# serycjon/WOFT

Measured on AMD Instinct MI355X. Metric: tracked frames/sec at 1080p, 12 RAFT iters; flow EPE vs reference, higher is better.
Workload: dtype bf16x3 (split-bf16 MFMA operands emulating fp32, fp32 accumulate)

## Files before the change

include/woft_hip.h:

```cpp
#ifndef WOFT_HIP_H
#define WOFT_HIP_H

#include <stdint.h>

#ifdef __cplusplus
extern "C" {
#endif

#define WOFT_OK 0
#define WOFT_EINVAL (-1)
#define WOFT_ELAUNCH (-2)

int woft_abi_version(void);
int woft_sizeof(int which);
int woft_set_tuning(int key, int value);

enum woft_epilogue {
    WOFT_EPI_LINEAR = 0,
    WOFT_EPI_RELU = 1,
    WOFT_EPI_SIGMOID = 2,
    WOFT_EPI_TANH = 3,
    WOFT_EPI_RELU_RES_RELU = 4,
    WOFT_EPI_GRU_ZR = 5,
    WOFT_EPI_GRU_Q = 6,
    WOFT_EPI_CTX = 7,
    WOFT_EPI_WH_MEAN = 8,
    WOFT_EPI_FLOWHEAD = 9
};

typedef struct woft_conv_params {
    const float* in0;
    const float* in1;
    int32_t cs0, cs1;
    int32_t c_split;
    int32_t n_img, h, w;
    int32_t ho, wo;
    int32_t taps_y, taps_x;
    int32_t stride, pad_y, pad_x;
    int32_t cin_pad;
    int32_t flat;
    const float* wgt;
    const void* wgt_hi;
    const void* wgt_lo;
    int32_t precision;
    const float* bias;
    float alpha;
    int32_t cout;
    int32_t cout_pad;
    float* out;
    int64_t ldo;
    int32_t co_off;
    int32_t out_w, out_pitch;
    int32_t epi;
    int32_t split;
    const float* e0;
    const float* e1;
    int32_t lde0, lde1;
    float* out1;
    int32_t ldo1;
    float* stat_sum;
    float* stat_sq;
    int32_t tile_m, tile_n;
    int32_t halo;
    int32_t in_norm;
    const float* in_mean;
    const float* in_rstd;
    const float* bias_map;
    int32_t ld_bias_map;
    const int32_t* out_index;
    const float* wh0_lookup;
    int32_t wh0_ld;
    const float* wh0_mean;
    const void* wh0_w;
    const float* wh0_bias;
    const int32_t* wh0_index;
    const void* wgt_frag;
    const void* wgt_mx;
    int32_t roi_y0, roi_x0, roi_h, roi_w;
} woft_conv_params;

int woft_conv2d(const woft_conv_params* p, void* stream);
int woft_conv2d_pair(const woft_conv_params* a, const woft_conv_params* b, void* stream);
int woft_upload_u8(const void* src, void* pinned, void* dev, int64_t bytes, int32_t n_chunks, void* stream);
int woft_split_bf16(const float* x, int64_t n, void* hi, void* lo, void* stream);
int woft_conv3x3_narrow(const float* in, int32_t cs, int32_t n_img, int32_t h, int32_t w, int32_t cin_pad,
                        const float* wgt, const float* bias, int32_t cout, float* out, int64_t ldo, int32_t co_off,
                        void* stream);
int woft_flow_head_update(const float* in, int32_t cs, int32_t h, int32_t w, int32_t cin_pad, const float* wgt,
                          const float* bias, float* delta, int64_t ld_delta, float* coords1, float* flow4,
                          float* flow_cat, int32_t ld_cat, void* stream);
int woft_flow_head_gather(const float* part, int32_t n_planes, int32_t ld, int32_t h, int32_t w, const float* bias2,
                          float* delta, int64_t ld_delta, float* coords1, float* flow4, float* flow_cat, int32_t ld_cat,
                          void* stream);
int woft_split_bf16_lines(const float* x, int64_t n, void* out, void* stream);
int woft_corr_gemm_bf16(const void* a, const void* b, int64_t m, int64_t n, int64_t rows_a, int64_t rows_b, int32_t k,
                        float alpha, void* out, int64_t ldo, int32_t terms, int32_t out_bf16, void* stream);

int woft_inorm_finalize(const float* stat_sum, const float* stat_sq, int32_t n_part, int32_t ld,
                        int32_t channels, int32_t channels_pad, int64_t count, float eps,
                        float* mean, float* rstd, void* ws, void* stream);
int64_t woft_inorm_ws_bytes(void);
int woft_inorm_apply(const float* x, const float* mean, const float* rstd, const float* res,
                     const float* res_mean, const float* res_rstd, int32_t res_mode,
                     float* out, int64_t n_pix, int32_t channels, int32_t mode, void* stream);

int woft_preprocess_bgr_u8(const uint8_t* img, int32_t h, int32_t w, float* out,
                           int32_t hp, int32_t wp, int32_t pad_top, int32_t pad_left, void* stream);

int woft_avgpool2_nhwc(const float* in, int32_t h, int32_t w, int32_t c, float* out, void* stream);

int woft_feature_pyramid(const float* in, int32_t h, int32_t w, int32_t c, int32_t levels, float* const* pooled,
                         void* const* split, int32_t terms, void* stream);

typedef struct woft_lookup_params {
    const void* vol[4];
    int32_t ht[4], wt[4];
    int64_t plane[4];
    int32_t levels, radius;
    const float* coords;
    int64_t n_pix;
    float* out;
    int32_t ldo;
    int32_t vol_bf16;
    int32_t ablate;
} woft_lookup_params;
int woft_corr_lookup(const woft_lookup_params* p, void* stream);
typedef struct woft_lookup_otf_params {
    const void* f1;
    const void* f2[4];
    int32_t h[4], w[4];
    int32_t levels, radius, terms;
    int32_t hf, wf, k;
    float alpha;
    const float* coords;
    float* out;
    const int32_t* need;
    int32_t ldo;
    int32_t ablate;
    const float* fh_part;
    const float* fh_bias;
    float* fh_delta;
    float* fh_flow4;
    float* fh_flow_cat;
    int32_t fh_planes, fh_ld, fh_ld_delta, fh_ld_cat;
    int32_t roi_y0, roi_x0, roi_h, roi_w;
    int32_t smp_y0, smp_x0, smp_h, smp_w;
} woft_lookup_otf_params;
int woft_corr_lookup_otf(const woft_lookup_otf_params* p, void* stream);
int woft_tile_rows(const float* in, int32_t h, int32_t w, int32_t c, float* out, void* stream);

int woft_coords_update(float* coords1, const float* delta, int32_t ld_delta, int32_t wf, int64_t n_pix,
                       float* flow4, float* flow_cat, int32_t ld_cat, void* stream);
int woft_coords_init(float* coords1, int32_t hf, int32_t wf, float* flow4, float* flow_cat,
                     int32_t ld_cat, void* stream);
int woft_coords_init_flow(float* coords1, const float* flow_init, int32_t hf, int32_t wf, float* flow4, float* flow_cat,
                          int32_t ld_cat, void* stream);
int woft_forward_interpolate(const float* flow, int32_t hf, int32_t wf, float* out, void* stream);

int woft_sample_bilinear(const float* data, int32_t c, int32_t h, int32_t w, const float* x, const float* y, int64_t n,
                         float* out, void* stream);
int woft_flow_chain(const float* fab, const float* fbc, int32_t h, int32_t w, float* fac, void* stream);
int woft_flow_fb(const float* fab, const float* fba, int32_t h, int32_t w, float alpha, float beta, float* err, float* ok,
                 void* stream);

int woft_flow_chain_fold(const float* prev_flow, const float* prev_cost, const float* prev_vis, const float* step_flow,
                         const float* step_wlogit, const float* step_mlogit, int32_t h, int32_t w, float unit_cost,
                         float vis_thr, int32_t k, int32_t first, float* best_flow, float* best_cost, float* best_vis,
                         int32_t* best_sel, void* stream);

#define WOFT_CHAIN_HIST 130
int woft_chain_tc(const float* flow, const float* cost, const float* vis, const int32_t* sel, const uint8_t* tmask, int32_t gh,
                  int32_t gw, int32_t mh, int32_t mw, float vis_thr, float* dst, float* w, float* ok, int32_t* hist, void* stream);

int woft_features_pack(const float* f1, int64_t ld_f1, const float* net, int64_t ld_net, const float* inp, int64_t ld_inp,
                       int64_t P, int32_t fdim, int32_t hdim, int32_t cdim, float* record, void* stream);
int woft_features_unpack(const float* record, int64_t P, int32_t fdim, int32_t hdim, int32_t cdim, float* fmap, int64_t ld_fmap,
                         void* fmap_split, float* net, int64_t ld_net, float* xbuf, int64_t ld_xbuf, float* inp_c,
                         int64_t ld_inp_c, void* stream);

int woft_colsum(const float* f, int64_t n_pix, int32_t c, double* ws, int32_t n_part, double* total, void* stream);
int woft_wh_conv0(const float* lookup, int32_t ld_lookup, const float* mean, int64_t n_pix, int32_t nwin,
                  const float* wt, const float* bias, float* out, const int32_t* index, void* stream);
int woft_wh_pack(const float* lookup, int32_t ld_lookup, const float* f1, int32_t c, const double* f2_total,
                 float alpha, int64_t n_pix, int32_t nwin, float* mean, float* x8, void* stream);
int woft_wh_reduce(const float* act, int32_t c, int32_t nwin2, const float* w, float bias,
                   int64_t n_pix, float* out, void* stream);
int woft_warp_features(const float* f, int32_t h, int32_t w, int32_t c, int32_t cs, const float* coords, int64_t n_pix,
                       float* out, int32_t ld_out, void* stream);
int woft_wh_needed(const float* pts, const int32_t* count, int32_t n_max, int32_t top, int32_t left, int32_t hf, int32_t wf,
                   const int32_t* index, int32_t n_win, int32_t* bitmap, int32_t* dyn_index, int32_t* n_needed, void* stream);

int woft_convex_upsample(const float* coords1, const float* wlow, const float* mask, int32_t ld_mask,
                         int32_t hf, int32_t wf, int32_t crop_top, int32_t crop_left, int32_t h, int32_t w,
                         float* flow_up, float* dst, float* wout, int32_t do_sigmoid, void* stream);
int woft_convex_weights_at(const float* pts, const int32_t* count, int32_t n_max, const float* wlow, const float* mask,
                           int32_t ld_mask, int32_t hf, int32_t wf, int32_t crop_top, int32_t crop_left,
                           int32_t do_sigmoid, float* wsel, void* stream);
#define WOFT_WH_TRAIN_CHUNK 16
#define WOFT_WH_TRAIN_MAX_WIN (9 * 2048)
int woft_convex_weights_at_bwd(const float* pts, const int32_t* count, int32_t n_max, const float* g_wsel, const float* wlow,
                               const float* mask, int32_t ld_mask, int32_t hf, int32_t wf, int32_t crop_top,
                               int32_t crop_left, int32_t do_sigmoid, const int32_t* index, int32_t n_win, float* g_wlow,
                               void* stream);
int woft_wh_reduce_bwd(const float* act, const float* w6, const float* g_wlow, const int32_t* index, int32_t n_win,
                       float* g_act, double* ws, float* g_w6, float* g_b6, void* stream);
int woft_wh_train_conv(const float* x, int32_t cin, const float* wt, const float* bias, const float* gate, int32_t n_win,
                       float* y, void* stream);
int64_t woft_wh_wgrad_ws_bytes(int32_t n_win, int32_t cin);
int woft_wh_wgrad(const float* gy, const float* x, int32_t cin, int32_t cin_out, int32_t n_win, float* ws, float* gw,
                  float* gb, void* stream);
int woft_flow_to_tc(const float* flow, const float* weights, int32_t h, int32_t w, float* dst, float* wout,
                    int32_t do_sigmoid, void* stream);
int woft_upflow8(const float* coords1, const float* wlow, int32_t hf, int32_t wf,
                 int32_t crop_top, int32_t crop_left, int32_t h, int32_t w,
                 float* flow_up, float* dst, float* wout, int32_t do_sigmoid, void* stream);

int woft_warp_perspective_u8(const uint8_t* img, int32_t h, int32_t w, int32_t c, const double* hinv,
                             uint8_t* out, uint8_t* valid, int32_t nearest, void* stream);

int woft_warp_perspective_window_u8(const uint8_t* img, int32_t h, int32_t w, int32_t c, const double* hinv, int32_t y0,
                                    int32_t x0, int32_t hw, int32_t ww, uint8_t* out, uint8_t* valid, int32_t nearest,
                                    void* stream);
int woft_crop_u8(const uint8_t* img, int32_t h, int32_t w, int32_t c, int32_t y0, int32_t x0, int32_t hw, int32_t ww,
                 uint8_t* out, void* stream);
int64_t woft_mask_bbox_ws_bytes(void);
int woft_mask_bbox(const uint8_t* mask, int32_t h, int32_t w, const double* hinv, uint8_t* warped, void* ws, int32_t* bbox,
                   void* stream);

int woft_resize_linear_u8(const uint8_t* img, int32_t h, int32_t w, int32_t c, uint8_t* out, int32_t ho, int32_t wo,
                          float scale_y, float scale_x, void* stream);

int64_t woft_tc_select_ws_bytes(int64_t n);
int woft_tc_select(const float* dst, const float* w, const uint8_t* tmask, const uint8_t* pwmask, int32_t gh,
                   int32_t gw, int32_t mh, int32_t mw, int32_t check_dst, const float* sobol_u, int32_t n_draw,
                   void* ws, float* pa, float* pb, float* wout, int32_t cap, int32_t* count, void* stream);
int woft_tc_flags(const float* dst, const uint8_t* tmask, const uint8_t* pwmask, int32_t gh, int32_t gw, int32_t mh,
                  int32_t mw, int32_t check_dst, uint8_t* flags, void* stream);
int woft_tc_select_vis(const float* dst, const float* w, const uint8_t* tmask, const uint8_t* pwmask, int32_t gh,
                       int32_t gw, int32_t mh, int32_t mw, int32_t check_dst, const float* sobol_u, int32_t n_draw,
                       const float* vis, int32_t vis_mode, float vis_thr, void* ws, float* pa, float* pb, float* wout,
                       int32_t cap, int32_t* count, void* stream);
int woft_tc_flags_vis(const float* dst, const uint8_t* tmask, const uint8_t* pwmask, int32_t gh, int32_t gw, int32_t mh,
                      int32_t mw, int32_t check_dst, const float* vis, int32_t vis_mode, float vis_thr, uint8_t* flags,
                      void* stream);

#define WOFT_HFIT_SINGLE_MAX 2048
int64_t woft_hfit_ws_bytes(void);
int woft_hfit(const float* pa, const float* pb, const float* w, int32_t n_max, const int32_t* count,
              int32_t reweight, float huber_k, int32_t n_irls, void* ws, float* Hout, int32_t* status, void* stream);
#define WOFT_HFIT_BATCH_MAX 65535
int woft_hfit_batched(const float* pa, const float* pb, const float* w, int32_t batch, int32_t n_max,
                      const int32_t* counts, int32_t reweight, float huber_k, int32_t n_irls, float* Hout,
                      int32_t* status, void* stream);
int woft_hfit_batched_bwd(const float* pa, const float* pb, const float* w, int32_t batch, int32_t n_max,
                          const int32_t* counts, const float* gH, float* gpa, float* gpb, float* gw, int32_t* status,
                          void* stream);
int woft_hfit_step(const float* pa, const float* pb, const float* w, int32_t n, const float* rew, int32_t first,
                   void* ws, float* res, float* Hout, int32_t* status, void* stream);
int woft_inlier_frac(const float* pa, const float* pb, int32_t n_max, const int32_t* count, const float* H,
                     float thr, float* frac, void* stream);

int64_t woft_ransac_ws_bytes(int32_t n_max, int32_t max_iters);
int woft_ransac(const float* pa, const float* pb, int32_t n_max, const int32_t* count, int32_t max_iters, double thr,
                double conf, uint64_t seed, int32_t refine, void* ws, float* Hout, int32_t* status, int32_t* info,
                uint8_t* inlier_mask, void* stream);

int64_t woft_trs_ws_bytes(int32_t n_max, int32_t max_iters);
int woft_trs(const float* pa, const float* pb, int32_t n_max, const int32_t* count, int32_t max_iters, double thr,
             double conf, uint64_t seed, int32_t refine, void* ws, float* Hout, int32_t* status, int32_t* info,
             uint8_t* inlier_mask, void* stream);

#ifdef __cplusplus
}
#endif
#endif
```

woft_amd/_lib.py:

```python
import ctypes as C
import os
from pathlib import Path

import torch

LIB_PATH = Path(os.environ.get("WOFT_HIP_LIB") or Path(__file__).resolve().parent / "lib" / "libwoft_hip.so")

EPI_LINEAR, EPI_RELU, EPI_SIGMOID, EPI_TANH, EPI_RELU_RES_RELU, EPI_GRU_ZR, EPI_GRU_Q, EPI_CTX, EPI_WH_MEAN, EPI_FLOWHEAD = range(10)

vp, i32, i64, f32 = C.c_void_p, C.c_int32, C.c_int64, C.c_float


class ConvParams(C.Structure):
    _fields_ = [
        ("in0", vp), ("in1", vp), ("cs0", i32), ("cs1", i32), ("c_split", i32),
        ("n_img", i32), ("h", i32), ("w", i32), ("ho", i32), ("wo", i32),
        ("taps_y", i32), ("taps_x", i32), ("stride", i32), ("pad_y", i32), ("pad_x", i32),
        ("cin_pad", i32), ("flat", i32), ("wgt", vp), ("wgt_hi", vp), ("wgt_lo", vp), ("precision", i32),
        ("bias", vp), ("alpha", f32),
        ("cout", i32), ("cout_pad", i32), ("out", vp), ("ldo", i64), ("co_off", i32),
        ("out_w", i32), ("out_pitch", i32), ("epi", i32), ("split", i32),
        ("e0", vp), ("e1", vp), ("lde0", i32), ("lde1", i32), ("out1", vp), ("ldo1", i32),
        ("stat_sum", vp), ("stat_sq", vp), ("tile_m", i32), ("tile_n", i32), ("halo", i32),
        ("in_norm", i32), ("in_mean", vp), ("in_rstd", vp), ("bias_map", vp), ("ld_bias_map", i32),
        ("out_index", vp),
        ("wh0_lookup", vp), ("wh0_ld", i32), ("wh0_mean", vp), ("wh0_w", vp), ("wh0_bias", vp), ("wh0_index", vp),
        ("wgt_frag", vp), ("wgt_mx", vp),
        ("roi_y0", i32), ("roi_x0", i32), ("roi_h", i32), ("roi_w", i32),
    ]


class LookupParams(C.Structure):
    _fields_ = [
        ("vol", vp * 4), ("ht", i32 * 4), ("wt", i32 * 4), ("plane", i64 * 4),
        ("levels", i32), ("radius", i32), ("coords", vp), ("n_pix", i64), ("out", vp), ("ldo", i32),
        ("vol_bf16", i32), ("ablate", i32),
    ]


class LookupOtfParams(C.Structure):
    _fields_ = [
        ("f1", vp), ("f2", vp * 4), ("h", i32 * 4), ("w", i32 * 4),
        ("levels", i32), ("radius", i32), ("terms", i32), ("hf", i32), ("wf", i32), ("k", i32),
        ("alpha", f32), ("coords", vp), ("out", vp), ("need", vp), ("ldo", i32), ("ablate", i32),
        ("fh_part", vp), ("fh_bias", vp), ("fh_delta", vp), ("fh_flow4", vp), ("fh_flow_cat", vp),
        ("fh_planes", i32), ("fh_ld", i32), ("fh_ld_delta", i32), ("fh_ld_cat", i32),
        ("roi_y0", i32), ("roi_x0", i32), ("roi_h", i32), ("roi_w", i32),
        ("smp_y0", i32), ("smp_x0", i32), ("smp_h", i32), ("smp_w", i32),
    ]


_SIGS = {
    "woft_abi_version": (i32, []),
    "woft_sizeof": (i32, [i32]),
    "woft_set_tuning": (i32, [i32, i32]),
    "woft_conv2d": (i32, [C.POINTER(ConvParams), vp]),
    "woft_conv2d_pair": (i32, [C.POINTER(ConvParams), C.POINTER(ConvParams), vp]),
    "woft_upload_u8": (i32, [vp, vp, vp, i64, i32, vp]),
    "woft_split_bf16": (i32, [vp, i64, vp, vp, vp]),
    "woft_split_bf16_lines": (i32, [vp, i64, vp, vp]),
    "woft_flow_to_tc": (i32, [vp, vp, i32, i32, vp, vp, i32, vp]),
    "woft_corr_lookup_otf": (i32, [C.POINTER(LookupOtfParams), vp]),
    "woft_conv3x3_narrow": (i32, [vp, i32, i32, i32, i32, i32, vp, vp, i32, vp, i64, i32, vp]),
    "woft_flow_head_update": (i32, [vp, i32, i32, i32, i32, vp, vp, vp, i64, vp, vp, vp, i32, vp]),
    "woft_flow_head_gather": (i32, [vp, i32, i32, i32, i32, vp, vp, i64, vp, vp, vp, i32, vp]),
    "woft_corr_gemm_bf16": (i32, [vp, vp, i64, i64, i64, i64, i32, f32, vp, i64, i32, i32, vp]),
    "woft_inorm_finalize": (i32, [vp, vp, i32, i32, i32, i32, i64, f32, vp, vp, vp, vp]),
    "woft_inorm_ws_bytes": (i64, []),
    "woft_inorm_apply": (i32, [vp, vp, vp, vp, vp, vp, i32, vp, i64, i32, i32, vp]),
    "woft_preprocess_bgr_u8": (i32, [vp, i32, i32, vp, i32, i32, i32, i32, vp]),
    "woft_avgpool2_nhwc": (i32, [vp, i32, i32, i32, vp, vp]),
    "woft_feature_pyramid": (i32, [vp, i32, i32, i32, i32, vp, vp, i32, vp]),
    "woft_corr_lookup": (i32, [C.POINTER(LookupParams), vp]),
    "woft_tile_rows": (i32, [vp, i32, i32, i32, vp, vp]),
    "woft_coords_update": (i32, [vp, vp, i32, i32, i64, vp, vp, i32, vp]),
    "woft_coords_init": (i32, [vp, i32, i32, vp, vp, i32, vp]),
    "woft_coords_init_flow": (i32, [vp, vp, i32, i32, vp, vp, i32, vp]),
    "woft_forward_interpolate": (i32, [vp, i32, i32, vp, vp]),
    "woft_sample_bilinear": (i32, [vp, i32, i32, i32, vp, vp, i64, vp, vp]),
    "woft_flow_chain": (i32, [vp, vp, i32, i32, vp, vp]),
    "woft_flow_fb": (i32, [vp, vp, i32, i32, f32, f32, vp, vp, vp]),
    "woft_flow_chain_fold": (i32, [vp, vp, vp, vp, vp, vp, i32, i32, f32, f32, i32, i32, vp, vp, vp, vp, vp]),
    "woft_chain_tc": (i32, [vp, vp, vp, vp, vp, i32, i32, i32, i32, f32, vp, vp, vp, vp, vp]),
    "woft_features_pack": (i32, [vp, i64, vp, i64, vp, i64, i64, i32, i32, i32, vp, vp]),
    "woft_features_unpack": (i32, [vp, i64, i32, i32, i32, vp, i64, vp, vp, i64, vp, i64, vp, i64, vp]),
    "woft_colsum":(i32, [vp, i64, i32, vp, i32, vp, vp]),
    "woft_wh_pack": (i32, [vp, i32, vp, i32, vp, f32, i64, i32, vp, vp, vp]),
    "woft_wh_conv0": (i32, [vp, i32, vp, i64, i32, vp, vp, vp, vp, vp]),
    "woft_wh_reduce": (i32, [vp, i32, i32, vp, f32, i64, vp, vp]),
    "woft_warp_features": (i32, [vp, i32, i32, i32, i32, vp, i64, vp, i32, vp]),
    "woft_wh_needed": (i32, [vp, vp, i32, i32, i32, i32, i32, vp, i32, vp, vp, vp, vp]),
    "woft_convex_upsample": (i32, [vp, vp, vp, i32, i32, i32, i32, i32, i32, i32, vp, vp, vp, i32, vp]),
    "woft_convex_weights_at": (i32, [vp, vp, i32, vp, vp, i32, i32, i32, i32, i32, i32, vp, vp]),
    "woft_convex_weights_at_bwd": (i32, [vp, vp, i32, vp, vp, vp, i32, i32, i32, i32, i32, i32, vp, i32, vp, vp]),
    "woft_wh_reduce_bwd": (i32, [vp, vp, vp, vp, i32, vp, vp, vp, vp, vp]),
    "woft_wh_train_conv": (i32, [vp, i32, vp, vp, vp, i32, vp, vp]),
    "woft_wh_wgrad_ws_bytes": (i64, [i32, i32]),
    "woft_wh_wgrad": (i32, [vp, vp, i32, i32, i32, vp, vp, vp, vp]),
    "woft_upflow8": (i32, [vp, vp, i32, i32, i32, i32, i32, i32, vp, vp, vp, i32, vp]),
    "woft_warp_perspective_u8": (i32, [vp, i32, i32, i32, C.POINTER(C.c_double), vp, vp, i32, vp]),
    "woft_resize_linear_u8": (i32, [vp, i32, i32, i32, vp, i32, i32, f32, f32, vp]),
    "woft_warp_perspective_window_u8": (i32, [vp, i32, i32, i32, C.POINTER(C.c_double), i32, i32, i32, i32, vp, vp, i32, vp]),
    "woft_crop_u8": (i32, [vp, i32, i32, i32, i32, i32, i32, i32, vp, vp]),
    "woft_mask_bbox_ws_bytes": (i64, []),
    "woft_mask_bbox": (i32, [vp, i32, i32, C.POINTER(C.c_double), vp, vp, vp, vp]),
    "woft_tc_select_ws_bytes": (i64, [i64]),
    "woft_tc_select": (i32, [vp, vp, vp, vp, i32, i32, i32, i32, i32, vp, i32, vp, vp, vp, vp, i32, vp, vp]),
    "woft_tc_flags": (i32, [vp, vp, vp, i32, i32, i32, i32, i32, vp, vp]),
    "woft_tc_select_vis": (i32, [vp, vp, vp, vp, i32, i32, i32, i32, i32, vp, i32, vp, i32, f32, vp, vp, vp, vp, i32, vp, vp]),
    "woft_tc_flags_vis": (i32, [vp, vp, vp, i32, i32, i32, i32, i32, vp, i32, f32, vp, vp]),
    "woft_hfit_ws_bytes": (i64, []),
    "woft_hfit": (i32, [vp, vp, vp, i32, vp, i32, f32, i32, vp, vp, vp, vp]),
    "woft_hfit_batched": (i32, [vp, vp, vp, i32, i32, vp, i32, f32, i32, vp, vp, vp]),
    "woft_hfit_batched_bwd": (i32, [vp, vp, vp, i32, i32, vp, vp, vp, vp, vp, vp, vp]),
    "woft_hfit_step": (i32, [vp, vp, vp, i32, vp, i32, vp, vp, vp, vp, vp]),
    "woft_inlier_frac": (i32, [vp, vp, i32, vp, vp, f32, vp, vp]),
    "woft_ransac_ws_bytes": (i64, [i32, i32]),
    "woft_ransac": (i32, [vp, vp, i32, vp, i32, C.c_double, C.c_double, C.c_uint64, i32, vp, vp, vp, vp, vp, vp]),
    "woft_trs_ws_bytes": (i64, [i32, i32]),
    "woft_trs": (i32, [vp, vp, i32, vp, i32, C.c_double, C.c_double, C.c_uint64, i32, vp, vp, vp, vp, vp, vp]),
}

EXPORTS = tuple(_SIGS)
_lib = None


class WoftHipError(RuntimeError):
    pass


def load():
    global _lib
    if _lib is not None:
        return _lib
    if not LIB_PATH.exists():
        raise WoftHipError(f"{LIB_PATH} is missing: build it with `python -m woft_amd.build` "
                           "(hipcc --offload-arch=gfx950); woft_amd has no CPU fallback")
    lib = C.CDLL(str(LIB_PATH))
    for name, (res, args) in _SIGS.items():
        fn = getattr(lib, name)
        fn.restype, fn.argtypes = res, args
    if lib.woft_sizeof(0) != C.sizeof(ConvParams) or lib.woft_sizeof(1) != C.sizeof(LookupParams) \
            or lib.woft_sizeof(2) != C.sizeof(LookupOtfParams):
        raise WoftHipError("ctypes mirror of woft_conv_params / woft_lookup_params is out of sync with the library")
    _lib = lib
    return lib


def check(rc, what):
    if rc != 0:
        raise WoftHipError(f"{what} failed with code {rc}")


def ptr(t):
    return None if t is None else t.data_ptr()


_RAW_STREAM = getattr(torch._C, "_cuda_getCurrentRawStream", None) if os.environ.get("WOFT_RAW_STREAM", "1") != "0" else None
_CUR_DEV = torch.cuda.current_device


def stream_ptr():
    if _RAW_STREAM is None:
        return torch.cuda.current_stream().cuda_stream
    return _RAW_STREAM(_CUR_DEV())
```

woft_amd/csrc/elementwise.hip:

```cpp
#include <string.h>

#include "common.h"
#include "halo_map.h"

namespace {

__global__ void preprocess_kernel(const uint8_t* __restrict__ img, int h, int w, float* __restrict__ out,
                                  int hp, int wp, int pad_top, int pad_left) {
    const int64_t i = (int64_t)blockIdx.x * blockDim.x + threadIdx.x;
    if (i >= (int64_t)hp * wp) return;
    const int y = (int)(i / wp), x = (int)(i - (int64_t)y * wp);
    const int sy = min(max(y - pad_top, 0), h - 1), sx = min(max(x - pad_left, 0), w - 1);
    const uint8_t* px = img + ((int64_t)sy * w + sx) * 3;
    f32x4 v;
    v[0] = 2.f * ((float)px[2] / 255.0f) - 1.0f;
    v[1] = 2.f * ((float)px[1] / 255.0f) - 1.0f;
    v[2] = 2.f * ((float)px[0] / 255.0f) - 1.0f;
    v[3] = 0.f;
    *(f32x4*)(out + i * 4) = v;
}

constexpr int FIN_T = 256, FIN_MAXG = 64, FIN_MAXC = 256;
__global__ __launch_bounds__(FIN_T) void inorm_finalize_kernel(const float* __restrict__ s1, const float* __restrict__ s2,
                                                               int n_part, int ld, int channels, int channels_pad,
                                                               int64_t count, float eps, float* __restrict__ mean,
                                                               float* __restrict__ rstd, double* ws) {
    __shared__ double red[2][FIN_T * 4];
    __shared__ int s_last;
    const int c4n = (channels + 3) / 4;
    const int rpp = FIN_T / c4n;
    const int tr = threadIdx.x / c4n, tc = threadIdx.x - tr * c4n;
    const int G = gridDim.x, g = blockIdx.x;
    double a[4] = {0.0, 0.0, 0.0, 0.0}, b[4] = {0.0, 0.0, 0.0, 0.0};
    if (tr < rpp)
        for (int i = g * rpp + tr; i < n_part; i += G * rpp) {
            const f32x4 u = *(const f32x4*)(s1 + (int64_t)i * ld + tc * 4), v = *(const f32x4*)(s2 + (int64_t)i * ld + tc * 4);
#pragma unroll
            for (int k = 0; k < 4; ++k) {
                a[k] += (double)u[k];
                b[k] += (double)v[k];
            }
        }
#pragma unroll
    for (int k = 0; k < 4; ++k) {
        red[0][threadIdx.x * 4 + k] = a[k];
        red[1][threadIdx.x * 4 + k] = b[k];
    }
    __syncthreads();
    const int c = threadIdx.x;
    double ta = 0.0, tb = 0.0;
    if (c < channels) {
        const int q = c >> 2, k = c & 3;
        for (int r = 0; r < rpp; ++r) {
            ta += red[0][(r * c4n + q) * 4 + k];
            tb += red[1][(r * c4n + q) * 4 + k];
        }
    }
    if (G > 1) {
        if (c < channels) {
            ws[(int64_t)g * 2 * FIN_MAXC + c] = ta;
            ws[(int64_t)g * 2 * FIN_MAXC + FIN_MAXC + c] = tb;
        }
        int* ticket = (int*)(ws + (int64_t)FIN_MAXG * 2 * FIN_MAXC);
        asm volatile("s_waitcnt vmcnt(0)" ::: "memory");
        __syncthreads();
        if (threadIdx.x == 0) {
            __builtin_amdgcn_fence(__ATOMIC_RELEASE, "agent");
            asm volatile("s_waitcnt vmcnt(0)" ::: "memory");
            s_last = (__hip_atomic_fetch_add(ticket, 1, __ATOMIC_RELAXED, __HIP_MEMORY_SCOPE_AGENT) == G - 1);
            if (s_last) __builtin_amdgcn_fence(__ATOMIC_ACQUIRE, "agent");
        }
        __syncthreads();
        if (!s_last) return;
        if (threadIdx.x == 0) *ticket = 0;
        int cp = 1;
        while (cp < channels) cp <<= 1;
        const int nsl = FIN_T / cp, sl = threadIdx.x / cp, cc = threadIdx.x & (cp - 1);
        double pa = 0.0, pb = 0.0;
        if (cc < channels) {
#pragma unroll 8
            for (int j = sl; j < G; j += nsl) {
                pa += ws[(int64_t)j * 2 * FIN_MAXC + cc];
                pb += ws[(int64_t)j * 2 * FIN_MAXC + FIN_MAXC + cc];
            }
        }
        __syncthreads();
        red[0][threadIdx.x] = pa;
        red[1][threadIdx.x] = pb;
        __syncthreads();
        ta = tb = 0.0;
        if (c < channels)
            for (int r = 0; r < nsl; ++r) {
                ta += red[0][r * cp + c];
                tb += red[1][r * cp + c];
            }
    }
    if (c < channels) {
        const double mu = ta / (double)count;
        double var = tb / (double)count - mu * mu;
        if (var < 0.0) var = 0.0;
        mean[c] = (float)mu;
        rstd[c] = (float)(1.0 / sqrt(var + (double)eps));
    } else if (c < channels_pad) {
        mean[c] = 0.f;
        rstd[c] = 0.f;
    }
}

__global__ void inorm_apply_kernel(const float* __restrict__ x, const float* __restrict__ mean,
                                   const float* __restrict__ rstd, const float* __restrict__ res,
                                   const float* __restrict__ res_mean, const float* __restrict__ res_rstd, int res_mode,
                                   float* __restrict__ out, int64_t n4, int channels, int mode) {
    const int64_t stride = (int64_t)gridDim.x * blockDim.x;
    for (int64_t i = (int64_t)blockIdx.x * blockDim.x + threadIdx.x; i < n4; i += stride) {
        const int c = (int)((i * 4) % channels);
        f32x4 v = *(const f32x4*)(x + i * 4);
        const f32x4 mu = *(const f32x4*)(mean + c), rs = *(const f32x4*)(rstd + c);
        f32x4 r = {0.f, 0.f, 0.f, 0.f};
        if (mode == 2) {
            r = *(const f32x4*)(res + i * 4);
            if (res_mode != 0) {
                const f32x4 rmu = *(const f32x4*)(res_mean + c), rrs = *(const f32x4*)(res_rstd + c);
#pragma unroll
                for (int k = 0; k < 4; ++k) {
                    r[k] = (r[k] - rmu[k]) * rrs[k];
                    if (res_mode == 2) r[k] = fmaxf(r[k], 0.f);
                }
            }
        }
#pragma unroll
        for (int k = 0; k < 4; ++k) {
            float y = (v[k] - mu[k]) * rs[k];
            if (mode >= 1) y = fmaxf(y, 0.f);
            if (mode == 2) y = fmaxf(r[k] + y, 0.f);
            v[k] = y;
        }
        *(f32x4*)(out + i * 4) = v;
    }
}

__global__ void avgpool2_kernel(const float* __restrict__ in, int h, int w, int c, float* __restrict__ out) {
    const int ho = h / 2, wo = w / 2, c4 = c / 4;
    const int64_t n = (int64_t)ho * wo * c4;
    const int64_t i = (int64_t)blockIdx.x * blockDim.x + threadIdx.x;
    if (i >= n) return;
    const int cc = (int)(i % c4);
    const int64_t pix = i / c4;
    const int oy = (int)(pix / wo), ox = (int)(pix - (int64_t)oy * wo);
    const float* b = in + ((int64_t)(2 * oy) * w + 2 * ox) * c + cc * 4;
    const f32x4 p00 = *(const f32x4*)b, p01 = *(const f32x4*)(b + c);
    const f32x4 p10 = *(const f32x4*)(b + (int64_t)w * c), p11 = *(const f32x4*)(b + (int64_t)w * c + c);
    f32x4 o;
#pragma unroll
    for (int k = 0; k < 4; ++k) o[k] = (p00[k] + p01[k] + p10[k] + p11[k]) * 0.25f;
    *(f32x4*)(out + pix * c + cc * 4) = o;
}

typedef __bf16 pbf16x4 __attribute__((ext_vector_type(4)));
struct PyrArgs {
    const float* in;
    float* pooled[3];
    __bf16* split[4];
    int h, w, c, levels;
};
template <int TERMS>
__device__ __forceinline__ void pyr_split(__bf16* out, int64_t pix, int c, int q, const f32x4 v) {
    const pbf16x4 hi = __builtin_convertvector(v, pbf16x4);
    if (TERMS == 3) {
        __bf16* line = out + pix * (2 * (int64_t)c) + (q >> 3) * 64 + (q & 7) * 4;
        *(pbf16x4*)line = hi;
        *(pbf16x4*)(line + 32) = __builtin_convertvector(v - __builtin_convertvector(hi, f32x4), pbf16x4);
    } else {
        *(pbf16x4*)(out + pix * (int64_t)c + q * 4) = hi;
    }
}
template <int TERMS>
__global__ __launch_bounds__(256) void feature_pyramid_kernel(const PyrArgs a) {
    __shared__ f32x4 l2s[4][64];
    const int bxn = (a.w + 7) / 8;
    const int by = (int)blockIdx.x / bxn, bx = (int)blockIdx.x - by * bxn;
    const int sub = threadIdx.x >> 6, q0 = threadIdx.x & 63;
    const int c4 = a.c / 4;
    const int y0 = by * 8 + (sub >> 1) * 4, x0 = bx * 8 + (sub & 1) * 4;
    const int h1 = a.h / 2, w1 = a.w / 2, h2 = h1 / 2, w2 = w1 / 2, h3 = h2 / 2, w3 = w2 / 2;
    for (int qb = 0; qb < c4; qb += 64) {
        const int q = qb + q0;
        const bool qok = q < c4;
        f32x4 p[4][4];
#pragma unroll
        for (int i = 0; i < 4; ++i)
#pragma unroll
            for (int j = 0; j < 4; ++j) {
                const int y = y0 + i, x = x0 + j;
                const bool ok = qok && y < a.h && x < a.w;
                p[i][j] = ok ? *(const f32x4*)(a.in + ((int64_t)y * a.w + x) * a.c + q * 4) : f32x4{0.f, 0.f, 0.f, 0.f};
                if (ok) pyr_split<TERMS>(a.split[0], (int64_t)y * a.w + x, a.c, q, p[i][j]);
            }
        f32x4 o1[2][2];
#pragma unroll
        for (int i = 0; i < 2; ++i)
#pragma unroll
            for (int j = 0; j < 2; ++j) {
#pragma unroll
                for (int k = 0; k < 4; ++k)
                    o1[i][j][k] = (p[2 * i][2 * j][k] + p[2 * i][2 * j + 1][k] + p[2 * i + 1][2 * j][k] + p[2 * i + 1][2 * j + 1][k]) * 0.25f;
                const int y = y0 / 2 + i, x = x0 / 2 + j;
                if (a.levels > 1 && qok && y < h1 && x < w1) {
                    const int64_t pix = (int64_t)y * w1 + x;
                    *(f32x4*)(a.pooled[0] + pix * a.c + q * 4) = o1[i][j];
                    pyr_split<TERMS>(a.split[1], pix, a.c, q, o1[i][j]);
                }
            }
        f32x4 o2;
#pragma unroll
        for (int k = 0; k < 4; ++k) o2[k] = (o1[0][0][k] + o1[0][1][k] + o1[1][0][k] + o1[1][1][k]) * 0.25f;
        {
            const int y = y0 / 4, x = x0 / 4;
            if (a.levels > 2 && qok && y < h2 && x < w2) {
                const int64_t pix = (int64_t)y * w2 + x;
                *(f32x4*)(a.pooled[1] + pix * a.c + q * 4) = o2;
                pyr_split<TERMS>(a.split[2], pix, a.c, q, o2);
            }
        }
        __syncthreads();
        l2s[sub][q0] = o2;
        __syncthreads();
        if (sub == 0 && a.levels > 3 && qok && by < h3 && bx < w3) {
            f32x4 o3;
#pragma unroll
            for (int k = 0; k < 4; ++k) o3[k] = (l2s[0][q0][k] + l2s[1][q0][k] + l2s[2][q0][k] + l2s[3][q0][k]) * 0.25f;
            const int64_t pix = (int64_t)by * w3 + bx;
            *(f32x4*)(a.pooled[2] + pix * a.c + q * 4) = o3;
            pyr_split<TERMS>(a.split[3], pix, a.c, q, o3);
        }
    }
}

}

extern "C" int woft_abi_version(void) { return 10000 * 0 + 100 * 4 + 0; }

extern "C" int woft_preprocess_bgr_u8(const uint8_t* img, int32_t h, int32_t w, float* out, int32_t hp, int32_t wp,
                                      int32_t pad_top, int32_t pad_left, void* stream) {
    if (!img || !out || h <= 0 || w <= 0 || hp < h || wp < w || pad_top < 0 || pad_left < 0) return WOFT_EINVAL;
    const int64_t n = (int64_t)hp * wp;
    hipLaunchKernelGGL(preprocess_kernel, dim3((unsigned)ceil_div64(n, 256)), dim3(256), 0, (hipStream_t)stream, img, h,
                       w, out, hp, wp, pad_top, pad_left);
    return woft_launch_status();
}

extern "C" int64_t woft_inorm_ws_bytes(void) { return (int64_t)FIN_MAXG * 2 * FIN_MAXC * 8 + 64; }

extern "C" int woft_inorm_finalize(const float* stat_sum, const float* stat_sq, int32_t n_part, int32_t ld,
                                   int32_t channels, int32_t channels_pad, int64_t count, float eps, float* mean,
                                   float* rstd, void* ws, void* stream) {
    if (!stat_sum || !stat_sq || !mean || !rstd || n_part <= 0 || channels <= 0 || count <= 0) return WOFT_EINVAL;
    if (channels_pad < channels || channels_pad > FIN_MAXC || ld % 4 != 0 || ld < channels) return WOFT_EINVAL;
    const int rpp = FIN_T / ((channels + 3) / 4);
    int G = (n_part + 4 * rpp - 1) / (4 * rpp);
    G = (ws == nullptr || G < 2) ? 1 : (G > FIN_MAXG ? FIN_MAXG : G);
    hipLaunchKernelGGL(inorm_finalize_kernel, dim3(G), dim3(FIN_T), 0, (hipStream_t)stream, stat_sum, stat_sq, n_part, ld,
                       channels, channels_pad, count, eps, mean, rstd, (double*)ws);
    return woft_launch_status();
}

extern "C" int woft_inorm_apply(const float* x, const float* mean, const float* rstd, const float* res,
                                const float* res_mean, const float* res_rstd, int32_t res_mode, float* out,
                                int64_t n_pix, int32_t channels, int32_t mode, void* stream) {
    if (!x || !mean || !rstd || !out || n_pix <= 0 || channels <= 0 || channels % 4 != 0) return WOFT_EINVAL;
    if (mode < 0 || mode > 2 || (mode == 2 && !res)) return WOFT_EINVAL;
    if (res_mode < 0 || res_mode > 2 || (res_mode != 0 && (mode != 2 || !res_mean || !res_rstd))) return WOFT_EINVAL;
    const int64_t n4 = n_pix * channels / 4;
    const int64_t blocks = ceil_div64(n4, 256);
    hipLaunchKernelGGL(inorm_apply_kernel, dim3((unsigned)(blocks < 8192 ? blocks : 8192)), dim3(256), 0,
                       (hipStream_t)stream, x, mean, rstd, res, res_mean, res_rstd, res_mode, out, n4, channels, mode);
    return woft_launch_status();
}

extern "C" int woft_avgpool2_nhwc(const float* in, int32_t h, int32_t w, int32_t c, float* out, void* stream) {
    if (!in || !out || h < 2 || w < 2 || c <= 0 || c % 4 != 0) return WOFT_EINVAL;
    const int64_t n = (int64_t)(h / 2) * (w / 2) * (c / 4);
    hipLaunchKernelGGL(avgpool2_kernel, dim3((unsigned)ceil_div64(n, 256)), dim3(256), 0, (hipStream_t)stream, in, h,
                       w, c, out);
    return woft_launch_status();
}

extern "C" int woft_upload_u8(const void* src, void* pinned, void* dev, int64_t bytes, int32_t n_chunks, void* stream) {
    if (!src || !pinned || !dev || bytes <= 0 || n_chunks < 1 || n_chunks > 64) return WOFT_EINVAL;
    const int64_t per = ((bytes + n_chunks - 1) / n_chunks + 4095) / 4096 * 4096;
    for (int64_t off = 0; off < bytes; off += per) {
        const int64_t n = bytes - off < per ? bytes - off : per;
        memcpy((char*)pinned + off, (const char*)src + off, (size_t)n);
        if (hipMemcpyAsync((char*)dev + off, (const char*)pinned + off, (size_t)n, hipMemcpyHostToDevice, (hipStream_t)stream) != hipSuccess)
            return WOFT_ELAUNCH;
    }
    return WOFT_OK;
}

extern "C" int woft_sizeof(int which) {
    if (which == 0) return (int)sizeof(woft_conv_params);
    if (which == 1) return (int)sizeof(woft_lookup_params);
    if (which == 2) return (int)sizeof(woft_lookup_otf_params);
    return -1;
}

extern "C" int woft_feature_pyramid(const float* in, int32_t h, int32_t w, int32_t c, int32_t levels, float* const* pooled,
                                    void* const* split, int32_t terms, void* stream) {
    if (!in || !pooled || !split || h <= 0 || w <= 0 || c <= 0 || c % 32 != 0 || levels < 1 || levels > 4 ||
        (terms != 1 && terms != 3))
        return WOFT_EINVAL;
    PyrArgs a;
    a.in = in; a.h = h; a.w = w; a.c = c; a.levels = levels;
    for (int l = 0; l < 4; ++l) {
        a.split[l] = l < levels ? (__bf16*)split[l] : nullptr;
        if (l < levels && a.split[l] == nullptr) return WOFT_EINVAL;
        if (l >= 1) {
            a.pooled[l - 1] = l < levels ? pooled[l - 1] : nullptr;
            if (l < levels && a.pooled[l - 1] == nullptr) return WOFT_EINVAL;
        }
    }
    const dim3 grid((unsigned)(((h + 7) / 8) * ((w + 7) / 8)));
    if (terms == 3) hipLaunchKernelGGL(feature_pyramid_kernel<3>, grid, dim3(256), 0, (hipStream_t)stream, a);
    else hipLaunchKernelGGL(feature_pyramid_kernel<1>, grid, dim3(256), 0, (hipStream_t)stream, a);
    return woft_launch_status();
}
```

woft_amd/csrc/lookup_otf.hip:

```cpp
#include <type_traits>
#include <utility>

#include "common.h"
#include "dma.h"

namespace {

typedef __bf16 bf16x8 __attribute__((ext_vector_type(8)));

template <bool MAX>
__device__ __forceinline__ int wave_reduce_minmax(int v) {
#define WOFT_DPP_STEP(ctrl, rmask)                                                        \
    {                                                                                     \
        const int o = __builtin_amdgcn_update_dpp(v, v, ctrl, rmask, 0xf, false);         \
        v = MAX ? (o > v ? o : v) : (o < v ? o : v);                                      \
    }
    WOFT_DPP_STEP(0xB1, 0xf)
    WOFT_DPP_STEP(0x4E, 0xf)
    WOFT_DPP_STEP(0x141, 0xf)
    WOFT_DPP_STEP(0x140, 0xf)
    WOFT_DPP_STEP(0x142, 0xa)
    WOFT_DPP_STEP(0x143, 0xc)
#undef WOFT_DPP_STEP
    return __builtin_amdgcn_readlane(v, 63);
}

__device__ __forceinline__ void lds_dma16x2(const void* gbase, uint32_t o0_plus_4096, uint32_t o1, uint32_t lds_addr_second) {
    const uint64_t gb = (uint64_t)(uintptr_t)gbase;
    const uint32_t g_hi = (uint32_t)__builtin_amdgcn_readfirstlane((int)(uint32_t)(gb >> 32));
    const uint32_t g_lo = (uint32_t)__builtin_amdgcn_readfirstlane((int)(uint32_t)gb);
    const uint64_t gu = ((uint64_t)g_hi << 32) | (uint64_t)g_lo;
    uint32_t saved_m0;
    asm volatile("s_mov_b32 %0, m0\n\ts_mov_b32 m0, %1\n\ts_nop 0\n\t"
                 "global_load_lds_dwordx4 %2, %4 offset:-4096\n\tglobal_load_lds_dwordx4 %3, %4\n\ts_mov_b32 m0, %0"
                 : "=&s"(saved_m0)
                 : "s"(lds_addr_second), "v"(o0_plus_4096), "v"(o1), "s"(gu)
                 : "memory", "vcc");
}

struct BlockRect {
    int by0, bx0, ny, nx;
};
__host__ __device__ __forceinline__ BlockRect block_rect(const woft_lookup_otf_params& p) {
    if ((p.roi_y0 | p.roi_x0 | p.roi_h | p.roi_w) == 0) return BlockRect{0, 0, (p.hf + 7) / 8, (p.wf + 7) / 8};
    const int by0 = p.roi_y0 / 8, bx0 = p.roi_x0 / 8;
    return BlockRect{by0, bx0, (p.roi_y0 + p.roi_h - 1) / 8 - by0 + 1, (p.roi_x0 + p.roi_w - 1) / 8 - bx0 + 1};
}

template <int TERMS, int R, int K, int ABL>
__global__ __launch_bounds__(256, 2) void corr_lookup_otf_kernel(const woft_lookup_otf_params p) {
    constexpr int NPX = 64, NT = 256;
    constexpr int NW = 2 * R + 1, N2 = NW * NW;
    constexpr int NPL = (TERMS == 1) ? 1 : 2;
    constexpr int LD = (TERMS == 1) ? K : 2 * K;
    constexpr int NK = LD / 64;
    constexpr int NSUB = (TERMS == 1) ? 4 : 2;
    constexpr int GS = 2, NGRP = 3, NST = GS * NGRP, DEPTH = NGRP - 1;
    static_assert(NK % GS == 0, "K steps per chunk must be a multiple of the steps per barrier");
    __shared__ __attribute__((aligned(16))) __bf16 stage[NST * 64 * 64];
    constexpr int WS = NW + 1, WLD = WS * WS + 2;
    __shared__ __attribute__((aligned(16))) float Wn[NPX * WLD];
    constexpr int MAXL = 4;
    __shared__ __attribute__((aligned(16))) int s_org[MAXL][NPX];
    __shared__ __attribute__((aligned(16))) int s_pm[MAXL][NPX];
    __shared__ float s_fx[MAXL][NPX], s_fy[MAXL][NPX];
    __shared__ int s_box[MAXL][4];
    __shared__ float s_trash[64];
    __shared__ uint32_t s_probe[24];
    int n_probe = 0;

    const int tid = threadIdx.x;
    const int lane = tid & 63;
    const int wave = __builtin_amdgcn_readfirstlane(tid >> 6);
    const int wm = wave >> 1, wn = wave & 1;
    const int r32 = lane & 31, hh = lane >> 5;
    constexpr int ld = LD, nk = NK;
    const BlockRect br = block_rect(p);
    const int tiles_x = br.nx, ntiles = br.nx * br.ny;
    int tile;
    {
        const int q = ntiles / 8, rr = ntiles % 8, xcd = blockIdx.x % 8, idx = blockIdx.x / 8;
        tile = (xcd < rr ? xcd * (q + 1) : rr * (q + 1) + (xcd - rr) * q) + idx;
    }
    const int px0 = (br.bx0 + tile % tiles_x) * 8, py0 = (br.by0 + tile / tiles_x) * 8;
    const bool sampled = (p.smp_y0 | p.smp_x0 | p.smp_h | p.smp_w) == 0 ||
                         (py0 < p.smp_y0 + p.smp_h && py0 + 8 > p.smp_y0 && px0 < p.smp_x0 + p.smp_w && px0 + 8 > p.smp_x0);
    if (p.need != nullptr) {
        int any = 0;
        if (tid < NPX) {
            const int y = py0 + (tid >> 3), x = px0 + (tid & 7);
            if (y < p.hf && x < p.wf) any = p.need[y * p.wf + x];
        }
        if (!__syncthreads_or(any)) return;
    }
    float cx = 0.f, cy = 0.f;
    if (tid < NPX) {
        const int y = py0 + (tid >> 3), x = px0 + (tid & 7);
        if (y < p.hf && x < p.wf) {
            const int64_t i = (int64_t)y * p.wf + x;
            cx = p.coords[i * 2];
            cy = p.coords[i * 2 + 1];
            if (p.fh_part != nullptr) {
                typedef float f32x2 __attribute__((ext_vector_type(2)));
                float dx = p.fh_bias ? p.fh_bias[0] : 0.f, dy = p.fh_bias ? p.fh_bias[1] : 0.f;
                const int64_t plane = (int64_t)p.hf * p.wf * p.fh_ld;
#pragma unroll
                for (int ky = 0; ky < 3; ++ky)
#pragma unroll
                    for (int kx = 0; kx < 3; ++kx) {
                        const int yy = y + ky - 1, xx = x + kx - 1;
                        f32x2 v = {0.f, 0.f};
                        if (yy >= 0 && yy < p.hf && xx >= 0 && xx < p.wf) {
                            const float* src = p.fh_part + ((int64_t)yy * p.wf + xx) * p.fh_ld + (ky * 3 + kx) * 2;
                            v = *(const f32x2*)src;
                            for (int t = 1; t < p.fh_planes; ++t) v += *(const f32x2*)(src + t * plane);
                        }
                        dx += v[0];
                        dy += v[1];
                    }
                p.fh_delta[i * p.fh_ld_delta] = dx;
                p.fh_delta[i * p.fh_ld_delta + 1] = dy;
                cx += dx;
                cy += dy;
                ((float*)p.coords)[i * 2] = cx;
                ((float*)p.coords)[i * 2 + 1] = cy;
                const float fx = cx - (float)x, fy = cy - (float)y;
                if (p.fh_flow4 != nullptr) *(f32x4*)(p.fh_flow4 + i * 4) = f32x4{fx, fy, 0.f, 0.f};
                if (p.fh_flow_cat != nullptr) {
                    p.fh_flow_cat[i * p.fh_ld_cat] = fx;
                    p.fh_flow_cat[i * p.fh_ld_cat + 1] = fy;
                }
            }
        }
    }
    if (!sampled) return;
    if (tid < NPX) {
        const int y = py0 + (tid >> 3), x = px0 + (tid & 7);
        const bool cvalid = y < p.hf && x < p.wf;
#pragma unroll
        for (int l = 0; l < MAXL; ++l) {
            if (l < p.levels) {
                int wx0 = 0, wy0 = 0;
                float fx = 0.f, fy = 0.f;
                if (cvalid) {
                    const float sc = 1.0f / (float)(1 << l);
                    const float xs = cx * sc, ys = cy * sc;
                    float flx = floorf(xs), fly = floorf(ys);
                    fx = xs - flx;
                    fy = ys - fly;
                    flx = fminf(fmaxf(flx, -1.0e6f), 1.0e6f);
                    fly = fminf(fmaxf(fly, -1.0e6f), 1.0e6f);
                    wx0 = (int)flx - R;
                    wy0 = (int)fly - R;
                }
                s_fx[l][tid] = fx; s_fy[l][tid] = fy;
                const int ox = wx0 < -16384 ? -16384 : (wx0 > 16384 ? 16384 : wx0);
                const int oy = wy0 < -16384 ? -16384 : (wy0 > 16384 ? 16384 : wy0);
                s_org[l][tid] = cvalid ? ((ox & 0xffff) | (oy << 16)) : 0x40004000;
                s_pm[l][tid] = 4 * (tid * WLD - (ox * WS + oy));
                const int b0 = wave_reduce_minmax<false>(cvalid ? wx0 : 0x3fffffff), b1 = wave_reduce_minmax<true>(cvalid ? wx0 : -0x3fffffff);
                const int b2 = wave_reduce_minmax<false>(cvalid ? wy0 : 0x3fffffff), b3 = wave_reduce_minmax<true>(cvalid ? wy0 : -0x3fffffff);
                if (tid == 0) { s_box[l][0] = b0; s_box[l][1] = b1; s_box[l][2] = b2; s_box[l][3] = b3; }
            }
        }
    }
    bf16x8 afr[NK][NSUB][NPL];
    {
        const int m = wm * 32 + r32;
        int y = py0 + (m >> 3), x = px0 + (m & 7);
        y = y < p.hf ? y : p.hf - 1;
        x = x < p.wf ? x : p.wf - 1;
        const char* row = (const char*)p.f1 + (int64_t)(y * p.wf + x) * (ld * 2);
#pragma unroll
        for (int ks = 0; ks < NK; ++ks)
#pragma unroll
            for (int s2 = 0; s2 < NSUB; ++s2) {
                if (TERMS == 0) {
                    afr[ks][s2][0] = *(const bf16x8*)(row + ks * 128 + hh * 64 + s2 * 32);
                    afr[ks][s2][NPL - 1] = *(const bf16x8*)(row + ks * 128 + hh * 64 + s2 * 32 + 16);
                } else {
                    afr[ks][s2][0] = *(const bf16x8*)(row + ks * 128 + (s2 * 2 + hh) * 16);
                    if (TERMS == 3) afr[ks][s2][NPL - 1] = *(const bf16x8*)(row + ks * 128 + 64 + (s2 * 2 + hh) * 16);
                }
            }
    }
    const int swz = (4 * (wave & 1) + (lane >> 4)) & 7;
    const uint32_t chunk_off = (uint32_t)(((lane & 7) ^ swz) * 16);
    const uint32_t st_addr = lds_addr_of(stage);
    const int sw = (r32 >> 1) & 7;
    const __bf16* b_rows = stage + (wn * 32 + r32) * 64;

    uint32_t* stamps = ((ABL & 16) && tid == 0 && p.ldo >= 4 * N2 + 24)
                           ? (uint32_t*)(p.out + ((int64_t)py0 * p.wf + px0) * p.ldo + 4 * N2) : nullptr;
    int n_stamp = 0;
    auto stamp = [&]() __attribute__((always_inline)) { if ((ABL & 16) && stamps && n_stamp < 24) stamps[n_stamp++] = (uint32_t)__builtin_amdgcn_s_memtime(); };
    stamp();

    __syncthreads();
    stamp();
    auto sel4 = [](int l, int a0, int a1, int a2, int a3) __attribute__((always_inline)) { return l == 0 ? a0 : (l == 1 ? a1 : (l == 2 ? a2 : a3)); };
    int W = 0, bx0 = 0, by0 = 0, bw = 1, N = 0, S = 0, G = 0;
    bool clipped = false;
    const char* f2 = nullptr;
    uint32_t b_off[2] = {0u, 0u};
    int is_c = 0, is_k = 0;
    auto issue = [&](int s_idx) __attribute__((always_inline)) {
        if (is_k == 0) {
#pragma unroll
            for (int tt = 0; tt < 2; ++tt) {
                int pos = is_c * 64 + (wave + 4 * tt) * 8 + (lane >> 3);
                pos = pos < N ? pos : N - 1;
                const int by = pos / bw, bx = pos - by * bw;
                b_off[tt] = (uint32_t)((by0 + by) * W + bx0 + bx) * (uint32_t)(ld * 2) + chunk_off + (tt == 0 ? 4096u : 0u);
            }
        }
        const uint32_t st = st_addr + (uint32_t)(s_idx % NST) * 8192u;
        if (!(ABL & 1) || s_idx < NST) lds_dma16x2(f2 + is_k * 128, b_off[0], b_off[1], st + (uint32_t)(wave + 4) * 1024u);
        if (++is_k == nk) { is_k = 0; ++is_c; }
    };
    auto start_level = [&](int l) __attribute__((always_inline)) {
        W = sel4(l, p.w[0], p.w[1], p.w[2], p.w[3]);
        const int H = sel4(l, p.h[0], p.h[1], p.h[2], p.h[3]);
        bx0 = __builtin_amdgcn_readfirstlane(s_box[l][0]);
        by0 = __builtin_amdgcn_readfirstlane(s_box[l][2]);
        int bx1 = __builtin_amdgcn_readfirstlane(s_box[l][1]), by1 = __builtin_amdgcn_readfirstlane(s_box[l][3]);
        clipped = bx0 < 0 || by0 < 0 || bx1 + NW > W - 1 || by1 + NW > H - 1;
        bx0 = bx0 > 0 ? bx0 : 0;
        by0 = by0 > 0 ? by0 : 0;
        bx1 = (bx1 + NW < W - 1) ? bx1 + NW : W - 1;
        by1 = (by1 + NW < H - 1) ? by1 + NW : H - 1;
        bw = bx1 - bx0 + 1;
        const int bh = by1 - by0 + 1;
        N = (bw > 0 && bh > 0) ? bw * bh : 0;
        bw = bw > 0 ? bw : 1;
        f2 = (const char*)(l == 0 ? p.f2[0] : (l == 1 ? p.f2[1] : (l == 2 ? p.f2[2] : p.f2[3])));
        S = ((N + 63) / 64) * nk;
        G = S / GS;
        is_c = 0; is_k = 0;
        for (int g = 0; g < DEPTH && g < G; ++g)
#pragma unroll
            for (int e = 0; e < GS; ++e) issue(g * GS + e);
    };
    start_level(0);
    for (int l = 0; l < p.levels; ++l) {
        if (clipped) {
            const f32x4 z4 = {0.f, 0.f, 0.f, 0.f};
            for (int i = tid; i < NPX * WLD / 4; i += NT) ((f32x4*)Wn)[i] = z4;
            static_assert((NPX * WLD) % 4 == 0, "window array is zeroed 16 bytes at a time");
        }
        f32x16 acc;
#pragma unroll
        for (int r = 0; r < 16; ++r) acc[r] = 0.f;
        int c0 = 0;
        stamp();
        for (int s0 = 0; s0 < S; s0 += NK) {
            [&]<int... KGS>(std::integer_sequence<int, KGS...>) {
            ([&] {
                constexpr int kg = KGS;
                const int g = s0 / GS + kg;
                const int rem = G - 1 - g;
                const bool pr = (ABL & 64) && l == 0 && s0 == NK && tid == 0;
                auto mark = [&]() __attribute__((always_inline)) { if ((ABL & 64) && pr && n_probe < 24) s_probe[n_probe++] = (uint32_t)__builtin_amdgcn_s_memtime(); };
                mark();
                if (rem >= DEPTH - 1) dma_wait<(DEPTH - 1) * GS * 2>();
                else dma_wait<0>();
                mark();
                __syncthreads();
                mark();
                const bool feed = g + DEPTH < G;
                mark();
                constexpr int NU = GS * NSUB;
                bf16x8 bq[2][NPL];
                auto load_b = [&](auto u_tag) __attribute__((always_inline)) {
                    constexpr int u = decltype(u_tag)::value;
                    constexpr int e = u / NSUB, s2 = u % NSUB;
                    const __bf16* br = b_rows + ((s0 + kg * GS + e) % NST) * 4096;
                    if (TERMS == 0) {
                        bq[u & 1][0] = *(const bf16x8*)(br + ((hh * 4 + s2 * 2) ^ sw) * 8);
                        bq[u & 1][NPL - 1] = *(const bf16x8*)(br + ((hh * 4 + s2 * 2 + 1) ^ sw) * 8);
                    } else {
                        bq[u & 1][0] = *(const bf16x8*)(br + ((s2 * 2 + hh) ^ sw) * 8);
                        if (TERMS == 3) bq[u & 1][NPL - 1] = *(const bf16x8*)(br + ((4 + s2 * 2 + hh) ^ sw) * 8);
                    }
                };
                if (!(ABL & 2)) {
                    load_b(std::integral_constant<int, 0>{});
                    [&]<int... U>(std::integer_sequence<int, U...>) {
                        ([&] {
                            constexpr int u = U, e = u / NSUB, s2 = u % NSUB;
                            constexpr int ks = kg * GS + e;
                            if constexpr (u + 1 < NU) load_b(std::integral_constant<int, u + 1>{});
                            __builtin_amdgcn_sched_barrier(0);
                            const bf16x8 bh = bq[u & 1][0];
                            if (TERMS == 0) {
                                const f32x4 a0 = __builtin_bit_cast(f32x4, afr[ks][s2][0]), a1 = __builtin_bit_cast(f32x4, afr[ks][s2][NPL - 1]);
                                const f32x4 b0 = __builtin_bit_cast(f32x4, bh), b1 = __builtin_bit_cast(f32x4, bq[u & 1][NPL - 1]);
#pragma unroll
                                for (int s = 0; s < 4; ++s) acc = __builtin_amdgcn_mfma_f32_32x32x2f32(a0[s], b0[s], acc, 0, 0, 0);
#pragma unroll
                                for (int s = 0; s < 4; ++s) acc = __builtin_amdgcn_mfma_f32_32x32x2f32(a1[s], b1[s], acc, 0, 0, 0);
                            } else if (TERMS == 3) {
                                const bf16x8 bl = bq[u & 1][NPL - 1];
                                const bf16x8 ah = afr[ks][s2][0], al = afr[ks][s2][NPL - 1];
                                acc = __builtin_amdgcn_mfma_f32_32x32x16_bf16(al, bh, acc, 0, 0, 0);
                                acc = __builtin_amdgcn_mfma_f32_32x32x16_bf16(ah, bl, acc, 0, 0, 0);
                                acc = __builtin_amdgcn_mfma_f32_32x32x16_bf16(ah, bh, acc, 0, 0, 0);
                            } else {
                                acc = __builtin_amdgcn_mfma_f32_32x32x16_bf16(afr[ks][s2][0], bh, acc, 0, 0, 0);
                            }
                            __builtin_amdgcn_sched_barrier(0);
                            if constexpr (s2 == 0) { if (feed) issue((g + DEPTH) * GS + e); }
                        }(), ...);
                    }(std::make_integer_sequence<int, NU>{});
                }
                mark();
            }(), ...);
            }(std::make_integer_sequence<int, NK / GS>{});
            if (!(ABL & 4)) {
                typedef int i32x4 __attribute__((ext_vector_type(4)));
                typedef unsigned short u16x2 __attribute__((ext_vector_type(2)));
                const int pos = c0 + wn * 32 + r32;
                const int by = pos / bw, bx = pos - by * bw;
                const int tx = bx0 + bx, ty = by0 + by;
                const int d_pos = pos < N ? ((tx & 0xffff) | (ty << 16)) : 0x7fff7fff;
                const uint32_t d_q4 = lds_addr_of(Wn) + 4u * (uint32_t)(tx * WS + ty);
                const uint32_t trash = lds_addr_of(s_trash) + 4u * (uint32_t)lane;
                i32x4 org[4], pm[4];
#pragma unroll
                for (int g4 = 0; g4 < 4; ++g4) {
                    org[g4] = *(const i32x4*)&s_org[l][wm * 32 + 4 * hh + 8 * g4];
                    pm[g4] = *(const i32x4*)&s_pm[l][wm * 32 + 4 * hh + 8 * g4];
                }
                const u16x2 lim = {(unsigned short)(WS - 1), (unsigned short)(WS - 1)};
#pragma unroll
                for (int r = 0; r < 16; ++r) {
                    const u16x2 dd = __builtin_bit_cast(u16x2, d_pos) - __builtin_bit_cast(u16x2, (int)org[r >> 2][r & 3]);
                    const u16x2 mn = __builtin_elementwise_min(dd, lim);
                    const bool inside = __builtin_bit_cast(uint32_t, mn) == __builtin_bit_cast(uint32_t, dd);
                    const uint32_t cell = inside ? (uint32_t)pm[r >> 2][r & 3] + d_q4 : trash;
                    *(__attribute__((address_space(3))) float*)(uintptr_t)cell = acc[r] * p.alpha;
                }
            }
#pragma unroll
            for (int r = 0; r < 16; ++r) acc[r] = 0.f;
            if ((ABL & 64) && l == 0 && s0 == NK && tid == 0 && n_probe < 24) s_probe[n_probe++] = (uint32_t)__builtin_amdgcn_s_memtime();
            c0 += 64;
        }
        stamp();
        __syncthreads();
        if (l + 1 < p.levels) start_level(l + 1);
        if (!(ABL & 8)) {
            for (int it = tid; it < NPX * NW; it += NT) {
                const int pix = it / NW, i = it - pix * NW;
                const int gy = py0 + (pix >> 3), gx = px0 + (pix & 7);
                if (gy >= p.hf || gx >= p.wf) continue;
                const float fx = s_fx[l][pix], fy = s_fy[l][pix];
                const float* cq = Wn + pix * WLD + i * WS;
                float h[WS];
#pragma unroll
                for (int j = 0; j < WS; ++j) h[j] = cq[j] * (1.f - fx) + cq[WS + j] * fx;
                float* o = p.out + ((int64_t)gy * p.wf + gx) * p.ldo + l * N2 + i * NW;
#pragma unroll
                for (int j = 0; j < NW; ++j) o[j] = h[j] * (1.f - fy) + h[j + 1] * fy;
            }
        }
        stamp();
        __syncthreads();
    }
    if ((ABL & 64) && tid == 0 && p.ldo >= 4 * N2 + 24) {
        uint32_t* o = (uint32_t*)(p.out + ((int64_t)py0 * p.wf + px0) * p.ldo + 4 * N2);
        for (int i = 0; i < 24; ++i) o[i] = i < n_probe ? s_probe[i] : 0u;
    }
}

}

extern "C" int woft_corr_lookup_otf(const woft_lookup_otf_params* pp, void* stream) {
    if (!pp) return WOFT_EINVAL;
    const woft_lookup_otf_params& p = *pp;
    if (p.levels < 1 || p.levels > 4 || !p.f1 || !p.coords || !p.out || p.hf <= 0 || p.wf <= 0) return WOFT_EINVAL;
    if (p.terms != 0 && p.terms != 1 && p.terms != 3) return WOFT_EINVAL;
    if (p.k <= 0 || p.k % (p.terms == 1 ? 64 : 32) != 0) return WOFT_EINVAL;
    const int64_t row_bytes = (int64_t)p.k * (p.terms == 1 ? 2 : 4);
    if ((int64_t)p.hf * p.wf * row_bytes >= (1ll << 32)) return WOFT_EINVAL;
    for (int l = 0; l < p.levels; ++l)
        if (!p.f2[l] || p.h[l] <= 0 || p.w[l] <= 0 || (int64_t)p.h[l] * p.w[l] * row_bytes >= (1ll << 32)) return WOFT_EINVAL;
    const int nout = p.levels * (2 * p.radius + 1) * (2 * p.radius + 1);
    if (p.ldo < nout) return WOFT_EINVAL;
    if (p.fh_part != nullptr && (p.fh_delta == nullptr || p.fh_planes < 1 || p.fh_ld < 20 || p.fh_ld % 4 != 0 || p.fh_ld_delta < 2 ||
                                 (p.fh_flow_cat != nullptr && p.fh_ld_cat < 2) || p.need != nullptr))
        return WOFT_EINVAL;
    for (int l = 0; l < p.levels; ++l) {
        if (p.h[l] > 16384 || p.w[l] > 16384) return WOFT_EINVAL;
        if ((int64_t)p.h[l] * p.w[l] * row_bytes >= (1ll << 32) - 4096) return WOFT_EINVAL;
    }
    auto rect_bad = [&](int y0, int x0, int h, int w) {
        return (y0 | x0 | h | w) != 0 && (h <= 0 || w <= 0 || y0 < 0 || x0 < 0 || y0 > p.hf - h || x0 > p.wf - w);
    };
    if (rect_bad(p.roi_y0, p.roi_x0, p.roi_h, p.roi_w) || rect_bad(p.smp_y0, p.smp_x0, p.smp_h, p.smp_w)) return WOFT_EINVAL;
    if (p.ablate != 0 && ((p.roi_y0 | p.roi_x0 | p.roi_h | p.roi_w) != 0 || (p.smp_y0 | p.smp_x0 | p.smp_h | p.smp_w) != 0)) return WOFT_EINVAL;
    hipStream_t s = (hipStream_t)stream;
    const BlockRect br = block_rect(p);
    dim3 grid((unsigned)(br.nx * br.ny));
#define OTF(T, RR, KK, AB) woft_launch(0, corr_lookup_otf_kernel<T, RR, KK, AB>, grid, dim3(256), 0, s, p)
    if (p.ablate != 0) {
        if (!(p.k == 256 && p.radius == 4 && p.terms == 3)) return WOFT_EINVAL;
        switch (p.ablate) {
            case 1: OTF(3, 4, 256, 1); break;
            case 2: OTF(3, 4, 256, 2); break;
            case 3: OTF(3, 4, 256, 3); break;
            case 8: OTF(3, 4, 256, 8); break;
            case 15: OTF(3, 4, 256, 15); break;
            case 16: OTF(3, 4, 256, 16); break;
            case 64: OTF(3, 4, 256, 64); break;
            default: return WOFT_EINVAL;
        }
    } else if (p.k == 256 && p.radius == 4) {
        if (p.terms == 3) OTF(3, 4, 256, 0); else if (p.terms == 0) OTF(0, 4, 256, 0); else OTF(1, 4, 256, 0);
    } else if (p.k == 128 && p.radius == 3) {
        if (p.terms == 3) OTF(3, 3, 128, 0); else if (p.terms == 0) OTF(0, 3, 128, 0); else OTF(1, 3, 128, 0);
    }
    else return WOFT_EINVAL;
#undef OTF
    return woft_launch_status();
}
```

woft_amd/engine.py:

```python
import math
import os
from typing import NamedTuple

import torch

from . import _lib, conv_select, flow_region, ops, wh_train
from .conv_select import KERNELS, Kernel
from .ops import Act, new_act

EPI = _lib
DEFER_NORM = os.environ.get("WOFT_DEFER_NORM", "1") != "0"
FUSE_FLOWHEAD = os.environ.get("WOFT_FUSE_FLOWHEAD", "1") != "0"
PAIR_BRANCHES = os.environ.get("WOFT_PAIR", "1") != "0"
PYRAMID_ONE_LAUNCH = os.environ.get("WOFT_PYRAMID", "1") != "0"
FOLD_GATHER = os.environ.get("WOFT_FOLD_GATHER", "1") != "0"


def _ru(x, m):
    return (x + m - 1) // m * m


class Step(NamedTuple):
    kind: str
    arg: object
    tag: str = None


class _Folded(NamedTuple):
    prog_iter_first: list
    prog_iter: list
    prog_iter_last: list
    gather: list
    lookup: object


def _timed(sink, launch, *args, extra=None):
    if sink is None:
        return launch(*args)
    s, e = torch.cuda.Event(enable_timing=True), torch.cuda.Event(enable_timing=True)
    s.record()
    launch(*args)
    e.record()
    sink.append((s, e) if extra is None else (s, e, extra()))


def _head_layers(sd, prefix, cin):
    idx = sorted(int(k.split(".")[2]) for k in sd if k.startswith(prefix) and k.endswith(".weight"))
    shapes = [tuple(sd[f"{prefix}{i}.weight"].shape) for i in idx]
    ok = not (len(idx) < 2 or shapes[-1][0] != 1 or shapes[-1][2:] != (1, 1) or shapes[0][1] != cin
              or any(a[0] != b[1] for a, b in zip(shapes, shapes[1:])) or any(sh[2] != sh[3] or sh[2] % 2 == 0 for sh in shapes))
    return idx, shapes, ok


class _Spec:

    def __init__(self, small):
        self.small = small
        if small:
            self.fdim, self.hdim, self.cdim, self.radius = 128, 96, 64, 3
            self.fnorm, self.cnorm = "instance", "none"
        else:
            self.fdim, self.hdim, self.cdim, self.radius = 256, 128, 128, 4
            self.fnorm, self.cnorm = "instance", "batch"
        self.levels = 4
        self.nwin = 2 * self.radius + 1
        self.corr_c = self.levels * self.nwin ** 2
        self.corr_cs = _ru(self.corr_c, 32)
        self.xdim = _ru(self.cdim + (82 if small else 128), 32)
        self.flow_off = self.cdim + (80 if small else 126)


class _Enc:

    def __init__(self, sd, p, norm, spec, out_split=None):
        self.norm = norm

        def get(name, stride=1, flat_cs=0, bn=None):
            w, b = sd[name + ".weight"], sd[name + ".bias"]
            if norm == "batch" and bn is not None:
                w, b = ops.fold_bn(w, b, sd[bn + ".weight"], sd[bn + ".bias"], sd[bn + ".running_mean"],
                                   sd[bn + ".running_var"])
            return ops.pack_conv(w, b, stride=stride, flat_cs=flat_cs)

        self.conv1 = get(p + ".conv1", 2, 4, p + ".norm1")
        self.blocks = []
        for li, stride in ((1, 1), (2, 2), (3, 2)):
            for bi in range(2):
                q = f"{p}.layer{li}.{bi}"
                s = stride if bi == 0 else 1
                if spec.small:
                    convs = [get(q + ".conv1", 1, bn=q + ".norm1"), get(q + ".conv2", s, bn=q + ".norm2"),
                             get(q + ".conv3", 1, bn=q + ".norm3")]
                else:
                    convs = [get(q + ".conv1", s, bn=q + ".norm1"), get(q + ".conv2", 1, bn=q + ".norm2")]
                blk = dict(stride=s, convs=convs)
                if s != 1:
                    blk["down"] = get(q + ".downsample.0", s, bn=q + ".downsample.1")
                self.blocks.append(blk)
        w2, b2 = sd[p + ".conv2.weight"], sd[p + ".conv2.bias"]
        if out_split:
            self.conv2_net = ops.pack_conv(w2[:out_split], b2[:out_split])
            self.conv2_inp = ops.pack_conv(w2[out_split:], b2[out_split:])
        else:
            self.conv2 = ops.pack_conv(w2, b2)


class RaftEngine:
    def __init__(self, state_dict, small=False, weighted=True, precision="fp32", corr="volume", volume_storage=None,
                 mask_head=False):
        if precision not in ops.PRECISION:
            raise ValueError(f"precision must be one of {sorted(ops.PRECISION)}")
        if corr not in ("volume", "otf"):
            raise ValueError("corr must be 'volume' or 'otf'")
        self.precision = precision
        self.prec_corr = self.prec_wh = "bf16x3" if precision in ("fp16", "f16mx8") else precision
        self.corr = corr
        self.volume_storage = volume_storage or ("bf16" if precision == "bf16" else "fp32")
        if self.volume_storage not in ("fp32", "bf16") or (self.volume_storage == "bf16" and precision == "fp32"):
            raise ValueError("volume_storage: 'fp32', or 'bf16' with the split-bf16 precisions (their GEMM packs it)")
        _lib.load()
        if not torch.cuda.is_available():
            raise _lib.WoftHipError("woft_amd needs a HIP device: there is no CPU fallback")
        sd = {k: v.detach().float().cpu() for k, v in state_dict.items()}
        self.weighted, self.small, self.mask_head = weighted, small, bool(mask_head)
        self.spec = sp = _Spec(small)
        self.radius, self.levels = sp.radius, sp.levels
        if self.mask_head and not weighted:
            raise ValueError("mask_head: the MaskHead belongs to WeightedRAFT (weighted_raft.py:75-76), not to plain RAFT")
        self.convc2 = self.mk1 = self.mk2 = None
        self.wh_std = self.wh_flat0 = False
        self.wh0 = self.wh2 = self.wh4 = self.wh0_frag = self.wh_layers = self.wh6_c = self.wh6_w = self.wh6_b = None
        self.mh_shapes = self.mh_layers = self.mh_c = self.mh_wlast = self.mh_b = None
        self._pack_encoders(sd)
        self._pack_update_block(sd)
        if weighted:
            self._pack_weight_head(sd)
        if self.mask_head:
            self._pack_mask_head(sd)
        self._plans = {}

    def _pack_encoders(self, sd):
        self.fnet = _Enc(sd, "fnet", self.spec.fnorm, self.spec)
        self.cnet = _Enc(sd, "cnet", self.spec.cnorm, self.spec, out_split=self.spec.hdim)

    def _pack_update_block(self, sd):
        sp, small, precision = self.spec, self.small, self.precision
        u = "update_block."
        g = lambda n, **kw: ops.pack_conv(sd[u + n + ".weight"], sd[u + n + ".bias"], **kw)
        self.convc1 = g("encoder.convc1")
        self.convf1 = g("encoder.convf1", flat_cs=4)
        self.convf2 = g("encoder.convf2")
        self.convm = g("encoder.conv")
        self.fh1 = g("flow_head.conv1")
        self.fh2 = g("flow_head.conv2")
        self.fh2_frag = (ops.pack_flowhead_frags(sd[u + "flow_head.conv2.weight"], 2 if precision in ("bf16x3", "f16mx8") else 1,
                                                 f16=precision == "fp16")
                         if precision != "fp32" and FUSE_FLOWHEAD else None)
        if not small:
            self.convc2 = g("encoder.convc2")
            self.mk1 = g("mask.0")
            self.mk2 = g("mask.2", scale=0.25)
        hd_, cd_, mot = sp.hdim, sp.cdim, (82 if small else 128)
        dyn = [(0, hd_, 0), (hd_ + cd_, hd_ + cd_ + mot, hd_)]
        ctx = [(hd_, hd_ + cd_, 0)]
        self.zr_dyn, self.zr_inp, self.q_dyn, self.q_inp = [], [], [], []
        for sfx, pd in (("", None),) if small else (("1", (0, 2)), ("2", (2, 0))):
            zr_w, zr_b = (torch.cat([sd[f"{u}gru.convz{sfx}{s}"], sd[f"{u}gru.convr{sfx}{s}"]], 0) for s in (".weight", ".bias"))
            q_w, q_b = sd[f"{u}gru.convq{sfx}.weight"], sd[f"{u}gru.convq{sfx}.bias"]
            self.zr_dyn.append(ops.pack_conv(zr_w, None, padding=pd, cin_layout=dyn))
            self.zr_inp.append(ops.pack_conv(zr_w, zr_b, padding=pd, cin_layout=ctx))
            self.q_dyn.append(ops.pack_conv(q_w, None, padding=pd, cin_layout=dyn))
            self.q_inp.append(ops.pack_conv(q_w, q_b, padding=pd, cin_layout=ctx))

    def _pack_weight_head(self, sd):
        sp, precision = self.spec, self.precision
        w = "weight_head.net."
        idx, shapes, ok = _head_layers(sd, w, sp.levels + 1)
        if not ok:
            raise ValueError(f"weight head layers {shapes}: not a WeightHead (weighted_raft.py:318-345)")
        self.wh_std = shapes == [(128, 5, 3, 3), (128, 128, 3, 3), (128, 128, 3, 3), (1, 128, 1, 1)]
        last = idx[-1]
        if self.wh_std:
            self.wh0, self.wh2, self.wh4, self.wh0_frag = self._wh_std_packed(sd)
        else:
            k0 = shapes[0][2]
            self.wh_flat0 = k0 * 8 <= 32
            self.wh_layers = [ops.pack_conv(sd[f"{w}{idx[0]}.weight"], sd[f"{w}{idx[0]}.bias"], flat_cs=8 if self.wh_flat0 else 0)]
            self.wh_layers += [ops.pack_conv(sd[f"{w}{i}.weight"], sd[f"{w}{i}.bias"]) for i in idx[1:-1]]
        self.wh6_c = shapes[-1][1]
        self.wh6_w = torch.zeros(_ru(self.wh6_c, 4))
        self.wh6_w[:self.wh6_c] = sd[f"{w}{last}.weight"].reshape(-1)
        self.wh6_w = self.wh6_w.contiguous().cuda()
        self.wh6_b = float(sd[f"{w}{last}.bias"].item())

    def _wh_std_packed(self, sd):
        w = "weight_head.net."
        wh0 = ops.pack_conv(sd[w + "0.weight"], sd[w + "0.bias"], flat_cs=8)
        wh2 = ops.pack_conv(sd[w + "2.weight"], sd[w + "2.bias"])
        wh4 = ops.pack_conv(sd[w + "4.weight"], sd[w + "4.bias"])
        wh0_frag = (ops.pack_wh0_frags(sd[w + "0.weight"], 2 if self.prec_wh == "bf16x3" else 1)
                    if self.precision != "fp32" and self.spec.nwin == 9 else None)
        return wh0, wh2, wh4, wh0_frag

    def repack_weight_head(self, sd):
        assert self.weighted and self.wh_std
        sd = {k: v.detach().float().cpu() for k, v in sd.items() if k.startswith("weight_head.net.")}
        wh0, wh2, wh4, frag = self._wh_std_packed(sd)
        for old, new in ((self.wh0, wh0), (self.wh2, wh2), (self.wh4, wh4)):
            ops.repack_conv_(old, new)
        if self.wh0_frag is not None:
            self.wh0_frag.copy_(frag)
        self.wh6_w[:self.wh6_c].copy_(sd["weight_head.net.6.weight"].reshape(-1))
        self.wh6_b = float(sd["weight_head.net.6.bias"].item())
        for plan in self._plans.values():
            plan.wh0_t.copy_(self.wh0.wgt[:128].t())
            plan.wh6_b.fill_(self.wh6_b)
            if plan._wh6_pad is not None:
                plan._wh6_pad[:self.wh6_c].copy_(self.wh6_w[:self.wh6_c])
            plan._graphs.clear()

    def _pack_mask_head(self, sd):
        sp = self.spec
        m = "mask_head.net."
        idx, shapes, ok = _head_layers(sd, m, 2 * sp.fdim)
        if not ok:
            raise ValueError(f"mask head layers {shapes}: not a MaskHead on {2 * sp.fdim} channels (weighted_raft.py:387-409)")
        self.mh_shapes = shapes
        self.mh_layers = [ops.pack_conv(sd[f"{m}{i}.weight"], sd[f"{m}{i}.bias"]) for i in idx[:-1]]
        self.mh_c = shapes[-1][1]
        self.mh_wlast = sd[f"{m}{idx[-1]}.weight"].reshape(-1).clone()
        self.mh_b = float(sd[f"{m}{idx[-1]}.bias"].item())

    def plan(self, hp, wp, slot=0):
        key = (hp, wp) if slot == 0 else (hp, wp, slot)
        if key not in self._plans:
            self._plans[key] = _Plan(self, hp, wp)
        return self._plans[key]

    def drop_plan(self, key):
        return self._plans.pop(key, None)


class _Plan:

    def __init__(self, eng, hp, wp):
        assert hp % 8 == 0 and wp % 8 == 0
        self.eng, self.hp, self.wp = eng, hp, wp
        self.prec, self.prec_corr, self.prec_wh = eng.precision, eng.prec_corr, eng.prec_wh
        self.otf = eng.corr == "otf"
        self.hf, self.wf, self.P = hp // 8, wp // 8, (hp // 8) * (wp // 8)
        self.source_tag = None
        self.target_valid = False
        self.lookup_events = None
        self.wh_events = None
        self.conv_events = None
        self._graphs = {}
        self.mk = self.mask = self.prog_iter_last = self.folded = self.fh_part = None
        self.x8 = self.x32 = self.wmean = self.wlow = self.cs_ws = self.cs_tot = self.wh6_b = self._wh6_pad = None
        self.a1 = self.a2 = self.wh0_t = self.wh_last = None
        self.wh0_direct = self.wh0_fused = self.wh_fused = False
        self.prog_mask, self.prog_wh, self.prog_mh = [], [], []
        self.mh_warped = self.mh_last = self.mh_w = self.mh_low = None
        self.flow_region, self._flow_regions = None, {}
        self.wh_region, self._wh_regions = None, {}
        self._wh_dyn = {}
        self._wh_train = None
        self._plan_features()
        self._plan_update_block()
        if eng.weighted:
            self._plan_weight_head()
        if eng.mask_head:
            self._plan_mask_head()

    @staticmethod
    def _z(*s, dtype=torch.float32):
        return torch.zeros(*s, dtype=dtype, device="cuda")

    def _plan_features(self):
        eng, sp, hp, wp, hf, wf, P, z = self.eng, self.eng.spec, self.hp, self.wp, self.hf, self.wf, self.P, self._z
        self.img = [new_act(1, hp, wp, 3, cs=4), new_act(1, hp, wp, 3, cs=4)]
        self.f1rows = z(_ru(P, 128), sp.fdim)
        self.f1 = Act(self.f1rows[:P], 1, hf, wf, sp.fdim)
        x3 = self.prec_corr == "bf16x3"
        bf = lambda rows: (z(rows.shape[0], rows.shape[1] * (2 if x3 else 1), dtype=torch.bfloat16)
                           if self.prec != "fp32" else None)
        self.f1s = bf(self.f1rows)
        if self.otf and self.prec == "fp32":
            self.f1s = self.f1rows
        self.dims, self.f2rows, self.f2act, self.vol, self.f2s = [], [], [], [], []
        h, w = hf, wf
        for _ in range(sp.levels):
            self.dims.append((h, w))
            self.f2act.append(new_act(1, h, w, sp.fdim, zero=True))
            if self.otf:
                self.f2s.append(bf(self.f2act[-1].t) if self.prec != "fp32" else self.f2act[-1].t)
            else:
                n = ops.tiled_dims(h, w)[2]
                rows = z(_ru(n, 128), sp.fdim)
                self.f2rows.append(rows)
                self.f2s.append(bf(rows))
                self.vol.append(z(P, n, dtype=torch.bfloat16 if eng.volume_storage == "bf16" else torch.float32))
            h, w = h // 2, w // 2
        self.net0 = new_act(1, hf, wf, sp.hdim, zero=True)
        self.xbuf = new_act(1, hf, wf, sp.xdim, zero=True)
        self.flow_cat = self.xbuf.t[:, sp.flow_off:]
        self._enc_scratch = {}
        n_stat = 2 * math.ceil((hp // 2) * (wp // 2) / 64) * 128
        self.stats = (z(n_stat), z(n_stat))
        self.fin_ws = ops.inorm_ws("cuda")
        self._norm_slots = {}
        self.prog_f_src = self._encoder_program(eng.fnet, self.img[0], [(eng.fnet.conv2, self.f1, 0, EPI.EPI_LINEAR)])
        self.prog_f_dst = self._encoder_program(eng.fnet, self.img[1],
                                                [(eng.fnet.conv2, self.f2act[0], 0, EPI.EPI_LINEAR)])
        self.prog_c_src = self._encoder_program(eng.cnet, self.img[0],
                                                [(eng.cnet.conv2_net, self.net0, 0, EPI.EPI_TANH),
                                                 (eng.cnet.conv2_inp, self.xbuf, 0, EPI.EPI_RELU)])
        self.prog_volume = self._volume_program()

    def _plan_update_block(self):
        eng, sp, hf, wf, P, z, cp = self.eng, self.eng.spec, self.hf, self.wf, self.P, self._z, self._cp
        self.coords = z(P, 2)
        self.corr = new_act(1, hf, wf, sp.corr_c, cs=sp.corr_cs, zero=True)
        self.c1 = new_act(1, hf, wf, 96 if sp.small else 256, zero=True)
        self.cf = new_act(1, hf, wf, 128 if sp.small else 256, zero=True)
        self.fl1 = new_act(1, hf, wf, 64 if sp.small else 128, zero=True)
        self.flow4 = new_act(1, hf, wf, 2, cs=4, zero=True)
        self.inp_c = new_act(1, hf, wf, sp.cdim, zero=True)
        self.gate_bias = [(new_act(1, hf, wf, 2 * sp.hdim, zero=True), new_act(1, hf, wf, sp.hdim, zero=True))
                          for _ in eng.zr_inp]
        self.prog_gate_bias = []
        for k in range(len(eng.zr_inp)):
            self.prog_gate_bias += [Step("conv", cp(self.inp_c, eng.zr_inp[k], self.gate_bias[k][0])),
                                    Step("conv", cp(self.inp_c, eng.q_inp[k], self.gate_bias[k][1]))]
        self.zbuf = new_act(1, hf, wf, sp.hdim, zero=True)
        self.rh = new_act(1, hf, wf, sp.hdim, zero=True)
        self.hA = new_act(1, hf, wf, sp.hdim, zero=True)
        self.hB = new_act(1, hf, wf, sp.hdim, zero=True)
        self.fh = new_act(1, hf, wf, 128 if sp.small else 256, zero=True)
        self.delta = new_act(1, hf, wf, 2, cs=4, zero=True)
        self.flow_init = z(2, hf, wf)
        if self.otf:
            terms = 3 if self.prec_corr == "bf16x3" else (0 if self.prec == "fp32" else 1)
            self.lookup = ops.make_lookup_otf_params(self.f1s, self.f2s, self.dims, hf, wf, sp.fdim, self.coords,
                                                     self.corr.t, sp.radius, terms)
        else:
            self.lookup = ops.make_lookup_params(self.vol, self.dims, self.coords, self.corr.t, sp.radius)
        self.prog_iter_first = self._iter_program(first=True)
        self.prog_iter = self._iter_program(first=False)
        if not sp.small:
            self.mk = new_act(1, hf, wf, 256, zero=True)
            self.mask = new_act(1, hf, wf, 576, zero=True)
            self.prog_mask = [cp(self.hB, eng.mk1, self.mk, epi=EPI.EPI_RELU),
                              cp(self.mk, eng.mk2, self.mask)]
            k = next((i for i, st in enumerate(self.prog_iter) if st.tag == "fh1"), None)
            if PAIR_BRANCHES and k is not None and ops.pair_ok(self.prog_iter[k].arg, self.prog_mask[0]):
                self.prog_iter_last = (self.prog_iter[:k] + [Step("conv2", (self.prog_iter[k].arg, self.prog_mask[0]), "fh1+mk1")]
                                       + self.prog_iter[k + 1:])
        self.folded = self._fold_gather_programs()

    def _plan_weight_head(self):
        eng, sp, P, z, n = self.eng, self.eng.spec, self.P, self._z, self.eng.spec.nwin
        self.x8 = new_act(P, n, n, 5, cs=8, zero=True)
        self.wmean = z(P)
        self.wlow = z(P)
        self.cs_ws = z(256, sp.fdim, dtype=torch.float64)
        self.cs_tot = z(sp.fdim, dtype=torch.float64)
        self.wh6_b = torch.tensor([eng.wh6_b], dtype=torch.float32, device="cuda")
        cpw = lambda *a, **kw: self._cp(*a, precision=self.prec_wh, **kw)
        if eng.wh_std:
            self.a2 = new_act(P, n, n, 128)
            self.wh0_direct = n in (7, 9)
            self.wh0_fused = (eng.wh0_frag is not None and os.environ.get("WOFT_WH0_FUSED", "1") != "0"
                              and ops.select_conv(self.a2, eng.wh2, precision=self.prec_wh).kernel is Kernel.WINDOW_9X9)
            self.a1 = self.a2 if self.wh0_fused else new_act(P, n, n, 128)
            self.wh0_t = eng.wh0.wgt[:128].t().contiguous()
            self.prog_wh, self.wh_fused = self._wh_program(P, None)
            return
        x = self.x8
        if not eng.wh_flat0:
            self.x32 = x = new_act(P, n, n, 5, cs=32, zero=True)
        for pc in eng.wh_layers:
            out = new_act(P, n, n, pc.cout, cs=_ru(_ru(pc.cout, 4), 32), zero=True)
            self.prog_wh.append(cpw(x, pc, out, epi=EPI.EPI_RELU))
            x = out
        self.wh_last = x

    def _plan_mask_head(self):
        eng, sp, hf, wf = self.eng, self.eng.spec, self.hf, self.wf
        self.mh_warped = new_act(1, hf, wf, sp.fdim, zero=True)
        x = None
        for k, pc in enumerate(eng.mh_layers):
            out = new_act(1, hf, wf, pc.cout, cs=_ru(_ru(pc.cout, 4), 32), zero=True)
            src = dict(x2=self.mh_warped, c_split=sp.fdim) if k == 0 else {}
            self.prog_mh.append(self._cp(self.f1 if k == 0 else x, pc, out, epi=EPI.EPI_RELU, precision=self.prec_wh, **src))
            x = out
        self.mh_last = x
        self.mh_w = torch.zeros(x.cs, dtype=torch.float32)
        self.mh_w[:eng.mh_c] = eng.mh_wlast
        self.mh_w = self.mh_w.to("cuda")
        self.mh_low = self._z(self.P)

    def _fold_gather_programs(self):
        progs = [p for p in (self.prog_iter_first, self.prog_iter, self.prog_iter_last) if p is not None]
        if not (FOLD_GATHER and self.otf and all(p and p[-1].kind == "fh_gather" and p[0].kind == "lookup" for p in progs)):
            return None
        n_planes, bias2 = self.prog_iter[-1].arg
        lk = ops.copy_params(self.lookup)
        lk.fh_part, lk.fh_bias, lk.fh_delta = _lib.ptr(self.fh_part), _lib.ptr(bias2), _lib.ptr(self.delta.t)
        lk.fh_flow4, lk.fh_flow_cat = _lib.ptr(self.flow4.t), self.flow_cat.data_ptr()
        lk.fh_planes, lk.fh_ld, lk.fh_ld_delta, lk.fh_ld_cat = n_planes, self.fh_part.shape[1], self.delta.cs, self.xbuf.cs
        lk._keep = (self.lookup._keep, bias2, self.fh_part)
        first, mid, last = ([head] + p[1:-1] if p is not None else None
                            for p, head in ((self.prog_iter_first, self.prog_iter_first[0]), (self.prog_iter, Step("lookup", lk)),
                                            (self.prog_iter_last, Step("lookup", lk))))
        return _Folded(first, mid, last, [self.prog_iter[-1]], lk)

    def _wh_program(self, n_win, index):
        eng, n = self.eng, self.eng.spec.nwin
        cp = lambda *a, **kw: self._cp(*a, precision=self.prec_wh, **kw)
        a1 = Act(self.a1.t[:n_win * n * n], n_win, n, n, 128)
        a2 = Act(self.a2.t[:n_win * n * n], n_win, n, n, 128)
        prog = ([] if self.wh0_direct else [cp(self.x8, eng.wh0, a1, epi=EPI.EPI_RELU)]) + [
            cp(a1, eng.wh2, a2, epi=EPI.EPI_RELU), cp(a2, eng.wh4, a1, epi=EPI.EPI_RELU)]
        if self.wh0_fused:
            assert Kernel(prog[0].halo) is Kernel.WINDOW_9X9
            prog[0] = cp(a1, eng.wh2, a2, epi=EPI.EPI_RELU,
                         wh0=(self.corr, self.wmean, eng.wh0_frag, eng.wh0.bias, index))
        last = prog[-1]
        fused = Kernel(last.halo) is Kernel.WINDOW_9X9
        if fused:
            last.epi = EPI.EPI_WH_MEAN
            last.e0, last.e1 = _lib.ptr(eng.wh6_w), _lib.ptr(self.wh6_b)
            last.out, last.ldo, last.co_off = _lib.ptr(self.wlow), 1, 0
            last.out_index = _lib.ptr(index) if index is not None else None
        return prog, fused

    def set_weight_region(self, index):
        if index is None or not (self.eng.weighted and self.wh0_direct and self.wh_fused):
            self.wh_region = None
            return
        key = index.data_ptr()
        if key not in self._wh_regions:
            prog, fused = self._wh_program(int(index.numel()), index)
            assert fused
            self._wh_regions[key] = (index, prog)
        self.wh_region = self._wh_regions[key]

    def _layer_taps(self):
        e = self.eng
        r = lambda pc: (flow_region.reach(pc.kh or pc.taps_y, pc.pad_y), flow_region.reach(pc.kw or pc.taps_x, pc.pad_x))
        return {"convc1": r(e.convc1), "convc2": r(e.convc2), "convf1": r(e.convf1), "convf2": r(e.convf2), "convm": r(e.convm),
                "gru0": r(e.zr_dyn[0]), "gru1": r(e.zr_dyn[1]), "fh1": r(e.fh1), "fh2": r(e.fh2), "mk1": r(e.mk1), "mk2": r(e.mk2)}

    def set_flow_region(self, rect, iters=None):
        self.flow_region = None
        sp = self.eng.spec
        if rect is None or iters is None or iters < 2 or sp.small or not self.otf or self.folded is None \
                or self.prog_iter_last is None or len(self.eng.zr_dyn) != 2:
            return False
        key = (tuple(int(v) for v in rect), int(iters))
        if key not in self._flow_regions:
            self._flow_regions[key] = self._flow_region_programs(*key, [self._iteration(it, key[1], True) for it in range(key[1])])
        self.flow_region = self._flow_regions[key]
        return self.flow_region is not None

    def _iteration(self, it, iters, folded):
        progs = self.folded if folded else self
        if it == 0:
            return progs.prog_iter_first
        if it == iters - 1 and progs.prog_iter_last is not None:
            return progs.prog_iter_last
        return progs.prog_iter

    def _flow_region_programs(self, rect, iters, base):
        hf, wf = self.hf, self.wf
        taps = self._layer_taps()
        parts = {}
        for first in (True, False):
            for _, pp in flow_region.iteration_launches(taps, first=first, last=True, folded=True):
                for part in pp:
                    parts[(first, part[0])] = part
        launches, where = [], []
        for it in range(iters):
            for k, st in enumerate(base[it]):
                if st.kind == "lookup":
                    names = (["gather"] if st.arg.fh_part else []) + ["lookup"]
                elif st.kind in ("conv", "conv2") and st.tag is not None:
                    names = st.tag.split("+")
                else:
                    return None
                if any((it == 0, n) not in parts for n in names):
                    return None
                launches.append((it, st.tag or "lookup", [parts[(it == 0, n)] for n in names]))
                where.append((it, k))
        launches += [(-1, tag, pp) for tag, pp in flow_region.closing_launches(taps)]
        rects, _ = flow_region.schedule(launches, flow_region.final_need(rect, hf, wf), hf, wf)

        def tiles(kernel, r):
            if kernel is not None:
                return conv_select.roi_tiles(kernel, r, hf, wf)
            y0, x0, h, w = r or (0, 0, hf, wf)
            return (-(-(y0 + h) // 8) - y0 // 8) * (-(-(x0 + w) // 8) - x0 // 8)

        small = lambda r, kernel=None: (r is not None and not flow_region.is_full(r, hf, wf)
                                        and 10 * tiles(kernel, r) <= 9 * tiles(kernel, None))
        roi = lambda p: KERNELS[Kernel(p.halo)].roi

        def restricted(p, r):
            q = ops.copy_params(p)
            q.roi_y0, q.roi_x0, q.roi_h, q.roi_w = r
            return q

        progs = {}
        for (it, k), (_, tag, _), rr in zip(where, launches, rects):
            st = base[it][k]
            new = None
            if st.kind == "lookup" and small(rr[-1]):
                lk = restricted(st.arg, rr[0])
                lk.smp_y0, lk.smp_x0, lk.smp_h, lk.smp_w = rr[-1]
                new = Step("lookup", lk)
            elif st.kind == "conv" and roi(st.arg) and small(rr[0], Kernel(st.arg.halo)):
                new = Step("conv", restricted(st.arg, rr[0]), tag + "@roi")
            elif st.kind == "conv2" and roi(st.arg[0]) and any(small(r, Kernel(st.arg[0].halo)) for r in rr):
                new = Step("conv2", tuple(restricted(p, r) if small(r, Kernel(p.halo)) else p for p, r in zip(st.arg, rr)), tag + "@roi")
            if new is not None:
                progs.setdefault(it, list(base[it]))[k] = new
        if not progs:
            return None
        return {"key": (rect, iters), "iters": progs,
                "rects": [(it, tag, rr) for (it, tag, _), rr in zip(launches, rects)]}

    def _cp(self, *a, **kw):
        kw.setdefault("precision", self.prec)
        return ops.conv_params(*a, **kw)

    def _scratch(self, name, n, h, w, c):
        cs = _ru(c, 32)
        key = (name, h, w, cs)
        if key not in self._enc_scratch:
            self._enc_scratch[key] = new_act(n, h, w, c, cs=cs, zero=True)
        return self._enc_scratch[key]

    def _encoder_program(self, e, img, outputs):
        prog = []
        inorm = e.norm == "instance"
        tag = "i" if inorm else "c"

        def slot(name):
            key = f"{tag}_{name}"
            if key not in self._norm_slots:
                self._norm_slots[key] = (torch.zeros(256, device="cuda"), torch.zeros(256, device="cuda"))
            return self._norm_slots[key]

        def materialise(x):
            if not isinstance(x, list):
                return x
            if x[4] is None:
                _, raw_x, mode, ms, _ = x
                x[4] = self._scratch(f"{tag}_mat_{len(prog)}", 1, raw_x.h, raw_x.w, raw_x.c)
                prog.append(Step("apply", (raw_x, x[4], mode - 1, None, ms, None, 0)))
            return x[4]

        def layer(x, pc, name, relu, res=None, defer=False):
            xin, in_norm, in_stats = x, 0, None
            if isinstance(x, list):
                _, raw_x, mode, ms, mat = x
                if mat is None and ops.select_conv(raw_x, pc, in_norm=mode, precision=self.prec).in_norm:
                    xin, in_norm, in_stats = raw_x, mode, ms
                else:
                    xin = materialise(x)
            ho, wo = pc.out_hw(xin.h, xin.w)
            out = self._scratch(f"{tag}_{name}", 1, ho, wo, pc.cout)
            kw = dict(in_norm=in_norm, in_stats=in_stats) if in_norm else {}
            if not inorm:
                epi = EPI.EPI_RELU_RES_RELU if res is not None else (EPI.EPI_RELU if relu else EPI.EPI_LINEAR)
                prog.append(Step("conv", self._cp(xin, pc, out, epi=epi, e0=materialise(res) if res is not None else None, **kw)))
                return out
            raw = self._scratch(f"{tag}_raw_{name}", 1, ho, wo, pc.cout)
            p = self._cp(xin, pc, raw, stats=self.stats, **kw)
            rows = 2 * p._m_tiles
            ms = slot(name)
            prog.append(Step("conv", p))
            prog.append(Step("fin", (rows, pc.cout_pad, pc.cout, raw.cs, p._m, ms)))
            if defer and res is None:
                return ["raw", raw, 2 if relu else 1, ms, None]
            if res is None:
                prog.append(Step("apply", (raw, out, 1 if relu else 0, None, ms, None, 0)))
            elif isinstance(res, list) and res[4] is None:
                prog.append(Step("apply", (raw, out, 2, res[1], ms, res[3], res[2])))
            else:
                prog.append(Step("apply", (raw, out, 2, materialise(res), ms, None, 0)))
            return out

        x = layer(img, e.conv1, "c1", True, defer=inorm and DEFER_NORM)
        for i, blk in enumerate(e.blocks):
            res = x if blk["stride"] == 1 else layer(x, blk["down"], f"b{i}_d", False, defer=inorm and DEFER_NORM)
            y = x
            for k, pc in enumerate(blk["convs"][:-1]):
                y = layer(y, pc, f"b{i}_{k}", True, defer=inorm)
            x = layer(y, blk["convs"][-1], f"b{i}_o", True, res=res)
        x = materialise(x)
        for pc, out, co_off, epi in outputs:
            prog.append(Step("conv", self._cp(x, pc, out, co_off=co_off, epi=epi)))
        return prog

    def _volume_program(self):
        sp = self.eng.spec
        prog = []
        alpha = 1.0 / math.sqrt(float(sp.fdim))
        x3 = self.prec_corr == "bf16x3"
        if self.otf and self.prec != "fp32" and PYRAMID_ONE_LAUNCH and sp.fdim % 32 == 0 and self.f2act[0].cs == sp.fdim and sp.levels <= 4:
            return [Step("pyramid", ops.PyramidArgs(self.f2act[:sp.levels], self.f2s[:sp.levels], 3 if x3 else 1))]
        for l in range(sp.levels):
            if l > 0:
                prog.append(Step("pool", (self.f2act[l - 1], self.f2act[l])))
            if self.otf:
                if self.prec != "fp32":
                    prog.append(Step("split", (self.f2act[l].t, self.f2s[l])))
                continue
            prog.append(Step("tile", (self.f2act[l], self.f2rows[l])))
            if self.prec == "fp32":
                prog.append(Step("conv", ops.corr_volume(self.f1, self.f2rows[l], self.vol[l].shape[1], self.vol[l], alpha)))
            else:
                prog.append(Step("split", (self.f2rows[l], self.f2s[l])))
                prog.append(Step("cgemm", (self.f1s, self.f2s[l], self.P, self.vol[l].shape[1], alpha, self.vol[l],
                                       3 if x3 else 1)))
        return prog

    def _iter_program(self, first):
        e, cp, sp = self.eng, self._cp, self.eng.spec
        hd = sp.hdim
        h_in = self.net0 if first else self.hB
        prog = [Step("lookup", self.lookup)]
        if sp.small:
            prog += [Step("conv", cp(self.corr, e.convc1, self.cf, co_off=0, epi=EPI.EPI_RELU)),
                     Step("conv", cp(self.flow4, e.convf1, self.fl1, epi=EPI.EPI_RELU)),
                     Step("conv", cp(self.fl1, e.convf2, self.cf, co_off=96, epi=EPI.EPI_RELU)),
                     Step("conv", cp(self.cf, e.convm, self.xbuf, co_off=sp.cdim, epi=EPI.EPI_RELU))]
        else:
            flo = [Step("conv", cp(self.flow4, e.convf1, self.fl1, epi=EPI.EPI_RELU), "convf1"),
                   Step("conv", cp(self.fl1, e.convf2, self.cf, co_off=192, epi=EPI.EPI_RELU), "convf2")]
            cor = [Step("conv", cp(self.corr, e.convc1, self.c1, epi=EPI.EPI_RELU), "convc1"),
                   Step("conv", cp(self.c1, e.convc2, self.cf, co_off=0, epi=EPI.EPI_RELU), "convc2")]
            if PAIR_BRANCHES:
                for c_, f_ in zip(cor, flo):
                    if ops.pair_ok(c_.arg, f_.arg):
                        prog.append(Step("conv2", (c_.arg, f_.arg), c_.tag + "+" + f_.tag))
                    else:
                        prog += [c_, f_]
            else:
                prog += cor + flo
            prog.append(Step("conv", cp(self.cf, e.convm, self.xbuf, co_off=sp.cdim, epi=EPI.EPI_RELU), "convm"))
        steps = len(e.zr_dyn)
        states = [h_in, self.hA, self.hB] if steps == 2 else [h_in, self.hB]
        if steps == 1 and not first:
            states = [self.hB, self.hA]
        for k in range(steps):
            hi, ho = states[k], states[k + 1]
            gz, gq = self.gate_bias[k]
            pzr = cp(hi, e.zr_dyn[k], self.zbuf, x2=self.xbuf, x2_off=sp.cdim, c_split=hd,
                     epi=EPI.EPI_GRU_ZR, split=hd, e0=hi, out1=self.rh, bias_map=gz)
            pq = cp(self.rh, e.q_dyn[k], ho, x2=self.xbuf, x2_off=sp.cdim, c_split=hd,
                    epi=EPI.EPI_GRU_Q, e0=hi, e1=self.zbuf, bias_map=gq)
            prog += [Step("conv", pzr, f"gru_zr{k}"), Step("conv", pq, f"gru_q{k}")]
        if steps == 1 and not first:
            prog.append(Step("copy", (self.hA.t, self.hB.t)))
        fused = None
        if e.fh2_frag is not None and e.fh2.cout == 2:
            if self.fh_part is None:
                self.fh_part = torch.zeros(4 * self.P, 20, dtype=torch.float32, device="cuda")
            fused = ops.flowhead_params(self.hB, e.fh1, self.fh_part, e.fh2_frag, precision=self.prec)
        if fused is not None:
            prog += [Step("conv", fused, "fh1"), Step("fh_gather", (fused._n_planes, e.fh2.bias[:2].contiguous()))]
            return prog
        prog.append(Step("conv", cp(self.hB, e.fh1, self.fh, epi=EPI.EPI_RELU), "fh1"))
        if ops.narrow_ok(self.fh, e.fh2):
            prog.append(Step("fh_update", (self.fh, e.fh2, self.delta)))
        else:
            prog += [Step("conv", cp(self.fh, e.fh2, self.delta)), Step("coords", None)]
        return prog

    def run(self, prog):
        ev = self.conv_events
        for kind, a, tag in prog:
            if kind == "conv":
                ops.run_conv(a) if ev is None else _timed(ev.get(tag), ops.run_conv, a)
            elif kind == "conv2":
                ops.run_conv_pair(*a) if ev is None else _timed(ev.get(tag), ops.run_conv_pair, *a)
            elif kind == "fin":
                rows, ld, c, c_pad, count, ms = a
                ops.inorm_finalize(self.stats, rows, ld, c, count, ms[0], ms[1], channels_pad=c_pad, ws=self.fin_ws)
            elif kind == "apply":
                raw, out, mode, res, ms, res_ms, res_mode = a
                ops.inorm_apply(raw, ms[0], ms[1], out, mode, res=res, res_stats=res_ms, res_mode=res_mode)
            elif kind == "pyramid":
                ops.feature_pyramid(a)
            elif kind == "pool":
                ops.avgpool2(a[0], a[1])
            elif kind == "split":
                self._split(a[0], a[1])
            elif kind == "tile":
                ops.tile_rows(a[0], a[1])
            elif kind == "cgemm":
                ops.corr_gemm_bf16(*a)
            elif kind == "lookup":
                self._lookup(a)
            elif kind == "copy":
                a[1].copy_(a[0])
            elif kind == "fh_gather":
                ops.flow_head_gather(self.fh_part, a[0], self.hf, self.wf, a[1], self.delta, self.coords, self.flow4.t,
                                     self.flow_cat, self.xbuf.cs)
            elif kind == "fh_update":
                ops.flow_head_update(a[0], a[1], a[2], self.coords, self.flow4.t, self.flow_cat, self.xbuf.cs)
            elif kind == "coords":
                ops.coords_update(self.coords, self.delta.t, self.delta.cs, self.wf, self.flow4.t, self.flow_cat, self.xbuf.cs)
            else:
                raise ValueError(kind)

    def _lookup(self, params):
        _timed(self.lookup_events, ops.run_lookup_otf if self.otf else ops.run_lookup, params)

    def _split(self, rows, out):
        if self.prec_corr == "bf16x3":
            ops.split_bf16_lines(rows, out)
        else:
            ops.split_bf16(rows, out, None)

    def load_image(self, slot, img_u8, pad_top, pad_left):
        ops.preprocess(img_u8, self.img[slot], self.hp, self.wp, pad_top, pad_left)

    def encode_source(self, reuse_target=False):
        reused = bool(reuse_target) and self.otf and self.target_valid
        if reused:
            self.f1rows[:self.P].copy_(self.f2act[0].t.view(self.P, -1))
            if self.prec != "fp32":
                self.f1s[:self.P].copy_(self.f2s[0])
        else:
            self.run(self.prog_f_src)
        self.run(self.prog_c_src)
        if self.prec != "fp32" and not reused:
            self._split(self.f1rows, self.f1s)
        self.inp_c.t.copy_(self.xbuf.t[:, :self.eng.spec.cdim])
        self.run(self.prog_gate_bias)
        return reused

    @property
    def record_dims(self):
        sp = self.eng.spec
        return sp.fdim, sp.hdim, sp.cdim

    def new_record(self):
        return torch.empty(ops.features_record_floats(self.P, *self.record_dims), dtype=torch.float32, device="cuda")

    def encode_record(self, record):
        self.source_tag, self.target_valid = None, False
        self.run(self.prog_f_src)
        self.run(self.prog_c_src)
        ops.features_pack(self.f1rows, self.net0.t, self.xbuf.t, self.P, self.record_dims, record)

    def restore_source(self, record):
        x3 = self.prec != "fp32" and self.prec_corr == "bf16x3"
        self.source_tag = None
        ops.features_unpack(record, self.P, self.record_dims, self.f1rows, self.f1s if x3 else None, self.net0.t, self.xbuf.t,
                            self.inp_c.t)
        if self.prec != "fp32" and not x3:
            self._split(self.f1rows, self.f1s)
        self.run(self.prog_gate_bias)

    def restore_target(self, record):
        self.target_valid = False
        ops.features_unpack(record, self.P, self.record_dims, self.f2act[0].t)

    def set_flow_init(self, flow_init):
        if tuple(flow_init.shape) != (2, self.hf, self.wf):
            raise ValueError(f"flow_init must have shape (2, {self.hf}, {self.wf}) for a {self.hp} x {self.wp} padded input, "
                             f"got {tuple(flow_init.shape)}")
        self.flow_init.copy_(flow_init, non_blocking=True)

    def flow_low(self):
        return self.flow4.t[:, :2].t().reshape(2, self.hf, self.wf).contiguous()

    def flow(self, iters, crop, h, w, flow_up=None, dst=None, wout=None, do_sigmoid=False, trace=None, defer_wh=False,
             mout=None, mask_sigmoid=False, flow_init=None, skip_wh=False, target_restored=False):
        e, sp = self.eng, self.eng.spec
        if iters < 1:
            raise ValueError("iters must be >= 1")
        if not target_restored:
            self.run(self.prog_f_dst)
        self.run(self.prog_volume)
        self.target_valid = True
        if flow_init is None:
            ops.coords_init(self.coords, self.hf, self.wf, self.flow4.t, self.flow_cat, self.xbuf.cs)
        else:
            if flow_init is not True:
                self.set_flow_init(flow_init)
            ops.coords_init_flow(self.coords, self.flow_init, self.hf, self.wf, self.flow4.t, self.flow_cat, self.xbuf.cs)
            if trace is not None:
                trace(self, -1)
        folded = self.folded is not None and trace is None
        region = self.flow_region if (trace is None and flow_init is None) else None
        if region is not None and region["key"][1] != iters:
            region = None
        for it in range(iters):
            prog = self._iteration(it, iters, folded)
            self.run(prog if region is None else region["iters"].get(it, prog))
            if trace is not None:
                trace(self, it)
        if folded:
            self.run(self.folded.gather)
        for p in self.prog_mask[1 if iters > 1 and self.prog_iter_last is not None else 0:]:
            ops.run_conv(p)
        if defer_wh:
            assert e.weighted and not sp.small and self.wh_region is not None and not e.mask_head
            self._upsample(None, crop, h, w, flow_up=flow_up, dst=dst, wout=None, do_sigmoid=do_sigmoid)
            return
        if skip_wh:
            self._upsample(None, crop, h, w, flow_up=flow_up, dst=dst, wout=None, do_sigmoid=do_sigmoid)
            return
        if e.weighted:
            self._weight_head(self.wh_region[1] if self.wh_region is not None else self.prog_wh,
                              self.wh_region[0] if self.wh_region is not None else None)
        wout = wout if e.weighted else None
        self._upsample(self.wlow, crop, h, w, flow_up=flow_up, dst=dst, wout=wout, do_sigmoid=do_sigmoid)
        if e.mask_head:
            self._mask_head()
            if mout is not None:
                self._upsample(self.mh_low, crop, h, w, wout=mout, do_sigmoid=mask_sigmoid)

    def _upsample(self, wlow, crop, h, w, **outputs):
        if self.eng.spec.small:
            ops.upflow8(self.coords, wlow, self.hf, self.wf, crop, h, w, **outputs)
        else:
            ops.convex_upsample(self.coords, wlow, self.mask.t, self.hf, self.wf, crop, h, w, **outputs)

    def _mask_head(self):
        e = self.eng
        ops.warp_features(self.f2act[0], self.coords, self.mh_warped)
        for p in self.prog_mh:
            ops.run_conv(p)
        ops.wh_reduce(self.mh_last, 1, self.mh_w, e.mh_b, self.P, self.mh_low)

    def finish_weights(self, pts, count, n_max, pad, crop, h, w, flow_up=None, dst=None, wout=None, do_sigmoid=False,
                       w_points=None):
        index, _ = self.wh_region[:2]
        key = index.data_ptr()
        if key not in self._wh_dyn:
            dyn = torch.full_like(index, -1)
            prog, fused = self._wh_program(int(index.numel()), dyn)
            assert fused
            self._wh_dyn[key] = (dyn, prog, torch.zeros(self.P, dtype=torch.int32, device=index.device),
                                 torch.zeros(1, dtype=torch.int32, device=index.device))
        dyn, prog, bitmap, n_needed = self._wh_dyn[key]
        ops.wh_needed(pts, count, n_max, pad[0], pad[1], self.hf, self.wf, index, bitmap, dyn, n_needed)
        self._weight_head(prog, dyn, n_needed, need=bitmap)
        if w_points is not None:
            ops.convex_weights_at(pts, count, n_max, self.wlow, self.mask.t, self.hf, self.wf, crop, w_points,
                                  do_sigmoid=do_sigmoid)
            return
        self._upsample(self.wlow, crop, h, w, flow_up=flow_up, dst=dst, wout=wout, do_sigmoid=do_sigmoid)

    def _wh6_padded(self, cs):
        if self._wh6_pad is None or self._wh6_pad.numel() != cs:
            self._wh6_pad = torch.zeros(cs, dtype=torch.float32, device="cuda")
            self._wh6_pad[:self.eng.wh6_c] = self.eng.wh6_w[:self.eng.wh6_c]
        return self._wh6_pad

    def _weight_head(self, prog_wh, index, n_needed=None, need=None):
        e, sp = self.eng, self.eng.spec
        if self.otf:
            self.lookup.need = _lib.ptr(need)
        self._lookup(self.lookup)
        if self.otf:
            self.lookup.need = None
        n = sp.nwin
        ops.colsum(self.f2act[0].t, self.P, sp.fdim, self.cs_ws, self.cs_tot)
        ops.wh_pack(self.corr, self.f1, self.cs_tot, 1.0 / (math.sqrt(float(sp.fdim)) * self.P), n, self.wmean,
                    None if self.wh0_direct else self.x8)
        if self.x32 is not None:
            self.x32.t[:, :8].copy_(self.x8.t)
        n_win = int(index.numel()) if index is not None else self.P
        if index is not None:
            self.wlow.zero_()
        if self.wh0_direct and not self.wh0_fused:
            ops.wh_conv0(self.corr, self.wmean, n_win, n, self.wh0_t, e.wh0.bias, self.a1, index)
        _timed(self.wh_events, ops.run_conv, prog_wh[0], extra=lambda: n_win if n_needed is None else n_needed.clone())
        for p in prog_wh[1:]:
            ops.run_conv(p)
        if not self.wh_fused:
            last = self.a1 if e.wh_std else self.wh_last
            ops.wh_reduce(last, n * n, self._wh6_padded(last.cs), e.wh6_b, self.P, self.wlow)

    def _wh_train_buffers(self, n_max):
        cap = 9 * n_max
        t = self._wh_train
        if t is None or t["cap"] < cap:
            z, P = self._z, self.P
            i32 = lambda *s: torch.zeros(*s, dtype=torch.int32, device="cuda")
            t = dict(cap=cap, x8=z(cap, 81, 8), act=[z(cap, 81, 128) for _ in range(3)], g=[z(cap, 81, 128) for _ in range(2)],
                     out=z(cap), wlow=z(P), g_wlow=z(P), bitmap=i32(P), dyn=i32(P),
                     all=torch.arange(P, dtype=torch.int32, device="cuda"),
                     ws=z(ops.wh_wgrad_ws_floats(cap, 128)), ws64=z(-(-cap // ops.WH_TRAIN_CHUNK) * 129, dtype=torch.float64),
                     gen=0 if t is None else t["gen"])
            self._wh_train = t
        return t

    def wh_train_forward(self, params, pts, count, n_max, pad, crop, do_sigmoid=False):
        sp, n = self.eng.spec, self.eng.spec.nwin
        assert self.eng.weighted and self.eng.wh_std and not sp.small and n == 9 and 0 < n_max <= ops.HFIT_SINGLE_MAX
        t = self._wh_train_buffers(n_max)
        t["gen"] += 1
        w0, b0, w2, b2, w4, b4, w6, b6 = (p.detach() for p in params)
        wsel = torch.zeros(n_max, dtype=torch.float32, device="cuda")
        ops.wh_needed(pts, count, n_max, pad[0], pad[1], self.hf, self.wf, t["all"], t["bitmap"], t["dyn"])
        index = t["dyn"][t["dyn"] >= 0].contiguous()
        n_win = int(index.numel())
        if n_win == 0:
            return wsel, None
        if self.otf:
            self.lookup.need = _lib.ptr(t["bitmap"])
        self._lookup(self.lookup)
        if self.otf:
            self.lookup.need = None
        ops.colsum(self.f2act[0].t, self.P, sp.fdim, self.cs_ws, self.cs_tot)
        ops.wh_pack(self.corr, self.f1, self.cs_tot, 1.0 / (math.sqrt(float(sp.fdim)) * self.P), n, self.wmean, None)
        li = index.long()
        x8 = t["x8"][:n_win]
        x8[:, :, :4] = self.corr.t[li, :4 * n * n].view(n_win, n * n, 4)
        x8[:, :, 4] = self.wmean[li][:, None]
        wh_train.head_forward(x8, n_win, (w0, b0, w2, b2, w4, b4, w6), t["act"], t["out"])
        t["wlow"].zero_()
        t["wlow"][li] = t["out"][:n_win] + b6.reshape(())
        ops.convex_weights_at(pts, count, n_max, t["wlow"], self.mask.t, self.hf, self.wf, crop, wsel, do_sigmoid=do_sigmoid)
        return wsel, dict(gen=t["gen"], index=index, n_win=n_win, pts=pts, count=count, n_max=n_max, crop=crop,
                          do_sigmoid=bool(do_sigmoid), w2=w2.clone(), w4=w4.clone(), w6=w6.reshape(-1).clone())

    def wh_train_backward(self, state, g_wsel):
        z = lambda *s: torch.zeros(*s, dtype=torch.float32, device="cuda")
        gw0, gb0, gw2, gb2, gw4, gb4, gw6, gb6 = z(128, 5, 3, 3), z(128), z(128, 128, 3, 3), z(128), z(128, 128, 3, 3), z(128), \
            z(1, 128, 1, 1), z(1)
        grads = (gw0, gb0, gw2, gb2, gw4, gb4, gw6, gb6)
        if state is None:
            return grads
        t = self._wh_train
        if t is None or t["gen"] != state["gen"]:
            raise RuntimeError("weights_at(): backward after a later flow or weights_at() in the same flow plan -- the activations "
                               "and the upsampling mask it reads are gone")
        n_win, index = state["n_win"], state["index"]
        ops.convex_weights_at_bwd(state["pts"], state["count"], state["n_max"], g_wsel, t["wlow"], self.mask.t, self.hf, self.wf,
                                  state["crop"], t["g_wlow"], index=index, do_sigmoid=state["do_sigmoid"])
        wh_train.head_backward(t["x8"], n_win, (state["w2"], state["w4"], state["w6"]), t["act"], t["g_wlow"], index, t["g"],
                               t["ws"], t["ws64"], grads)
        return grads
```

woft_amd/flow_provider.py:

```python
import logging
import os
from collections import OrderedDict
from pathlib import Path
from timeit import default_timer as timer

import numpy as np
import torch

from . import _lib, ops, wh_train
from .engine import RaftEngine

logger = logging.getLogger(__name__)


def _pad_geometry(h, w, mode):
    if mode == "nopad":
        assert h % 8 == 0
        assert w % 8 == 0
        return h, w, 0, 0, h, w, h, w
    if mode == "crop":
        ch, cw = (h // 8) * 8, (w // 8) * 8
        return ch, cw, 0, 0, ch, cw, ch, cw
    if mode == "RAFT":
        ph = (((h // 8) + 1) * 8 - h) % 8
        pw = (((w // 8) + 1) * 8 - w) % 8
        return h + ph, w + pw, ph // 2, pw // 2, h, w, h, w
    if mode == "Michal":
        raise NotImplementedError("padding_mode 'Michal' (raft.py:250-271) fails in the reference itself for "
                                  "raft_type 'orig'/'weighted'; it is not provided on the HIP path")
    raise ValueError(f"invalid padding_mode '{mode}'")


def _mask_head_shapes(structure, fdim):
    try:
        layers = [tuple(d) if isinstance(d, (list, tuple)) else (d, 3) for d in structure]
        shapes, cur = [], 2 * fdim
        for c, k in layers:
            c, k = int(c), int(k)
            if c < 1 or k < 1 or k % 2 == 0:
                raise ValueError
            shapes.append((c, cur, k, k))
            cur = c
    except (TypeError, ValueError):
        raise ValueError(f"class_params.mask_head_structure {structure!r}: not a list of (channels, odd kernel) tuples "
                         "or channel counts (weighted_raft.py:387-409)") from None
    return shapes + [(1, cur, 1, 1)]


class FrameFeatures:

    def __init__(self, provider, record, geometry, size):
        self.provider, self.record = provider, record
        self.geometry, self.size = tuple(int(v) for v in geometry), tuple(int(v) for v in size)

    @property
    def shape(self):
        return self.size + (3,)

    @property
    def nbytes(self):
        return self.record.numel() * self.record.element_size()

    def __repr__(self):
        return f"FrameFeatures({self.size[0]} x {self.size[1]}, padded geometry {self.geometry}, {self.nbytes} bytes)"


class _Recent:

    def __init__(self):
        self.order, self.protected = OrderedDict(), None

    def touch(self, key, keep, protect=False):
        if protect:
            self.protected = key
        self.order[key] = None
        self.order.move_to_end(key)
        others = [k for k in self.order if k != self.protected]
        dropped = others[:max(0, len(others) - keep)]
        for k in dropped:
            del self.order[k]
        return dropped


class RAFTWrapper:
    def __init__(self, config):
        self.C = config
        cp = config.class_params
        if self.C.raft_type not in ("orig", "weighted", "weighted_masked"):
            raise ValueError(f"Unknown RAFT type {self.C.raft_type}")
        self.masked = self.C.raft_type == "weighted_masked"
        if self.masked and not cp.mask_estimation:
            raise ValueError("raft_type 'weighted_masked' needs class_params.mask_estimation = True (and mask_head_structure): "
                             "without the MaskHead the network has no mask output")
        if self.C.raft_type == "weighted" and cp.mask_estimation:
            raise ValueError("class_params.mask_estimation is set with raft_type 'weighted', which returns no mask: use raft_type "
                             "'weighted_masked'")
        self._cache_mask_warned = False
        logger.info(f"Loading weights from: {self.C.model}")

        def read(src):
            sd = src if isinstance(src, dict) else torch.load(src, map_location="cpu")
            return {(k[len("module."):] if k.startswith("module.") else k): v for k, v in sd.items()}
        state_dict = read(self.C.model)
        if self.C.backbone_model:
            in_backbone = lambda k: ("fnet" in k) or ("cnet" in k) or ("update_block" in k)
            state_dict = {k: v for k, v in state_dict.items() if not in_backbone(k)}
            state_dict.update({k: v for k, v in read(self.C.backbone_model).items() if in_backbone(k)})
        weighted = self.C.raft_type in ("weighted", "weighted_masked")
        small = bool(cp.small)
        if self.masked:
            if not cp.mask_head_structure:
                raise ValueError("raft_type 'weighted_masked' needs class_params.mask_head_structure (weighted_raft.py:387-409)")
            want = _mask_head_shapes(cp.mask_head_structure, 128 if small else 256)
            idx = sorted(int(k.split(".")[2]) for k in state_dict if k.startswith("mask_head.net.") and k.endswith(".weight"))
            got = [tuple(state_dict[f"mask_head.net.{i}.weight"].shape) for i in idx]
            if got != want or idx != list(range(0, 2 * len(want), 2)):
                raise ValueError(f"class_params.mask_head_structure {cp.mask_head_structure!r} expects mask_head.net layers {want}; "
                                 f"the checkpoint has {got} (at net.{idx})")
        for src, val in (("env WOFT_PRECISION", os.environ.get("WOFT_PRECISION")),
                         ("flow config key 'precision'", self.C.precision),
                         ("class_params.mixed_precision", "fp16" if cp.mixed_precision else None),
                         ("built-in default (no key in the flow config): fp32-emulating bf16x3 -- finer than the TF32 convolutions "
                          "the reference's torch 1.8.1 runs by default on Ampere; 'fp32' = exact products", "bf16x3")):
            if val:
                self.precision, self.precision_source = str(val), src
                break
        note = (f"RAFT arithmetic: precision = '{self.precision}' (from: {self.precision_source}). "
                + ("This is the reference's arithmetic (exact IEEE fp32 products)." if self.precision == "fp32" else
                   "NOT the reference's IEEE-fp32 products: set precision = 'fp32' in the flow config (or WOFT_PRECISION=fp32) "
                   "for the reference's arithmetic (about 4x slower)."))
        logger.log(logging.WARNING if self.precision_source.startswith("built-in default") else logging.INFO, note)
        self.precision_note = note
        self.corr = os.environ.get("WOFT_CORR") or getattr(self.C, "corr", None) or "otf"
        self.engine = RaftEngine(state_dict, small=small, weighted=weighted, precision=self.precision, corr=self.corr,
                                 volume_storage=getattr(self.C, "volume_storage", None), mask_head=self.masked)
        self._wh_loaded = {k: v for k, v in state_dict.items() if k.startswith("weight_head.net.")}
        self._wh_params, self._wh_flow = None, None
        v = getattr(self.C, "flow_region", None)
        self.flow_region_on = (os.environ.get("WOFT_FLOW_REGION", "1") != "0") if (v is None or isinstance(v, type(self.C))) else bool(v)
        self.use_graph = (os.environ.get("WOFT_GRAPH") or str(int(bool(getattr(self.C, "graph", False))))) == "1"
        self._pinned = None
        self._pinned_key = None
        self._wmask, self._wregion, self._all_pixels = None, {}, {}
        self._fmask, self._fregion = None, {}
        self.weights_deferred, self._deferred = False, None
        self.defer_min_ratio = 6
        self._out = {}
        self._cache_errors = set()
        self._last_dst = {}
        self.source_features_reused = False
        self._plan_bound = None
        self._recent_plans, self._recent_outs, self._recent_pixels = _Recent(), _Recent(), _Recent()

    def bound_plans(self, n_other):
        self._plan_bound = None if n_other is None else max(1, int(n_other))

    def _touch_plan(self, plan_key, out_key, n_pix, pinned_here):
        n = self._plan_bound
        if n is None:
            return
        for key in self._recent_plans.touch(plan_key, n, protect=pinned_here):
            plan = self.engine.drop_plan(key)
            self._last_dst.pop(id(plan), None)
        for key in self._recent_outs.touch(out_key, n, protect=pinned_here):
            self._out.pop(key, None)
        for key in self._recent_pixels.touch(n_pix, n, protect=pinned_here):
            self._all_pixels.pop(key, None)

    def _run_flow(self, plan, iters, crop, oh, ow, o, weighted, do_sigmoid, defer_wh=False, want_flow=True, mask_sigmoid=False,
                  has_init=False, skip_wh=False, target_restored=False):
        self._wh_flow = (plan, crop)
        if plan._wh_train is not None:
            plan._wh_train["gen"] += 1

        def eager():
            plan.flow(iters, crop, oh, ow, flow_up=o["flow"] if want_flow else None, dst=o["dst"], wout=o["w"] if weighted else None,
                      do_sigmoid=do_sigmoid, defer_wh=defer_wh, mout=o.get("m"), mask_sigmoid=mask_sigmoid,
                      flow_init=True if has_init else None, skip_wh=skip_wh, target_restored=target_restored)
        if not self.use_graph or plan.lookup_events is not None or plan.wh_events is not None or plan.conv_events is not None:
            return eager()
        region = plan.wh_region
        fregion = plan.flow_region if not has_init else None
        key = (iters, crop, oh, ow, weighted, do_sigmoid, want_flow, bool(defer_wh), o["flow"].data_ptr(),
               region[0].data_ptr() if region is not None else 0, bool(mask_sigmoid), bool(has_init),
               fregion["key"] if fregion is not None else None, bool(skip_wh), bool(target_restored))
        g = plan._graphs.get(key)
        if g is None:
            eager()
            if key in plan._graphs:
                g = torch.cuda.CUDAGraph()
                with torch.cuda.graph(g):
                    eager()
            plan._graphs[key] = g
        else:
            g.replay()

    def finish_weights(self, pts, count, n_max, out=None):
        plan, crop, oh, ow, o, do_sigmoid = self._deferred
        self._deferred = None
        plan.finish_weights(pts, count, n_max, crop, crop, oh, ow, flow_up=o["flow"], dst=o["dst"], wout=o["w"],
                            do_sigmoid=do_sigmoid, w_points=out)
        return o["w"] if out is None else out

    def _wh_trainable(self):
        eng = self.engine
        why = (f"raft_type '{self.C.raft_type}' (only 'weighted' is covered)" if self.C.raft_type != "weighted" else
               "the small model (its head reads 7x7 windows of another lookup)" if eng.small else
               "a weight_head_structure other than [(128, 3), (128, 3), (128, 3)]" if not eng.wh_std else
               "a weights_postprocessing_fn between the head and the weights" if self.C.weights_postprocessing_fn else None)
        if why:
            raise NotImplementedError(f"training of the weight head is not provided for {why}")

    def weight_head_parameters(self):
        self._wh_trainable()
        if self._wh_params is None:
            self._wh_params = wh_train.make_parameters(self._wh_loaded)
        return self._wh_params

    def weights_at(self, pts, count=None, do_sigmoid=False):
        self._wh_trainable()
        if self._wh_flow is None:
            raise RuntimeError("weights_at(): no computed flow to evaluate the head on (none yet, or the last one came from the "
                               "flow cache)")
        if not (isinstance(pts, torch.Tensor) and pts.is_cuda and pts.dtype == torch.float32 and pts.dim() == 2
                and pts.shape[1] == 2 and pts.shape[0] >= 1):
            raise TypeError("weights_at(): pts must be a (n_max, 2) float32 device tensor of (x, y) pixels")
        if pts.shape[0] > ops.HFIT_SINGLE_MAX:
            raise ValueError(f"weights_at(): at most {ops.HFIT_SINGLE_MAX} points per call, got {pts.shape[0]}")
        if count is not None and not (isinstance(count, torch.Tensor) and count.is_cuda and count.dtype == torch.int32
                                      and count.numel() == 1):
            raise TypeError("weights_at(): count must be a device int32 scalar")
        plan, crop = self._wh_flow
        params = self.weight_head_parameters().values()
        return wh_train.weights_at(plan, params, pts.detach().contiguous(), count, int(pts.shape[0]), crop, do_sigmoid)

    def sync_weight_head(self):
        self.engine.repack_weight_head({k: v.detach() for k, v in self.weight_head_parameters().items()})

    def pin_source(self, src_img):
        self._pinned = src_img
        self._pinned_key = None
        self._wmask, self._wregion = None, {}
        self._fmask, self._fregion = None, {}

    def pin_flow_region(self, mask):
        self._fmask = None if mask is None else np.ascontiguousarray(np.asarray(mask) > 0)
        self._fregion = {}

    def _flow_region(self, key, hp, wp, top, left, oh, ow):
        if self._fmask is None:
            return None
        if key not in self._fregion:
            ys, xs = np.nonzero(self._fmask[:oh, :ow])
            rect = None
            if ys.size:
                y0, y1, x0, x1 = (ys.min() + top) >> 3, (ys.max() + top) >> 3, (xs.min() + left) >> 3, (xs.max() + left) >> 3
                rect = (int(y0), int(x0), int(y1 - y0 + 1), int(x1 - x0 + 1))
            self._fregion[key] = rect
        return self._fregion[key]

    def pin_weight_region(self, mask):
        self._wmask = None if mask is None else np.ascontiguousarray(np.asarray(mask) > 0)
        self._wregion = {}

    def _weight_region(self, key, hp, wp, top, left, oh, ow):
        if self._wmask is None:
            return None
        if key not in self._wregion:
            m = self._wmask[:oh, :ow]
            coarse = np.zeros((hp // 8, wp // 8), bool)
            ys, xs = np.nonzero(m)
            coarse[(ys + top) >> 3, (xs + left) >> 3] = True
            pad = np.pad(coarse, 1)
            dil = np.zeros_like(coarse)
            for dy in range(3):
                for dx in range(3):
                    dil |= pad[dy:dy + coarse.shape[0], dx:dx + coarse.shape[1]]
            idx = np.flatnonzero(dil).astype(np.int32)
            self._wregion[key] = torch.from_numpy(idx).cuda() if idx.size and idx.size < dil.size else None
        return self._wregion[key]

    def postprocess_weights(self, flat_weights, fn):
        s = self.last_flow_shape
        weights = fn(flat_weights.reshape(s["batch"], 1, s["H"], s["W"]))
        return weights.reshape(s["batch"], s["H"] * s["W"])

    def _outputs(self, h, w):
        key = (h, w)
        if key not in self._out:
            z = lambda *s: torch.empty(*s, dtype=torch.float32, device="cuda")
            self._out[key] = dict(flow=z(2, h, w), dst=z(2, h * w), w=z(1, h * w),
                                  src=torch.stack([torch.arange(h * w, device="cuda") % w,
                                                   torch.div(torch.arange(h * w, device="cuda"), w, rounding_mode="floor")]))
            if self.masked:
                self._out[key]["m"] = z(1, h * w)
        return self._out[key]

    def _cached_flow(self, src_img, identifier, mode, numpy_out, do_sigmoid, borrow=False):
        dataset_name, seq_name, frame_i = identifier
        self._wh_flow = None
        path = Path(self.C.flow_cache_dir) / dataset_name / seq_name / f"{frame_i}-{frame_i + 1}.npz"
        data = np.load(path, allow_pickle=False)
        flow = np.ascontiguousarray(data["half_flow"].astype(np.float32))
        wts = data["half_weights"].astype(np.float32)
        wts = np.ascontiguousarray(wts) if wts.size > 1 else None
        h, w = flow.shape[1:]
        post = self.C.weights_postprocessing_fn if wts is not None else None
        o = self._outputs(h, w)
        o["flow"].copy_(torch.from_numpy(flow), non_blocking=True)
        wl = None
        if wts is not None:
            wl = torch.from_numpy(wts).cuda(non_blocking=True)
        lib = _lib.load()
        _lib.check(lib.woft_flow_to_tc(_lib.ptr(o["flow"]), _lib.ptr(wl), h, w, _lib.ptr(o["dst"]),
                                       _lib.ptr(o["w"]) if wl is not None else None, int(bool(do_sigmoid) and not post),
                                       _lib.stream_ptr()), "woft_flow_to_tc")
        if post:
            self._postprocess_logits(o, h, w, do_sigmoid)
        return self._deliver(o, o["w"] if wl is not None else None, mode, h, w, numpy_out, borrow)

    def _postprocess_logits(self, o, h, w, do_sigmoid):
        wts = self.C.weights_postprocessing_fn(o["w"].reshape(1, 1, h, w))
        wts = torch.as_tensor(wts, device=o["w"].device, dtype=torch.float32).reshape(1, h * w)
        o["w"].copy_(torch.sigmoid(wts) if do_sigmoid else wts)

    def _deliver(self, o, weights, mode, oh, ow, numpy_out, borrow):
        own = (lambda t: t) if borrow else (lambda t: t.clone())
        host = lambda t: t.cpu().numpy()
        conv = host if numpy_out else own
        extra = ()
        if mode == "flow":
            wts = weights.reshape(1, oh, ow) if weights is not None else None
            if self.masked:
                extra = (conv(o["m"].reshape(1, oh, ow)),)
            return (conv(o["flow"]), (conv(wts) if wts is not None else None)) + extra
        self.last_flow_shape = {"batch": 1, "delta": 2, "H": oh, "W": ow}
        if self.masked:
            extra = (conv(o["m"]),)
        if numpy_out:
            return (host(o["src"]), host(o["dst"]), (host(weights) if weights is not None else None)) + extra
        return (own(o["src"]), own(o["dst"]), (own(weights) if weights is not None else None)) + extra

    @staticmethod
    def _as_flow_init(flow_init, hp, wp):
        want = (2, hp // 8, wp // 8)
        t = flow_init if isinstance(flow_init, torch.Tensor) else torch.from_numpy(np.ascontiguousarray(flow_init))
        if t.dim() == 4 and t.shape[0] == 1:
            t = t[0]
        if tuple(t.shape) != want or not t.is_floating_point():
            raise ValueError(f"flow_init must be a float array of shape {want} or {(1,) + want} (1/8-resolution pixels of the "
                             f"{hp} x {wp} padded image), got {tuple(flow_init.shape)} {flow_init.dtype}")
        return t.detach().to(torch.float32)

    def flow_key(self, src_img):
        hp, wp, top, left = _pad_geometry(src_img.shape[0], src_img.shape[1], self.C.padding_mode)[:4]
        return (0 if (src_img is self._pinned or self._pinned is None) else 1, hp, wp, top, left)

    def flow_low(self, copy=True):
        plan = getattr(self, "_low_plan", None)
        if plan is None:
            raise RuntimeError("flow_low(): no flow has been computed yet")
        return plan.flow_low() if copy else plan.flow4.t[:, :2].t().reshape(2, plan.hf, plan.wf)

    def flow_map(self):
        m = getattr(self, "_flow_map", None)
        if m is None:
            raise RuntimeError("flow_map(): the last flow wrote no flow map (mode 'TC' without keep_flow, or no flow yet)")
        return m

    def _upload(self, a, H, W, lh, lw, what="compute_flow"):
        if isinstance(a, torch.Tensor):
            t = a if a.is_cuda else a.cuda(non_blocking=True)
        else:
            t = torch.from_numpy(np.ascontiguousarray(a)).cuda(non_blocking=True)
        if t.dtype != torch.uint8 or t.dim() != 3 or t.shape[2] != 3:
            raise TypeError(f"{what} takes (H, W, 3) uint8 BGR images, got {tuple(t.shape)} {t.dtype}")
        if (lh, lw) != (H, W):
            t = t[:lh, :lw].contiguous()
        return t.contiguous()

    def _operand_geometry(self, a):
        if isinstance(a, FrameFeatures):
            return a.geometry + a.size
        h, w = int(a.shape[0]), int(a.shape[1])
        return tuple(_pad_geometry(h, w, self.C.padding_mode)[:4]) + (h, w)

    def encode_frame(self, img):
        H, W = img.shape[:2]
        hp, wp, top, left, oh, ow, lh, lw = _pad_geometry(H, W, self.C.padding_mode)
        slot = 0 if self._pinned is None else 1
        plan = self.engine.plan(hp, wp, slot)
        self._touch_plan((hp, wp) if slot == 0 else (hp, wp, slot), (oh, ow), plan.P, False)
        plan.load_image(0, self._upload(img, H, W, lh, lw, "encode_frame"), top, left)
        self._last_dst.pop(id(plan), None)
        if slot == 0:
            self._pinned_key = None
        record = plan.new_record()
        plan.encode_record(record)
        return FrameFeatures(self, record, (hp, wp, top, left), (H, W))

    def compute_flow_fb(self, src_img, dst_img, alpha=0.01, beta=0.5, numpy_out=False, share_features=False):
        alpha, beta = float(alpha), float(beta)
        if not (0.0 <= alpha < float("inf")) or not (0.0 <= beta < float("inf")):
            raise ValueError(f"compute_flow_fb: alpha and beta must be finite and >= 0, got {alpha!r}, {beta!r}")
        if share_features:
            src_img, dst_img = (a if isinstance(a, FrameFeatures) else self.encode_frame(a) for a in (src_img, dst_img))
        fwd = self.compute_flow(src_img, dst_img, mode="flow", skip_weights=True)[0]
        bwd = self.compute_flow(dst_img, src_img, mode="flow", skip_weights=True)[0]
        err, ok = ops.flow_fb(fwd, bwd, alpha, beta)
        out = (fwd, bwd, err[None], ok[None])
        return tuple(t.cpu().numpy() for t in out) if numpy_out else out

    def compute_flow(self, src_img, dst_img, mode="TC", vis=False, src_img_identifier=None,
                     numpy_out=False, do_sigmoid=False, borrow=False, defer_weights=False, weight_region=False,
                     src_is_previous_dst=False, visibility=False, flow_init=None, iters=None, flow_region=False,
                     keep_flow=False, skip_weights=False):
        if visibility and not self.masked:
            raise ValueError("compute_flow(visibility=True) needs raft_type 'weighted_masked': no other type has a mask output")
        assert mode in ["flow", "TC"]
        src_rec = src_img if isinstance(src_img, FrameFeatures) else None
        dst_rec = dst_img if isinstance(dst_img, FrameFeatures) else None
        if src_rec is not None or dst_rec is not None:
            for rec in (src_rec, dst_rec):
                if rec is not None and rec.provider is not self:
                    raise ValueError("compute_flow: a FrameFeatures record of another provider (its encoders made other features)")
            if src_img_identifier is not None:
                raise ValueError("compute_flow: src_img_identifier (the flow cache) cannot be combined with a FrameFeatures record")
            gs, gd = self._operand_geometry(src_img), self._operand_geometry(dst_img)
            if gs != gd:
                raise ValueError(f"compute_flow: the operands have different padded geometries (hp, wp, top, left, H, W): src {gs}, "
                                 f"dst {gd} -- a FrameFeatures record serves only the geometry it was encoded at")
        assert src_img.shape == dst_img.shape
        self._flow_map = None
        if src_img_identifier is not None and self.masked:
            if not self._cache_mask_warned:
                self._cache_mask_warned = True
                logger.warning("raft_type 'weighted_masked': the flow cache holds no visibility mask -- cached flows are not used, "
                               "every flow is computed")
        elif src_img_identifier is not None:
            try:
                return self._cached_flow(src_img, src_img_identifier, mode, numpy_out, do_sigmoid, borrow)
            except Exception as ex:
                key = (type(ex), str(ex))
                if key not in self._cache_errors:
                    self._cache_errors.add(key)
                    logger.warning(f"no cached flow: {ex}")
        H, W = src_img.shape[:2]
        hp, wp, top, left, oh, ow, lh, lw = _pad_geometry(H, W, self.C.padding_mode)
        pinned_here = src_img is self._pinned
        slot = 0 if (pinned_here or self._pinned is None) else 1
        plan = self.engine.plan(hp, wp, slot)
        if flow_init is not None:
            flow_init = self._as_flow_init(flow_init, hp, wp)
        n_iters = int(self.C.iters) if iters is None else int(iters)
        if n_iters < 1:
            raise ValueError("iters must be >= 1")
        self._touch_plan((hp, wp) if slot == 0 else (hp, wp, slot), (oh, ow), plan.P, pinned_here)
        start_time = timer()

        up = lambda a: self._upload(a, H, W, lh, lw)
        key = (hp, wp, top, left)
        if pinned_here and self._pinned_key == key and plan.source_tag is self:
            pass
        elif src_rec is not None:
            plan.restore_source(src_rec.record)
            self.source_features_reused = False
            if slot == 0:
                self._pinned_key = None
        else:
            s = up(src_img)
            plan.load_image(0, s, top, left)
            reuse = bool(src_is_previous_dst) and self._last_dst.get(id(plan)) == (id(src_img), key)
            self.source_features_reused = bool(plan.encode_source(reuse_target=reuse))
            plan.source_tag = self if pinned_here else None
            if pinned_here:
                self._pinned_key = key
        post = self.C.weights_postprocessing_fn or None
        region = None
        if weight_region and not post:
            if pinned_here:
                region = self._weight_region(key, hp, wp, top, left, oh, ow)
            if region is None and defer_weights:
                if plan.P not in self._all_pixels:
                    self._all_pixels[plan.P] = torch.arange(plan.P, dtype=torch.int32, device="cuda")
                region = self._all_pixels[plan.P]
        plan.set_weight_region(region)
        frect = None
        if flow_region and self.flow_region_on and pinned_here and not post and flow_init is None and not self.masked:
            frect = self._flow_region(key, hp, wp, top, left, oh, ow)
        plan.set_flow_region(frect, n_iters)
        if dst_rec is not None:
            plan.restore_target(dst_rec.record)
            self._last_dst.pop(id(plan), None)
        else:
            d = up(dst_img)
            plan.load_image(1, d, top, left)
            self._last_dst[id(plan)] = (id(dst_img), key)
        o = self._outputs(oh, ow)
# ... 22 lines not shown
```

woft_amd/ops.py:

```python
import ctypes as C
import math
import os
from dataclasses import dataclass

import numpy as np
import torch

from . import _lib, conv_select
from ._lib import ConvParams, LookupOtfParams, LookupParams, check, ptr, stream_ptr
from .conv_select import KERNELS, PRECISION, Kernel, pair_ok

DEV = "cuda"


def _round_up(x, m):
    return (x + m - 1) // m * m


@dataclass
class Act:
    t: torch.Tensor
    n: int
    h: int
    w: int
    c: int

    @property
    def cs(self):
        return self.t.shape[1]

    @property
    def n_pix(self):
        return self.n * self.h * self.w

    def nchw(self):
        return self.t[:, :self.c].reshape(self.n, self.h, self.w, self.c).permute(0, 3, 1, 2).contiguous()


def _rows(n_pix, cs, zero):
    return (torch.zeros if zero else torch.empty)(n_pix, cs, dtype=torch.float32, device=DEV)


def act_from_nchw(x, cs=None):
    n, c, h, w = x.shape
    cs = cs or _round_up(c, 4)
    t = _rows(n * h * w, cs, True)
    t[:, :c] = x.to(DEV).permute(0, 2, 3, 1).reshape(n * h * w, c)
    return Act(t, n, h, w, c)


def new_act(n, h, w, c, cs=None, zero=False):
    cs = cs or _round_up(c, 4)
    return Act(_rows(n * h * w, cs, zero), n, h, w, c)


@dataclass
class PackedConv:
    wgt: torch.Tensor
    bias: torch.Tensor
    cout: int
    cout_pad: int
    cin_pad: int
    taps_y: int
    taps_x: int
    pad_y: int
    pad_x: int
    stride: int
    flat: int
    flat_cs: int = 0
    kh: int = 0
    kw: int = 0
    wgt_hi: torch.Tensor = None
    wgt_lo: torch.Tensor = None
    _frag: dict = None
    _f16: torch.Tensor = None

    def wgt_f16(self):
        if self._f16 is None:
            w = self.wgt.detach().cpu()
            if float(w.abs().max()) >= 65504.0:
                raise ValueError("precision 'fp16': a weight exceeds the fp16 range")
            self._f16 = w.to(torch.float16).view(torch.bfloat16).to(self.wgt.device)
        return self._f16

    def frag(self, planes, f16=False):
        if self._frag is None:
            self._frag = {}
        key = "f16" if f16 else planes
        if key not in self._frag:
            taps, nchunk = self.taps_y * self.taps_x, self.cin_pad // 32
            w = self.wgt.detach().cpu().reshape(self.cout_pad // 32, 32, taps, nchunk, 2, 2, 8)
            w = w.permute(0, 3, 2, 4, 5, 1, 6).contiguous()
            if f16:
                pl = [w.to(torch.float16).view(torch.bfloat16)]
            else:
                hi = w.to(torch.bfloat16)
                pl = [hi] + ([(w - hi.float()).to(torch.bfloat16)] if planes == 2 else [])
            self._frag[key] = torch.stack(pl, dim=3).contiguous().to(self.wgt.device)
        return self._frag[key]

    def frag_mx(self):
        if self._frag is None:
            self._frag = {}
        if "mx" not in self._frag:
            taps, nchunk = self.taps_y * self.taps_x, self.cin_pad // 32
            npair = (taps + 1) // 2
            w = self.wgt.detach().cpu().reshape(self.cout_pad, taps, nchunk, 32)
            if float(w.abs().max()) >= 65504.0:
                raise ValueError("precision 'f16mx8': a weight exceeds the fp16 range")
            lw = w - w.to(torch.float16).float()
            bands = self.cout_pad // 32
            out = torch.zeros(bands, nchunk, npair, 2, 64 * 32 + 64 * 4, dtype=torch.uint8)
            for t, x in enumerate((w, lw)):
                amax = x.abs().amax(dim=3)
                e = torch.floor(torch.log2(torch.clamp(amax, min=1e-38)))
                sc = torch.where(amax > 0, e - 7 + 127, torch.full_like(e, 127.0)).clamp(0, 254)
                q = (x / torch.exp2(sc - 127)[..., None]).to(torch.float8_e4m3fn).view(torch.uint8)
                if taps % 2:
                    q = torch.cat([q, torch.zeros_like(q[:, :1])], 1)
                    sc = torch.cat([sc, torch.full_like(sc[:, :1], 127.0)], 1)
                q = q.reshape(bands, 32, npair, 2, nchunk, 2, 16)
                data = q.permute(0, 4, 2, 5, 1, 3, 6).reshape(bands, nchunk, npair, 64 * 32)
                scl = sc.reshape(bands, 32, npair, 2, nchunk).permute(0, 4, 2, 3, 1).reshape(bands, nchunk, npair, 64)
                scl4 = torch.zeros(bands, nchunk, npair, 64, 4, dtype=torch.uint8)
                scl4[..., 0] = scl.to(torch.uint8)
                out[:, :, :, t, :64 * 32] = data
                out[:, :, :, t, 64 * 32:] = scl4.reshape(bands, nchunk, npair, 256)
            self._frag["mx"] = out.contiguous().to(self.wgt.device)
        return self._frag["mx"]

    def __post_init__(self):
        if self.wgt is not None and self.wgt_hi is None and self.wgt.dtype == torch.float32:
            w = self.wgt.detach().cpu()
            hi = w.to(torch.bfloat16)
            self.wgt_hi = hi.to(self.wgt.device)
            self.wgt_lo = (w - hi.float()).to(torch.bfloat16).to(self.wgt.device)

    def out_hw(self, h, w):
        kh, kw = (self.kh or self.taps_y), (self.kw or self.taps_x)
        return (h + 2 * self.pad_y - kh) // self.stride + 1, (w + 2 * self.pad_x - kw) // self.stride + 1


def pack_conv(weight, bias, stride=1, padding=None, cin_layout=None, flat_cs=0, scale=1.0):
    weight = weight.detach().float().cpu() * scale
    cout, cin, kh, kw = weight.shape
    if padding is None:
        padding = (kh // 2, kw // 2)
    if isinstance(padding, int):
        padding = (padding, padding)
    cout_pad = _round_up(cout, 64)
    if cout_pad > 64:
        cout_pad = _round_up(cout, 128)
    b = torch.zeros(cout_pad)
    if bias is not None:
        b[:cout] = bias.detach().float().cpu() * scale
    if flat_cs:
        assert kw * flat_cs <= 32 and cin <= flat_cs
        wp = torch.zeros(cout_pad, kh, 32)
        for kx in range(kw):
            wp[:cout, :, kx * flat_cs:kx * flat_cs + cin] = weight[:, :, :, kx].permute(0, 2, 1)
        return PackedConv(wp.reshape(cout_pad, kh * 32).contiguous().to(DEV), b.to(DEV), cout, cout_pad, 32,
                          kh, 1, padding[0], padding[1], stride, 1, flat_cs, kh, kw)
    if cin_layout is None:
        cin_layout = [(0, cin, 0)]
    cin_pad = _round_up(max(d + (e - s) for s, e, d in cin_layout), 32)
    wp = torch.zeros(cout_pad, kh * kw, cin_pad)
    wt = weight.permute(0, 2, 3, 1).reshape(cout, kh * kw, cin)
    for s, e, d in cin_layout:
        wp[:cout, :, d:d + (e - s)] = wt[:, :, s:e]
    return PackedConv(wp.reshape(cout_pad, kh * kw * cin_pad).contiguous().to(DEV), b.to(DEV), cout, cout_pad,
                      cin_pad, kh, kw, padding[0], padding[1], stride, 0, 0, kh, kw)


def repack_conv_(pc, new):
    assert pc.wgt.shape == new.wgt.shape and pc.bias.shape == new.bias.shape
    pc.wgt.copy_(new.wgt)
    pc.bias.copy_(new.bias)
    pc.wgt_hi.copy_(new.wgt_hi)
    pc.wgt_lo.copy_(new.wgt_lo)
    for key, t in (pc._frag or {}).items():
        t.copy_(new.frag_mx() if key == "mx" else new.frag(1, f16=True) if key == "f16" else new.frag(key))
    if pc._f16 is not None:
        pc._f16.copy_(new.wgt_f16())


def fold_bn(weight, bias, bn_w, bn_b, mean, var, eps=1e-5):
    s = (bn_w.double() / torch.sqrt(var.double() + eps))
    w = (weight.double() * s[:, None, None, None]).float()
    b = ((bias.double() - mean.double()) * s + bn_b.double()).float()
    return w, b


MX_LAYERS = os.environ.get("WOFT_MX_LAYERS", "auto")
SLOW_GATES = os.environ.get("WOFT_SLOW_GATES", "0") != "0"
USE_HALO = os.environ.get("WOFT_HALO", "1") != "0"
USE_REGB = os.environ.get("WOFT_REGB", "1") != "0"
REGB_TY4 = os.environ.get("WOFT_REGB_TY4", "1") != "0"
USE_STEM = os.environ.get("WOFT_STEM", "1") != "0"
USE_1X1 = os.environ.get("WOFT_1X1", "1") != "0"
HALO_MIN_BLOCKS = int(os.environ.get("WOFT_HALO_MIN_BLOCKS", "400"))
WH_HALO = int(os.environ.get("WOFT_WH_HALO", "2"))
TILE_MIN_BLOCKS = int(os.environ.get("WOFT_TILE_MIN_BLOCKS", "400"))
assert conv_select.EPI_FLOWHEAD == _lib.EPI_FLOWHEAD


def _switches():
    return conv_select.Switches(USE_HALO, USE_REGB, REGB_TY4, USE_STEM, USE_1X1, WH_HALO, HALO_MIN_BLOCKS, TILE_MIN_BLOCKS,
                                MX_LAYERS, os.environ.get("WOFT_MX_ZR", "12"))


def select_conv(x, pc, epi=_lib.EPI_LINEAR, x2=None, stats=None, ho=None, wo=None, tiles=None, cout=None, precision=0, halo=None,
                in_norm=0, bias_map=None, wh0=None, **_):
    if ho is None or wo is None:
        ho, wo = pc.out_hw(x.h, x.w)
    layer = conv_select.Layer(x.n, x.h, x.w, ho, wo, pc.taps_y, pc.taps_x, pc.stride, pc.pad_y, pc.pad_x, pc.cin_pad,
                              cout or pc.cout, pc.cout_pad, pc.flat, x.cs, x2 is not None, stats is not None, int(in_norm or 0),
                              bias_map is not None, wh0 is not None, epi)
    return conv_select.select(layer, PRECISION.get(precision, precision), _switches(), tiles, halo)


def conv_params(x, pc, out, co_off=0, epi=_lib.EPI_LINEAR, x2=None, c_split=0, e0=None, e1=None, out1=None,
                split=0, alpha=1.0, stats=None, ho=None, wo=None, tiles=None, cout=None, precision=0, halo=None,
                in_norm=0, in_stats=None, bias_map=None, x2_off=0, wh0=None):
    if ho is None or wo is None:
        ho, wo = pc.out_hw(x.h, x.w)
    sel = select_conv(x, pc, epi=epi, x2=x2, stats=stats, ho=ho, wo=wo, tiles=tiles, cout=cout, precision=precision, halo=halo,
                      in_norm=in_norm, bias_map=bias_map, wh0=wh0)
    p = ConvParams()
    p.in0, p.cs0 = ptr(x.t), x.cs
    if x2 is not None:
        p.in1, p.cs1, p.c_split = x2.t.data_ptr() + 4 * x2_off, x2.cs, c_split
    else:
        p.in1, p.cs1, p.c_split = None, 0, pc.cin_pad
    p.n_img, p.h, p.w, p.ho, p.wo = x.n, x.h, x.w, ho, wo
    p.taps_y, p.taps_x, p.stride, p.pad_y, p.pad_x = pc.taps_y, pc.taps_x, pc.stride, pc.pad_y, pc.pad_x
    p.cin_pad, p.flat = pc.cin_pad, pc.flat
    p.wgt, p.bias, p.alpha = ptr(pc.wgt), ptr(pc.bias), alpha
    p.wgt_hi, p.wgt_lo, p.precision = ptr(pc.wgt_hi), ptr(pc.wgt_lo), sel.precision
    if PRECISION.get(precision, precision) == conv_select.FP16:
        p.wgt_hi, p.wgt_lo = ptr(pc.wgt_f16()), None
    p.wgt_frag = p.wgt_mx = None
    if KERNELS[sel.kernel].weights == conv_select.FRAG:
        p.wgt_frag = ptr(pc.frag(2 if sel.precision == conv_select.BF16X3 else 1,
                                 f16=sel.precision in (conv_select.FP16, conv_select.F16MX8)))
        if sel.precision == conv_select.F16MX8:
            p.wgt_mx = ptr(pc.frag_mx())
    p.cout, p.cout_pad = (cout or pc.cout), sel.cout_pad
    p.out, p.ldo, p.co_off = ptr(out.t), out.cs, co_off
    p.out_w, p.out_pitch = (-12346 if SLOW_GATES else 0), 0
    p.epi, p.split = epi, split
    p.e0, p.lde0 = (ptr(e0.t), e0.cs) if e0 is not None else (None, 0)
    p.e1, p.lde1 = (ptr(e1.t), e1.cs) if e1 is not None else (None, 0)
    p.out1, p.ldo1 = (ptr(out1.t), out1.cs) if out1 is not None else (None, 0)
    p.tile_m, p.tile_n, p.halo = sel.tile_m, sel.tile_n, sel.kernel
    p.bias_map, p.ld_bias_map = (ptr(bias_map.t), bias_map.cs) if bias_map is not None else (None, 0)
    p.in_norm, p.in_mean, p.in_rstd = (sel.in_norm, ptr(in_stats[0]), ptr(in_stats[1])) if sel.in_norm else (0, None, None)
    if stats is not None:
        assert stats[0].numel() >= 2 * sel.m_tiles * pc.cout_pad
        p.stat_sum, p.stat_sq = ptr(stats[0]), ptr(stats[1])
    else:
        p.stat_sum, p.stat_sq = None, None
    if wh0 is not None:
        lk, mean, frag, b0, index = wh0
        p.wh0_lookup, p.wh0_ld, p.wh0_mean = ptr(lk.t), lk.cs, ptr(mean)
        p.wh0_w, p.wh0_bias, p.wh0_index = ptr(frag), ptr(b0), (ptr(index) if index is not None else None)
    p._keep = (x, x2, pc, out, e0, e1, out1, stats, in_stats, bias_map, wh0, p.wgt_frag and pc._frag)
    p._m, p._m_tiles = x.n * ho * wo, sel.m_tiles
    return p


def pack_wh0_frags(w0, planes):
    k = torch.zeros(128, 48)
    k[:, :45] = w0.detach().float().cpu().permute(0, 2, 3, 1).reshape(128, 45)
    k = k.reshape(4, 32, 3, 2, 8).permute(0, 2, 3, 1, 4).reshape(4, 3, 64, 8)
    hi = k.to(torch.bfloat16)
    pl = [hi] + ([(k - hi.float()).to(torch.bfloat16)] if planes == 2 else [])
    return torch.stack(pl, dim=2).contiguous().to(DEV)


def pack_flowhead_frags(w2, planes, f16=False):
    w2 = w2.detach().float().cpu()
    c = w2.shape[1]
    assert w2.shape[0] == 2 and tuple(w2.shape[2:]) == (3, 3) and c % 32 == 0
    cols = torch.zeros(32, c)
    cols[:18] = w2.permute(2, 3, 0, 1).reshape(18, c)
    f = cols.reshape(32, c // 32, 2, 2, 8).permute(1, 2, 3, 0, 4).reshape(c // 32, 2, 64, 8)
    if f16:
        return f.to(torch.float16).view(torch.bfloat16).reshape(c // 32, 2, 1, 64, 8).contiguous().to(DEV)
    hi = f.to(torch.bfloat16)
    pl = [hi] + ([(f - hi.float()).to(torch.bfloat16)] if planes == 2 else [])
    return torch.stack(pl, dim=2).contiguous().to(DEV)


def flowhead_params(x, pc, part, frags, **kw):
    p = conv_params(x, pc, Act(part, 1, x.h, x.w, 18), epi=_lib.EPI_FLOWHEAD, **kw)
    if Kernel(p.halo) is not Kernel.REGB_8X16 or pc.cout % 32 != 0:
        return None
    n_planes = p.cout_pad // p.tile_n
    assert part.shape[0] >= n_planes * x.n_pix and part.shape[1] >= 20 and x.n == 1
    p.e0, p.lde0 = ptr(frags), 0
    p._keep = p._keep + (part, frags)
    p._n_planes = n_planes
    return p


def flow_head_gather(part, n_planes, h, w, bias2, delta, coords, flow4=None, flow_cat=None, ld_cat=0):
    check(_lib.load().woft_flow_head_gather(ptr(part), n_planes, part.shape[1], h, w, ptr(bias2), ptr(delta.t), delta.cs,
                                            ptr(coords), ptr(flow4), ptr(flow_cat), ld_cat, stream_ptr()),
          "woft_flow_head_gather")


def run_conv_pair(a, b):
    check(_lib.load().woft_conv2d_pair(C.byref(a), C.byref(b), stream_ptr()), "woft_conv2d_pair")


def run_conv(p):
    check(_lib.load().woft_conv2d(C.byref(p), stream_ptr()), "woft_conv2d")


def conv2d(x, pc, c_out_stride=None, **kw):
    ho, wo = pc.out_hw(x.h, x.w)
    out = kw.pop("out", None) or new_act(x.n, ho, wo, pc.cout, cs=c_out_stride or _round_up(pc.cout, 4), zero=True)
    p = conv_params(x, pc, out, ho=ho, wo=wo, **kw)
    run_conv(p)
    return out


def inorm_ws(device="cuda"):
    return torch.zeros(int(_lib.load().woft_inorm_ws_bytes()), dtype=torch.uint8, device=device)


def inorm_finalize(stats, n_part, ld, channels, count, mean, rstd, eps=1e-5, channels_pad=None, ws=None):
    check(_lib.load().woft_inorm_finalize(ptr(stats[0]), ptr(stats[1]), n_part, ld, channels, channels_pad or channels,
                                          count, eps, ptr(mean), ptr(rstd), ptr(ws), stream_ptr()), "woft_inorm_finalize")


def inorm_apply(x, mean, rstd, out, mode, res=None, res_stats=None, res_mode=0):
    assert out.cs == x.cs and (res is None or res.cs == x.cs)
    rm, rr = res_stats if res_stats is not None else (None, None)
    check(_lib.load().woft_inorm_apply(ptr(x.t), ptr(mean), ptr(rstd), ptr(res.t) if res is not None else None,
                                       ptr(rm), ptr(rr), res_mode, ptr(out.t), x.n_pix, x.cs, mode, stream_ptr()),
          "woft_inorm_apply")


class PyramidArgs:
    def __init__(self, maps, splits, terms):
        import ctypes
        self.maps, self.splits, self.terms = maps, splits, terms
        self.levels = len(maps)
        assert 1 <= self.levels <= 4 and len(splits) == self.levels and all(m.cs == maps[0].cs == m.c for m in maps)
        for l in range(1, self.levels):
            assert (maps[l].h, maps[l].w) == (maps[l - 1].h // 2, maps[l - 1].w // 2)
        self.pooled = (ctypes.c_void_p * 3)(*[maps[l].t.data_ptr() if l < self.levels else None for l in range(1, 4)])
        self.split = (ctypes.c_void_p * 4)(*[splits[l].data_ptr() if l < self.levels else None for l in range(4)])


def feature_pyramid(a):
    m = a.maps[0]
    check(_lib.load().woft_feature_pyramid(ptr(m.t), m.h, m.w, m.cs, a.levels, a.pooled, a.split, a.terms, stream_ptr()),
          "woft_feature_pyramid")


def preprocess(img_u8, out, hp, wp, pad_top, pad_left):
    h, w = img_u8.shape[:2]
    check(_lib.load().woft_preprocess_bgr_u8(ptr(img_u8), h, w, ptr(out.t), hp, wp, pad_top, pad_left, stream_ptr()),
          "woft_preprocess_bgr_u8")


def avgpool2(x, out):
    check(_lib.load().woft_avgpool2_nhwc(ptr(x.t), x.h, x.w, x.cs, ptr(out.t), stream_ptr()), "woft_avgpool2_nhwc")


def split_bf16(x, hi, lo=None):
    check(_lib.load().woft_split_bf16(ptr(x), x.numel(), ptr(hi), ptr(lo), stream_ptr()), "woft_split_bf16")


def conv3x3_narrow(x, pc, out, co_off=0):
    assert (pc.taps_y, pc.taps_x, pc.stride, pc.pad_y, pc.pad_x, pc.flat) == (3, 3, 1, 1, 1, 0) and pc.cout <= 2
    assert out.n == x.n and out.h == x.h and out.w == x.w
    check(_lib.load().woft_conv3x3_narrow(ptr(x.t), x.cs, x.n, x.h, x.w, pc.cin_pad, ptr(pc.wgt), ptr(pc.bias), pc.cout,
                                          ptr(out.t), out.cs, co_off, stream_ptr()), "woft_conv3x3_narrow")


def flow_head_update(x, pc, delta, coords, flow4=None, flow_cat=None, ld_cat=0):
    assert narrow_ok(x, pc) and pc.cout == 2 and x.n == 1 and coords.shape[0] == x.h * x.w
    check(_lib.load().woft_flow_head_update(ptr(x.t), x.cs, x.h, x.w, pc.cin_pad, ptr(pc.wgt), ptr(pc.bias), ptr(delta.t),
                                            delta.cs, ptr(coords), ptr(flow4), ptr(flow_cat), ld_cat, stream_ptr()),
          "woft_flow_head_update")


def narrow_ok(x, pc):
    return ((pc.taps_y, pc.taps_x, pc.stride, pc.pad_y, pc.pad_x, pc.flat) == (3, 3, 1, 1, 1, 0) and pc.cout <= 2
            and pc.cin_pad in (128, 256) and x.cs >= pc.cin_pad)


def make_lookup_otf_params(f1s, f2s, dims, hf, wf, k, coords, out, radius, terms):
    p = LookupOtfParams()
    p.f1 = ptr(f1s)
    for l, (t, (h, w)) in enumerate(zip(f2s, dims)):
        p.f2[l], p.h[l], p.w[l] = ptr(t), h, w
    p.levels, p.radius, p.terms = len(f2s), radius, terms
    p.hf, p.wf, p.k = hf, wf, k
    p.alpha = 1.0 / math.sqrt(float(k))
    p.coords, p.out, p.ldo = ptr(coords), ptr(out), out.shape[1]
    p._keep = (f1s, f2s, coords, out)
    return p


def run_lookup_otf(p):
    check(_lib.load().woft_corr_lookup_otf(C.byref(p), stream_ptr()), "woft_corr_lookup_otf")


def split_bf16_lines(x, out):
    check(_lib.load().woft_split_bf16_lines(ptr(x), x.numel(), ptr(out), stream_ptr()), "woft_split_bf16_lines")


def features_record_floats(n_pix, fdim, hdim, cdim):
    return n_pix * (fdim + hdim + cdim)


def features_pack(f1rows, net, xbuf, n_pix, dims, record):
    fdim, hdim, cdim = dims
    assert record.dtype == torch.float32 and record.is_contiguous() and record.numel() == features_record_floats(n_pix, *dims)
    assert f1rows.shape[0] >= n_pix and net.shape[0] >= n_pix and xbuf.shape[0] >= n_pix
    check(_lib.load().woft_features_pack(ptr(f1rows), f1rows.stride(0), ptr(net), net.stride(0), ptr(xbuf), xbuf.stride(0),
                                         n_pix, fdim, hdim, cdim, ptr(record), stream_ptr()), "woft_features_pack")


def features_unpack(record, n_pix, dims, fmap, fmap_split=None, net=None, xbuf=None, inp_c=None):
    fdim, hdim, cdim = dims
    assert record.dtype == torch.float32 and record.is_contiguous() and record.numel() == features_record_floats(n_pix, *dims)
    assert fmap.shape[0] >= n_pix and all(t is None or t.shape[0] >= n_pix for t in (fmap_split, net, xbuf, inp_c))
    ld = lambda t: 0 if t is None else t.stride(0)
    check(_lib.load().woft_features_unpack(ptr(record), n_pix, fdim, hdim, cdim, ptr(fmap), ld(fmap), ptr(fmap_split), ptr(net),
                                           ld(net), ptr(xbuf), ld(xbuf), ptr(inp_c), ld(inp_c), stream_ptr()),
          "woft_features_unpack")


def corr_gemm_bf16(a, b, m, n, alpha, out, terms):
    k = a.shape[1] // 2 if terms == 3 else a.shape[1]
    assert out.dtype in (torch.float32, torch.bfloat16)
    check(_lib.load().woft_corr_gemm_bf16(ptr(a), ptr(b), m, n, a.shape[0], b.shape[0], k, float(alpha), ptr(out),
                                          out.shape[1], terms, int(out.dtype == torch.bfloat16), stream_ptr()),
          "woft_corr_gemm_bf16")


def corr_volume(f1, f2_rows, n_q, out, alpha, precision=0, f2_hi=None, f2_lo=None):
    p = ConvParams()
    p.in0, p.cs0, p.in1, p.cs1, p.c_split = ptr(f1.t), f1.cs, None, 0, f1.cs
    p.n_img, p.h, p.w, p.ho, p.wo = 1, f1.h, f1.w, f1.h, f1.w
    p.taps_y = p.taps_x = p.stride = 1
    p.pad_y = p.pad_x = 0
    p.cin_pad, p.flat = f1.cs, 0
    p.wgt, p.bias, p.alpha = ptr(f2_rows), None, alpha
    p.wgt_hi, p.wgt_lo, p.precision = ptr(f2_hi), ptr(f2_lo), PRECISION.get(precision, precision)
    p.cout, p.cout_pad = n_q, f2_rows.shape[0]
    p.out, p.ldo, p.co_off = ptr(out), out.shape[1], 0
    p.out_w, p.out_pitch = 0, 0
    p.epi = _lib.EPI_LINEAR
    p.tile_m, p.tile_n = (128, 128) if f2_rows.shape[0] % 128 == 0 else (128, 64)
    p.halo = Kernel.GATHER
    p._keep = (f1, f2_rows, out, f2_hi, f2_lo)
    return p


def tiled_dims(h, w, tw=4):
    ht, wt = (h + 3) // 4, (w + tw - 1) // tw
    return ht, wt, ht * wt * 4 * tw


def tile_rows(x, out):
    check(_lib.load().woft_tile_rows(ptr(x.t), x.h, x.w, x.cs, ptr(out), stream_ptr()), "woft_tile_rows")


def tile_planes(planes, tw=4):
    P, h, w = planes.shape
    ht, wt, n = tiled_dims(h, w, tw)
    pad = torch.zeros(P, ht * 4, wt * tw, dtype=planes.dtype, device=planes.device)
    pad[:, :h, :w] = planes
    return pad.reshape(P, ht, 4, wt, tw).permute(0, 1, 3, 2, 4).reshape(P, n).contiguous()


def untile_planes(vol, h, w, tw=4):
    ht, wt, n = tiled_dims(h, w, tw)
    P = vol.shape[0]
    return vol[:, :n].reshape(P, ht, wt, 4, tw).permute(0, 1, 3, 2, 4).reshape(P, ht * 4, wt * tw)[:, :h, :w]


def make_lookup_params(vols, dims, coords, out, radius):
    p = LookupParams()
    assert len({v.dtype for v in vols}) == 1 and vols[0].dtype in (torch.float32, torch.bfloat16)
    p.vol_bf16 = int(vols[0].dtype == torch.bfloat16)
    for l, v in enumerate(vols):
        p.vol[l] = ptr(v)
        p.ht[l], p.wt[l], n = tiled_dims(*dims[l])
        assert v.shape[1] >= n
        p.plane[l] = v.shape[1]
    p.levels, p.radius = len(vols), radius
    p.coords, p.n_pix, p.out, p.ldo = ptr(coords), coords.shape[0], ptr(out), out.shape[1]
    p._keep = (vols, coords, out)
    return p


def run_lookup(p):
    check(_lib.load().woft_corr_lookup(C.byref(p), stream_ptr()), "woft_corr_lookup")


def coords_init(coords, hf, wf, flow4=None, flow_cat=None, ld_cat=0):
    check(_lib.load().woft_coords_init(ptr(coords), hf, wf, ptr(flow4), ptr(flow_cat), ld_cat, stream_ptr()),
          "woft_coords_init")


def coords_init_flow(coords, flow_init, hf, wf, flow4=None, flow_cat=None, ld_cat=0):
    assert flow_init.dtype == torch.float32 and flow_init.is_contiguous() and tuple(flow_init.shape) == (2, hf, wf)
    check(_lib.load().woft_coords_init_flow(ptr(coords), ptr(flow_init), hf, wf, ptr(flow4), ptr(flow_cat), ld_cat,
                                            stream_ptr()), "woft_coords_init_flow")


def forward_interpolate(flow, out=None):
    assert flow.dtype == torch.float32 and flow.is_contiguous() and flow.dim() == 3 and flow.shape[0] == 2
    if out is None:
        out = torch.empty_like(flow)
    assert out.dtype == torch.float32 and out.is_contiguous() and out.shape == flow.shape
    check(_lib.load().woft_forward_interpolate(ptr(flow), flow.shape[1], flow.shape[2], ptr(out), stream_ptr()),
          "woft_forward_interpolate")
    return out


def _f32c(t, *shape):
    return t.dtype == torch.float32 and t.is_contiguous() and t.is_cuda and (not shape or tuple(t.shape) == shape)


def sample_bilinear(data, x, y, out=None):
    assert data.dim() == 3 and _f32c(data) and x.dim() == 1 and _f32c(x) and _f32c(y, *x.shape)
    c, h, w = data.shape
    n = x.shape[0]
    if out is None:
        out = torch.empty((c, n), dtype=torch.float32, device=data.device)
    assert _f32c(out, c, n)
    check(_lib.load().woft_sample_bilinear(ptr(data), c, h, w, ptr(x), ptr(y), n, ptr(out), stream_ptr()), "woft_sample_bilinear")
    return out


def flow_chain(flow_ab, flow_bc, out=None):
    assert flow_ab.dim() == 3 and flow_ab.shape[0] == 2 and _f32c(flow_ab) and _f32c(flow_bc, *flow_ab.shape)
    if out is None:
        out = torch.empty_like(flow_ab)
    assert _f32c(out, *flow_ab.shape) and out.data_ptr() != flow_bc.data_ptr()
    check(_lib.load().woft_flow_chain(ptr(flow_ab), ptr(flow_bc), flow_ab.shape[1], flow_ab.shape[2], ptr(out), stream_ptr()),
          "woft_flow_chain")
    return out


def flow_fb(flow_ab, flow_ba, alpha=0.01, beta=0.5, err=None, ok=None, want_err=True, want_ok=True):
    assert flow_ab.dim() == 3 and flow_ab.shape[0] == 2 and _f32c(flow_ab) and _f32c(flow_ba, *flow_ab.shape)
    h, w = flow_ab.shape[1:]
    if err is None and want_err:
        err = torch.empty((h, w), dtype=torch.float32, device=flow_ab.device)
    if ok is None and want_ok:
        ok = torch.empty((h, w), dtype=torch.float32, device=flow_ab.device)
    assert (err is None or (_f32c(err) and err.numel() == h * w)) and (ok is None or (_f32c(ok) and ok.numel() == h * w))
    check(_lib.load().woft_flow_fb(ptr(flow_ab), ptr(flow_ba), h, w, float(alpha), float(beta), ptr(err), ptr(ok), stream_ptr()),
          "woft_flow_fb")
    return err, ok


def flow_chain_fold(best, prev, step_flow, step_wlogit=None, step_mlogit=None, k=0, vis_thr=0.5, unit_cost=1.0, first=False):
    assert step_flow.dim() == 3 and step_flow.shape[0] == 2 and _f32c(step_flow)
    h, w = step_flow.shape[1:]
    n = h * w
    plane = lambda t: t is None or (_f32c(t) and t.numel() == n)
    assert plane(step_wlogit) and plane(step_mlogit)
    if prev is not None:
        assert len(prev) == 3 and _f32c(prev[0], 2, h, w) and _f32c(prev[1]) and prev[1].numel() == n and plane(prev[2]) \
            and prev[2] is not None
    k, vis_thr, unit_cost = int(k), float(vis_thr), float(unit_cost)
    if not 0 <= k <= 127:
        raise ValueError(f"flow_chain_fold: k must be in [0, 127], got {k}")
    if not (0.0 <= vis_thr <= 1.0) or not (unit_cost >= 0.0):
        raise ValueError(f"flow_chain_fold: vis_thr must be in [0, 1] and unit_cost >= 0, got {vis_thr!r}, {unit_cost!r}")
    if best is None:
        assert first, "flow_chain_fold: without a running best the fold must be the first"
        new = lambda dtype: torch.empty((h, w), dtype=dtype, device=step_flow.device)
        best = (torch.empty_like(step_flow), new(torch.float32), new(torch.float32), new(torch.int32))
    bf, bc, bv, bs = best
    assert _f32c(bf, 2, h, w) and plane(bc) and plane(bv) and bc is not None and bv is not None
    assert bs.dtype == torch.int32 and bs.is_contiguous() and bs.is_cuda and bs.numel() == n
    pf, pc, pv = prev if prev is not None else (None, None, None)
    check(_lib.load().woft_flow_chain_fold(ptr(pf), ptr(pc), ptr(pv), ptr(step_flow), ptr(step_wlogit), ptr(step_mlogit), h, w,
                                           unit_cost, vis_thr, k, int(bool(first)), ptr(bf), ptr(bc), ptr(bv), ptr(bs),
                                           stream_ptr()), "woft_flow_chain_fold")
    return best


CHAIN_HIST = 130


def chain_tc(flow, cost, vis, sel, tmask_u8, vis_thr, want_w=True, mask_hw=None, out=None):
    assert flow.dim() == 3 and flow.shape[0] == 2 and _f32c(flow)
    h, w = flow.shape[1:]
    n = h * w
    assert all(_f32c(t) and t.numel() == n for t in (cost, vis))
    assert sel.dtype == torch.int32 and sel.is_contiguous() and sel.is_cuda and sel.numel() == n
    vis_thr = float(vis_thr)
    if not (0.0 <= vis_thr <= 1.0):
        raise ValueError(f"chain_tc: vis_thr must be in [0, 1], got {vis_thr!r}")
    mh, mw = mask_hw or (h, w)
    if tmask_u8 is not None:
        assert tmask_u8.dtype == torch.uint8 and tmask_u8.is_contiguous() and tmask_u8.is_cuda and tmask_u8.numel() == mh * mw
    if out is None:
        new = lambda *s: torch.empty(s, dtype=torch.float32, device=flow.device)
        out = (new(2, n), new(1, n) if want_w else None, new(1, n), torch.empty(CHAIN_HIST, dtype=torch.int32, device=flow.device))
    dst, wout, ok, hist = out
    if not want_w:
        wout = None
    assert _f32c(dst, 2, n) and _f32c(ok, 1, n) and (wout is None or _f32c(wout, 1, n))
    assert hist is None or (hist.dtype == torch.int32 and hist.is_contiguous() and hist.is_cuda and hist.numel() == CHAIN_HIST)
    check(_lib.load().woft_chain_tc(ptr(flow), ptr(cost), ptr(vis), ptr(sel), ptr(tmask_u8), h, w, mh, mw, vis_thr, ptr(dst),
                                    ptr(wout), ptr(ok), ptr(hist), stream_ptr()), "woft_chain_tc")
    return dst, wout, ok, hist


def coords_update(coords, delta, ld_delta, wf, flow4=None, flow_cat=None, ld_cat=0):
    check(_lib.load().woft_coords_update(ptr(coords), ptr(delta), ld_delta, wf, coords.shape[0], ptr(flow4),
                                         ptr(flow_cat), ld_cat, stream_ptr()), "woft_coords_update")


def wh_needed(pts, count, n_max, top, left, hf, wf, index, bitmap, dyn_index, n_needed=None):
    check(_lib.load().woft_wh_needed(ptr(pts), ptr(count), n_max, top, left, hf, wf, ptr(index), index.numel(), ptr(bitmap),
                                     ptr(dyn_index), ptr(n_needed), stream_ptr()), "woft_wh_needed")


def colsum(f, n_pix, c, ws, total):
    check(_lib.load().woft_colsum(ptr(f), n_pix, c, ptr(ws), ws.shape[0], ptr(total), stream_ptr()), "woft_colsum")


def wh_pack(lookup, f1, f2_total, alpha, nwin, mean, x8=None):
    check(_lib.load().woft_wh_pack(ptr(lookup.t), lookup.cs, ptr(f1.t), f1.c, ptr(f2_total), alpha, f1.n_pix, nwin, ptr(mean),
                                   ptr(x8.t) if x8 is not None else None, stream_ptr()), "woft_wh_pack")


def wh_conv0(lookup, mean, n_win, nwin, wt, bias, out, index=None):
    check(_lib.load().woft_wh_conv0(ptr(lookup.t), lookup.cs, ptr(mean), n_win, nwin, ptr(wt), ptr(bias), ptr(out.t), ptr(index),
                                    stream_ptr()), "woft_wh_conv0")


def wh_reduce(act, nwin2, w, bias, n_pix, out):
    check(_lib.load().woft_wh_reduce(ptr(act.t), act.cs, nwin2, ptr(w), bias, n_pix, ptr(out), stream_ptr()), "woft_wh_reduce")


def copy_params(p):
    q = type(p).from_buffer_copy(p)
    q.__dict__.update(p.__dict__)
    return q


def warp_features(f, coords, out):
    check(_lib.load().woft_warp_features(ptr(f.t), f.h, f.w, f.c, f.cs, ptr(coords), out.n_pix, ptr(out.t), out.cs,
                                         stream_ptr()), "woft_warp_features")


def convex_upsample(coords, wlow, mask, hf, wf, crop, h, w, flow_up=None, dst=None, wout=None, do_sigmoid=False):
    check(_lib.load().woft_convex_upsample(ptr(coords), ptr(wlow), ptr(mask), mask.shape[1], hf, wf, crop[0], crop[1],
                                           h, w, ptr(flow_up), ptr(dst), ptr(wout), int(do_sigmoid), stream_ptr()),
          "woft_convex_upsample")


def convex_weights_at(pts, count, n_max, wlow, mask, hf, wf, crop, wsel, do_sigmoid=False):
    check(_lib.load().woft_convex_weights_at(ptr(pts), ptr(count), n_max, ptr(wlow), ptr(mask), mask.shape[1], hf, wf,
                                             crop[0], crop[1], int(do_sigmoid), ptr(wsel), stream_ptr()),
          "woft_convex_weights_at")


WH_TRAIN_CHUNK = 16
WH_TRAIN_MAX_WIN = 9 * 2048


def convex_weights_at_bwd(pts, count, n_max, g_wsel, wlow, mask, hf, wf, crop, g_wlow, index=None, do_sigmoid=False):
    assert _f32c(g_wsel) and g_wsel.numel() >= n_max and _f32c(g_wlow) and g_wlow.numel() == hf * wf
    n_win = hf * wf if index is None else index.numel()
    check(_lib.load().woft_convex_weights_at_bwd(ptr(pts), ptr(count), n_max, ptr(g_wsel), ptr(wlow), ptr(mask), mask.shape[1],
                                                 hf, wf, crop[0], crop[1], int(do_sigmoid), ptr(index), n_win, ptr(g_wlow),
                                                 stream_ptr()), "woft_convex_weights_at_bwd")


def wh_reduce_bwd(act, w6, g_wlow, index, n_win, g_act, ws, g_w6, g_b6):
    assert _f32c(act) and _f32c(g_act) and act.numel() >= n_win * 81 * 128 and g_act.numel() >= n_win * 81 * 128
    assert ws.dtype == torch.float64 and ws.numel() >= -(-n_win // WH_TRAIN_CHUNK) * 129
    assert _f32c(w6) and w6.numel() >= 128 and _f32c(g_w6) and g_w6.numel() >= 128 and _f32c(g_b6)
    assert index is None or (index.dtype == torch.int32 and index.numel() >= n_win)
    check(_lib.load().woft_wh_reduce_bwd(ptr(act), ptr(w6), ptr(g_wlow), ptr(index), n_win, ptr(g_act), ptr(ws), ptr(g_w6),
                                         ptr(g_b6), stream_ptr()), "woft_wh_reduce_bwd")


def wh_train_conv(x, cin, wt, n_win, y, bias=None, gate=None):
    assert _f32c(x) and x.numel() >= n_win * 81 * cin and _f32c(wt, 9, cin, 128) and _f32c(y) and y.numel() >= n_win * 81 * 128
    assert bias is None or (_f32c(bias) and bias.numel() == 128)
    assert gate is None or (_f32c(gate) and gate.numel() >= n_win * 81 * 128)
    check(_lib.load().woft_wh_train_conv(ptr(x), cin, ptr(wt), ptr(bias), ptr(gate), n_win, ptr(y), stream_ptr()),
          "woft_wh_train_conv")


def wh_wgrad_ws_floats(n_win, cin):
    return int(_lib.load().woft_wh_wgrad_ws_bytes(n_win, cin)) // 4


def wh_wgrad(gy, x, cin, n_win, ws, gw, gb):
    assert _f32c(gy) and gy.numel() >= n_win * 81 * 128 and _f32c(x) and x.numel() >= n_win * 81 * cin
    assert _f32c(gw) and gw.shape[0] == 128 and tuple(gw.shape[2:]) == (3, 3) and _f32c(gb, 128)
    assert _f32c(ws) and ws.numel() >= wh_wgrad_ws_floats(n_win, cin)
    check(_lib.load().woft_wh_wgrad(ptr(gy), ptr(x), cin, gw.shape[1], n_win, ptr(ws), ptr(gw), ptr(gb), stream_ptr()),
          "woft_wh_wgrad")


def upflow8(coords, wlow, hf, wf, crop, h, w, flow_up=None, dst=None, wout=None, do_sigmoid=False):
# ... 218 lines not shown
```

Baseline: 124.3.

## Precompute banded correlation around each pixel once and reuse across RAFT iterations

Adds a band build pass that computes correlation values in a fixed window around each pixel's identity position at every pyramid level, run once per frame pair. Each iteration's lookup then interpolates from this band and falls back to the on-the-fly GEMM lookup only for blocks whose coordinates leave the band. The goal is to avoid recomputing the correlation dot products on every iteration. The cost is an extra build kernel, a per-pixel band buffer, a miss mask, and a fallback launch on every iteration, which loses out when flows are large.

```diff
diff --git a/include/woft_hip.h b/include/woft_hip.h
--- a/include/woft_hip.h
+++ b/include/woft_hip.h
@@ -147,6 +147,19 @@
     int32_t smp_y0, smp_x0, smp_h, smp_w;
 } woft_lookup_otf_params;
 int woft_corr_lookup_otf(const woft_lookup_otf_params* p, void* stream);
+#define WOFT_BAND_M0 3
+#define WOFT_BAND_LD 16
+#define WOFT_BAND_M(l) ((WOFT_BAND_M0 + (1 << (l)) - 1) >> (l))
+#define WOFT_BAND_W(radius, l) (2 * ((radius) + 1 + WOFT_BAND_M(l)))
+int woft_corr_band_geometry(int32_t radius, int32_t levels, int32_t* m, int32_t* w, int32_t* row_off);
+typedef struct woft_lookup_band_params {
+    woft_lookup_otf_params otf;
+    float* band;
+    int32_t* miss;
+    int32_t* miss_count;
+} woft_lookup_band_params;
+int woft_corr_band_build(const woft_lookup_band_params* p, void* stream);
+int woft_corr_lookup_band(const woft_lookup_band_params* p, void* stream);
 int woft_tile_rows(const float* in, int32_t h, int32_t w, int32_t c, float* out, void* stream);
 
 int woft_coords_update(float* coords1, const float* delta, int32_t ld_delta, int32_t wf, int64_t n_pix,
diff --git a/woft_amd/_lib.py b/woft_amd/_lib.py
--- a/woft_amd/_lib.py
+++ b/woft_amd/_lib.py
@@ -50,6 +50,10 @@
     ]
 
 
+class LookupBandParams(C.Structure):
+    _fields_ = LookupOtfParams._fields_ + [("band", vp), ("miss", vp), ("miss_count", vp)]
+
+
 _SIGS = {
     "woft_abi_version": (i32, []),
     "woft_sizeof": (i32, [i32]),
@@ -61,6 +65,9 @@
     "woft_split_bf16_lines": (i32, [vp, i64, vp, vp]),
     "woft_flow_to_tc": (i32, [vp, vp, i32, i32, vp, vp, i32, vp]),
     "woft_corr_lookup_otf": (i32, [C.POINTER(LookupOtfParams), vp]),
+    "woft_corr_band_geometry": (i32, [i32, i32, C.POINTER(i32), C.POINTER(i32), C.POINTER(i32)]),
+    "woft_corr_band_build": (i32, [C.POINTER(LookupBandParams), vp]),
+    "woft_corr_lookup_band": (i32, [C.POINTER(LookupBandParams), vp]),
     "woft_conv3x3_narrow": (i32, [vp, i32, i32, i32, i32, i32, vp, vp, i32, vp, i64, i32, vp]),
     "woft_flow_head_update": (i32, [vp, i32, i32, i32, i32, vp, vp, vp, i64, vp, vp, vp, i32, vp]),
     "woft_flow_head_gather": (i32, [vp, i32, i32, i32, i32, vp, vp, i64, vp, vp, vp, i32, vp]),
@@ -141,7 +148,7 @@
         fn = getattr(lib, name)
         fn.restype, fn.argtypes = res, args
     if lib.woft_sizeof(0) != C.sizeof(ConvParams) or lib.woft_sizeof(1) != C.sizeof(LookupParams) \
-            or lib.woft_sizeof(2) != C.sizeof(LookupOtfParams):
+            or lib.woft_sizeof(2) != C.sizeof(LookupOtfParams) or lib.woft_sizeof(3) != C.sizeof(LookupBandParams):
         raise WoftHipError("ctypes mirror of woft_conv_params / woft_lookup_params is out of sync with the library")
     _lib = lib
     return lib
diff --git a/woft_amd/csrc/elementwise.hip b/woft_amd/csrc/elementwise.hip
--- a/woft_amd/csrc/elementwise.hip
+++ b/woft_amd/csrc/elementwise.hip
@@ -301,6 +301,7 @@
     if (which == 0) return (int)sizeof(woft_conv_params);
     if (which == 1) return (int)sizeof(woft_lookup_params);
     if (which == 2) return (int)sizeof(woft_lookup_otf_params);
+    if (which == 3) return (int)sizeof(woft_lookup_band_params);
     return -1;
 }
 
diff --git a/woft_amd/csrc/lookup_band.hip b/woft_amd/csrc/lookup_band.hip
--- /dev/null
+++ b/woft_amd/csrc/lookup_band.hip
@@ -0,0 +1,172 @@
+#include "common.h"
+#include "lookup_blocks.h"
+
+namespace {
+
+template <int R>
+__global__ __launch_bounds__(256) void corr_lookup_band_kernel(const woft_lookup_band_params bp) {
+    const woft_lookup_otf_params& p = bp.otf;
+    constexpr int NPX = 64, NT = 256, MAXL = 4;
+    constexpr int NW = 2 * R + 1, N2 = NW * NW, WS = NW + 1;
+    constexpr int RS = WOFT_BAND_LD + 4;
+    constexpr int PLD = WS * RS;
+    constexpr int NLD = NPX * WS * 4 / NT;
+    static_assert(NLD * NT == NPX * WS * 4, "pieces divide among the threads");
+    __shared__ __attribute__((aligned(16))) float Wl[NPX * PLD];
+    __shared__ int s_ox[MAXL][NPX], s_oy[MAXL][NPX];
+    __shared__ float s_fx[MAXL][NPX], s_fy[MAXL][NPX];
+
+    const int tid = threadIdx.x;
+    const BlockRect br = block_rect(p);
+    const int tiles_x = br.nx, ntiles = br.nx * br.ny;
+    int tile;
+    {
+        const int q = ntiles / 8, rr = ntiles % 8, xcd = blockIdx.x % 8, idx = blockIdx.x / 8;
+        tile = (xcd < rr ? xcd * (q + 1) : rr * (q + 1) + (xcd - rr) * q) + idx;
+    }
+    const int px0 = (br.bx0 + tile % tiles_x) * 8, py0 = (br.by0 + tile / tiles_x) * 8;
+    const bool sampled = (p.smp_y0 | p.smp_x0 | p.smp_h | p.smp_w) == 0 ||
+                         (py0 < p.smp_y0 + p.smp_h && py0 + 8 > p.smp_y0 && px0 < p.smp_x0 + p.smp_w && px0 + 8 > p.smp_x0);
+    const int y = py0 + ((tid & 63) >> 3), x = px0 + (tid & 7);
+    const bool cvalid = tid < NPX && y < p.hf && x < p.wf;
+    const int64_t i = (int64_t)y * p.wf + x;
+    if (p.need != nullptr) {
+        const int any = cvalid ? p.need[i] : 0;
+        if (!__syncthreads_or(any)) {
+            if (cvalid) bp.miss[i] = 0;
+            return;
+        }
+    }
+    float cx = 0.f, cy = 0.f;
+    if (cvalid) {
+        cx = p.coords[i * 2];
+        cy = p.coords[i * 2 + 1];
+        if (p.fh_part != nullptr) {
+            typedef float f32x2 __attribute__((ext_vector_type(2)));
+            float dx = p.fh_bias ? p.fh_bias[0] : 0.f, dy = p.fh_bias ? p.fh_bias[1] : 0.f;
+            const int64_t plane = (int64_t)p.hf * p.wf * p.fh_ld;
+#pragma unroll
+            for (int ky = 0; ky < 3; ++ky)
+#pragma unroll
+                for (int kx = 0; kx < 3; ++kx) {
+                    const int yy = y + ky - 1, xx = x + kx - 1;
+                    f32x2 v = {0.f, 0.f};
+                    if (yy >= 0 && yy < p.hf && xx >= 0 && xx < p.wf) {
+                        const float* src = p.fh_part + ((int64_t)yy * p.wf + xx) * p.fh_ld + (ky * 3 + kx) * 2;
+                        v = *(const f32x2*)src;
+                        for (int t = 1; t < p.fh_planes; ++t) v += *(const f32x2*)(src + t * plane);
+                    }
+                    dx += v[0];
+                    dy += v[1];
+                }
+            p.fh_delta[i * p.fh_ld_delta] = dx;
+            p.fh_delta[i * p.fh_ld_delta + 1] = dy;
+            cx += dx;
+            cy += dy;
+            ((float*)p.coords)[i * 2] = cx;
+            ((float*)p.coords)[i * 2 + 1] = cy;
+            const float fx = cx - (float)x, fy = cy - (float)y;
+            if (p.fh_flow4 != nullptr) *(f32x4*)(p.fh_flow4 + i * 4) = f32x4{fx, fy, 0.f, 0.f};
+            if (p.fh_flow_cat != nullptr) {
+                p.fh_flow_cat[i * p.fh_ld_cat] = fx;
+                p.fh_flow_cat[i * p.fh_ld_cat + 1] = fy;
+            }
+        }
+    }
+    if (!sampled) {
+        if (cvalid) bp.miss[i] = 0;
+        return;
+    }
+    int ok = 1;
+    if (cvalid) {
+#pragma unroll
+        for (int l = 0; l < MAXL; ++l) {
+            if (l < p.levels) {
+                const float sc = 1.0f / (float)(1 << l);
+                const float xs = cx * sc, ys = cy * sc;
+                float flx = floorf(xs), fly = floorf(ys);
+                s_fx[l][tid] = xs - flx;
+                s_fy[l][tid] = ys - fly;
+                flx = fminf(fmaxf(flx, -1.0e6f), 1.0e6f);
+                fly = fminf(fmaxf(fly, -1.0e6f), 1.0e6f);
+                const int m = WOFT_BAND_M(l);
+                const int ox = (int)flx - (x >> l) + m, oy = (int)fly - (y >> l) + m;
+                ok &= (ox >= 0 && ox <= 2 * m && oy >= 0 && oy <= 2 * m) ? 1 : 0;
+                s_ox[l][tid] = ox;
+                s_oy[l][tid] = oy;
+            }
+        }
+    }
+    const int hit = __syncthreads_and(ok);
+    if (cvalid) bp.miss[i] = hit ? 0 : 1;
+    if (!hit) {
+        if (tid == 0) atomicAdd(bp.miss_count, 1);
+        return;
+    }
+    const int rows = band_row_off(R, p.levels);
+    f32x4 pc[NLD];
+    auto load_level = [&](int l) __attribute__((always_inline)) {
+        const int roff = band_row_off(R, l);
+#pragma unroll
+        for (int k = 0; k < NLD; ++k) {
+            const int it = tid + k * NT;
+            const int pix = it / (4 * WS), rem = it - pix * (4 * WS);
+            const int gy = py0 + (pix >> 3), gx = px0 + (pix & 7);
+            pc[k] = f32x4{0.f, 0.f, 0.f, 0.f};
+            if (gy < p.hf && gx < p.wf)
+                pc[k] = *(const f32x4*)(bp.band + (((int64_t)gy * p.wf + gx) * rows + roff + s_ox[l][pix]) * WOFT_BAND_LD + rem * 4);
+        }
+    };
+    load_level(0);
+    for (int l = 0; l < p.levels; ++l) {
+#pragma unroll
+        for (int k = 0; k < NLD; ++k) {
+            const int it = tid + k * NT;
+            const int pix = it / (4 * WS), rem = it - pix * (4 * WS);
+            *(f32x4*)(Wl + pix * PLD + (rem >> 2) * RS + (rem & 3) * 4) = pc[k];
+        }
+        __syncthreads();
+        if (l + 1 < p.levels) load_level(l + 1);
+        for (int it = tid; it < NPX * NW; it += NT) {
+            const int pix = it / NW, c = it - pix * NW;
+            const int gy = py0 + (pix >> 3), gx = px0 + (pix & 7);
+            if (gy >= p.hf || gx >= p.wf) continue;
+            const float fx = s_fx[l][pix], fy = s_fy[l][pix];
+            const float* cq = Wl + pix * PLD + c * RS + s_oy[l][pix];
+            float h[WS];
+#pragma unroll
+            for (int j = 0; j < WS; ++j) h[j] = cq[j] * (1.f - fx) + cq[RS + j] * fx;
+            float* o = p.out + ((int64_t)gy * p.wf + gx) * p.ldo + l * N2 + c * NW;
+#pragma unroll
+            for (int j = 0; j < NW; ++j) o[j] = h[j] * (1.f - fy) + h[j + 1] * fy;
+        }
+        __syncthreads();
+    }
+}
+
+}
+
+extern "C" int woft_corr_lookup_band(const woft_lookup_band_params* bp, void* stream) {
+    if (!bp || !bp->band || !bp->miss || !bp->miss_count) return WOFT_EINVAL;
+    const woft_lookup_otf_params& p = bp->otf;
+    if (p.levels < 1 || p.levels > 4 || !p.f1 || !p.coords || !p.out || p.hf <= 0 || p.wf <= 0 || p.ablate != 0) return WOFT_EINVAL;
+    if (p.terms != 1 && p.terms != 3) return WOFT_EINVAL;
+    if (!((p.k == 256 && p.radius == 4) || (p.k == 128 && p.radius == 3))) return WOFT_EINVAL;
+    for (int l = 0; l < p.levels; ++l)
+        if (p.h[l] <= 0 || p.w[l] <= 0) return WOFT_EINVAL;
+    const int nout = p.levels * (2 * p.radius + 1) * (2 * p.radius + 1);
+    if (p.ldo < nout) return WOFT_EINVAL;
+    if (p.fh_part != nullptr && (p.fh_delta == nullptr || p.fh_planes < 1 || p.fh_ld < 20 || p.fh_ld % 4 != 0 || p.fh_ld_delta < 2 ||
+                                 (p.fh_flow_cat != nullptr && p.fh_ld_cat < 2) || p.need != nullptr))
+        return WOFT_EINVAL;
+    auto rect_bad = [&](int y0, int x0, int h, int w) {
+        return (y0 | x0 | h | w) != 0 && (h <= 0 || w <= 0 || y0 < 0 || x0 < 0 || y0 > p.hf - h || x0 > p.wf - w);
+    };
+    if (rect_bad(p.roi_y0, p.roi_x0, p.roi_h, p.roi_w) || rect_bad(p.smp_y0, p.smp_x0, p.smp_h, p.smp_w)) return WOFT_EINVAL;
+    const BlockRect br = block_rect(p);
+    dim3 grid((unsigned)(br.nx * br.ny));
+    hipStream_t s = (hipStream_t)stream;
+    if (p.radius == 4) woft_launch(0, corr_lookup_band_kernel<4>, grid, dim3(256), 0, s, *bp);
+    else woft_launch(0, corr_lookup_band_kernel<3>, grid, dim3(256), 0, s, *bp);
+    return woft_launch_status();
+}
diff --git a/woft_amd/csrc/lookup_blocks.h b/woft_amd/csrc/lookup_blocks.h
--- /dev/null
+++ b/woft_amd/csrc/lookup_blocks.h
@@ -0,0 +1,17 @@
+#pragma once
+#include "common.h"
+
+struct BlockRect {
+    int by0, bx0, ny, nx;
+};
+__host__ __device__ __forceinline__ BlockRect block_rect(const woft_lookup_otf_params& p) {
+    if ((p.roi_y0 | p.roi_x0 | p.roi_h | p.roi_w) == 0) return BlockRect{0, 0, (p.hf + 7) / 8, (p.wf + 7) / 8};
+    const int by0 = p.roi_y0 / 8, bx0 = p.roi_x0 / 8;
+    return BlockRect{by0, bx0, (p.roi_y0 + p.roi_h - 1) / 8 - by0 + 1, (p.roi_x0 + p.roi_w - 1) / 8 - bx0 + 1};
+}
+
+__host__ __device__ __forceinline__ int band_row_off(int R, int l) {
+    int o = 0;
+    for (int i = 0; i < l; ++i) o += WOFT_BAND_W(R, i);
+    return o;
+}
diff --git a/woft_amd/csrc/lookup_otf.hip b/woft_amd/csrc/lookup_otf.hip
--- a/woft_amd/csrc/lookup_otf.hip
+++ b/woft_amd/csrc/lookup_otf.hip
@@ -3,6 +3,7 @@
 
 #include "common.h"
 #include "dma.h"
+#include "lookup_blocks.h"
 
 namespace {
 
@@ -38,16 +39,7 @@
                  : "memory", "vcc");
 }
 
-struct BlockRect {
-    int by0, bx0, ny, nx;
-};
-__host__ __device__ __forceinline__ BlockRect block_rect(const woft_lookup_otf_params& p) {
-    if ((p.roi_y0 | p.roi_x0 | p.roi_h | p.roi_w) == 0) return BlockRect{0, 0, (p.hf + 7) / 8, (p.wf + 7) / 8};
-    const int by0 = p.roi_y0 / 8, bx0 = p.roi_x0 / 8;
-    return BlockRect{by0, bx0, (p.roi_y0 + p.roi_h - 1) / 8 - by0 + 1, (p.roi_x0 + p.roi_w - 1) / 8 - bx0 + 1};
-}
-
-template <int TERMS, int R, int K, int ABL>
+template <int TERMS, int R, int K, int ABL, bool BAND = false>
 __global__ __launch_bounds__(256, 2) void corr_lookup_otf_kernel(const woft_lookup_otf_params p) {
     constexpr int NPX = 64, NT = 256;
     constexpr int NW = 2 * R + 1, N2 = NW * NW;
@@ -58,7 +50,7 @@
     constexpr int GS = 2, NGRP = 3, NST = GS * NGRP, DEPTH = NGRP - 1;
     static_assert(NK % GS == 0, "K steps per chunk must be a multiple of the steps per barrier");
     __shared__ __attribute__((aligned(16))) __bf16 stage[NST * 64 * 64];
-    constexpr int WS = NW + 1, WLD = WS * WS + 2;
+    constexpr int WS = NW + 1, WST = BAND ? WOFT_BAND_LD : WS, WLD = BAND ? WOFT_BAND_LD * WOFT_BAND_LD + 4 : WS * WS + 2;
     __shared__ __attribute__((aligned(16))) float Wn[NPX * WLD];
     constexpr int MAXL = 4;
     __shared__ __attribute__((aligned(16))) int s_org[MAXL][NPX];
@@ -85,7 +77,7 @@
     const int px0 = (br.bx0 + tile % tiles_x) * 8, py0 = (br.by0 + tile / tiles_x) * 8;
     const bool sampled = (p.smp_y0 | p.smp_x0 | p.smp_h | p.smp_w) == 0 ||
                          (py0 < p.smp_y0 + p.smp_h && py0 + 8 > p.smp_y0 && px0 < p.smp_x0 + p.smp_w && px0 + 8 > p.smp_x0);
-    if (p.need != nullptr) {
+    if (!BAND && p.need != nullptr) {
         int any = 0;
         if (tid < NPX) {
             const int y = py0 + (tid >> 3), x = px0 + (tid & 7);
@@ -94,7 +86,7 @@
         if (!__syncthreads_or(any)) return;
     }
     float cx = 0.f, cy = 0.f;
-    if (tid < NPX) {
+    if (!BAND && tid < NPX) {
         const int y = py0 + (tid >> 3), x = px0 + (tid & 7);
         if (y < p.hf && x < p.wf) {
             const int64_t i = (int64_t)y * p.wf + x;
@@ -133,7 +125,7 @@
             }
         }
     }
-    if (!sampled) return;
+    if (!BAND && !sampled) return;
     if (tid < NPX) {
         const int y = py0 + (tid >> 3), x = px0 + (tid & 7);
         const bool cvalid = y < p.hf && x < p.wf;
@@ -142,7 +134,10 @@
             if (l < p.levels) {
                 int wx0 = 0, wy0 = 0;
                 float fx = 0.f, fy = 0.f;
-                if (cvalid) {
+                if (BAND) {
+                    wx0 = (x >> l) - R - WOFT_BAND_M(l);
+                    wy0 = (y >> l) - R - WOFT_BAND_M(l);
+                } else if (cvalid) {
                     const float sc = 1.0f / (float)(1 << l);
                     const float xs = cx * sc, ys = cy * sc;
                     float flx = floorf(xs), fly = floorf(ys);
@@ -157,7 +152,7 @@
                 const int ox = wx0 < -16384 ? -16384 : (wx0 > 16384 ? 16384 : wx0);
                 const int oy = wy0 < -16384 ? -16384 : (wy0 > 16384 ? 16384 : wy0);
                 s_org[l][tid] = cvalid ? ((ox & 0xffff) | (oy << 16)) : 0x40004000;
-                s_pm[l][tid] = 4 * (tid * WLD - (ox * WS + oy));
+                s_pm[l][tid] = 4 * (tid * WLD - (ox * WST + oy));
                 const int b0 = wave_reduce_minmax<false>(cvalid ? wx0 : 0x3fffffff), b1 = wave_reduce_minmax<true>(cvalid ? wx0 : -0x3fffffff);
                 const int b2 = wave_reduce_minmax<false>(cvalid ? wy0 : 0x3fffffff), b3 = wave_reduce_minmax<true>(cvalid ? wy0 : -0x3fffffff);
                 if (tid == 0) { s_box[l][0] = b0; s_box[l][1] = b1; s_box[l][2] = b2; s_box[l][3] = b3; }
@@ -220,15 +215,16 @@
     };
     auto start_level = [&](int l) __attribute__((always_inline)) {
         W = sel4(l, p.w[0], p.w[1], p.w[2], p.w[3]);
+        const int NWL = BAND ? WOFT_BAND_W(R, l) - 1 : NW;
         const int H = sel4(l, p.h[0], p.h[1], p.h[2], p.h[3]);
         bx0 = __builtin_amdgcn_readfirstlane(s_box[l][0]);
         by0 = __builtin_amdgcn_readfirstlane(s_box[l][2]);
         int bx1 = __builtin_amdgcn_readfirstlane(s_box[l][1]), by1 = __builtin_amdgcn_readfirstlane(s_box[l][3]);
-        clipped = bx0 < 0 || by0 < 0 || bx1 + NW > W - 1 || by1 + NW > H - 1;
+        clipped = bx0 < 0 || by0 < 0 || bx1 + NWL > W - 1 || by1 + NWL > H - 1;
         bx0 = bx0 > 0 ? bx0 : 0;
         by0 = by0 > 0 ? by0 : 0;
-        bx1 = (bx1 + NW < W - 1) ? bx1 + NW : W - 1;
-        by1 = (by1 + NW < H - 1) ? by1 + NW : H - 1;
+        bx1 = (bx1 + NWL < W - 1) ? bx1 + NWL : W - 1;
+        by1 = (by1 + NWL < H - 1) ? by1 + NWL : H - 1;
         bw = bx1 - bx0 + 1;
         const int bh = by1 - by0 + 1;
         N = (bw > 0 && bh > 0) ? bw * bh : 0;
@@ -323,7 +319,7 @@
                 const int by = pos / bw, bx = pos - by * bw;
                 const int tx = bx0 + bx, ty = by0 + by;
                 const int d_pos = pos < N ? ((tx & 0xffff) | (ty << 16)) : 0x7fff7fff;
-                const uint32_t d_q4 = lds_addr_of(Wn) + 4u * (uint32_t)(tx * WS + ty);
+                const uint32_t d_q4 = lds_addr_of(Wn) + 4u * (uint32_t)(tx * WST + ty);
                 const uint32_t trash = lds_addr_of(s_trash) + 4u * (uint32_t)lane;
                 i32x4 org[4], pm[4];
 #pragma unroll
@@ -331,7 +327,8 @@
                     org[g4] = *(const i32x4*)&s_org[l][wm * 32 + 4 * hh + 8 * g4];
                     pm[g4] = *(const i32x4*)&s_pm[l][wm * 32 + 4 * hh + 8 * g4];
                 }
-                const u16x2 lim = {(unsigned short)(WS - 1), (unsigned short)(WS - 1)};
+                const unsigned short lim1 = (unsigned short)(BAND ? WOFT_BAND_W(R, l) - 1 : WS - 1);
+                const u16x2 lim = {lim1, lim1};
 #pragma unroll
                 for (int r = 0; r < 16; ++r) {
                     const u16x2 dd = __builtin_bit_cast(u16x2, d_pos) - __builtin_bit_cast(u16x2, (int)org[r >> 2][r & 3]);
@@ -349,7 +346,19 @@
         stamp();
         __syncthreads();
         if (l + 1 < p.levels) start_level(l + 1);
-        if (!(ABL & 8)) {
+        if constexpr (BAND) {
+            const int wl = WOFT_BAND_W(R, l), roff = band_row_off(R, l), rows = band_row_off(R, p.levels);
+            for (int it = tid; it < NPX * WOFT_BAND_LD * 4; it += NT) {
+                const int pix = it >> 6, c = (it >> 2) & 15, q4 = it & 3;
+                const int gy = py0 + (pix >> 3), gx = px0 + (pix & 7);
+                if (c >= wl || gy >= p.hf || gx >= p.wf) continue;
+                f32x4 v = *(const f32x4*)(Wn + pix * WLD + c * WST + q4 * 4);
+#pragma unroll
+                for (int e = 0; e < 4; ++e)
+                    if (q4 * 4 + e >= wl) v[e] = 0.f;
+                *(f32x4*)(p.out + (((int64_t)gy * p.wf + gx) * rows + roff + c) * WOFT_BAND_LD + q4 * 4) = v;
+            }
+        } else if (!(ABL & 8)) {
             for (int it = tid; it < NPX * NW; it += NT) {
                 const int pix = it / NW, i = it - pix * NW;
                 const int gy = py0 + (pix >> 3), gx = px0 + (pix & 7);
@@ -424,3 +433,41 @@
 #undef OTF
     return woft_launch_status();
 }
+
+extern "C" int woft_corr_band_geometry(int32_t radius, int32_t levels, int32_t* m, int32_t* w, int32_t* row_off) {
+    if (radius < 1 || levels < 1 || levels > 4 || WOFT_BAND_W(radius, 0) > WOFT_BAND_LD) return WOFT_EINVAL;
+    for (int l = 0; l < levels; ++l) {
+        if (m) m[l] = WOFT_BAND_M(l);
+        if (w) w[l] = WOFT_BAND_W(radius, l);
+        if (row_off) row_off[l] = band_row_off(radius, l);
+    }
+    return band_row_off(radius, levels);
+}
+
+extern "C" int woft_corr_band_build(const woft_lookup_band_params* bp, void* stream) {
+    if (!bp || !bp->band) return WOFT_EINVAL;
+    woft_lookup_otf_params p = bp->otf;
+    if (p.levels < 1 || p.levels > 4 || !p.f1 || p.hf <= 0 || p.wf <= 0 || p.ablate != 0) return WOFT_EINVAL;
+    if (p.terms != 1 && p.terms != 3) return WOFT_EINVAL;
+    if (!((p.k == 256 && p.radius == 4) || (p.k == 128 && p.radius == 3))) return WOFT_EINVAL;
+    const int64_t row_bytes = (int64_t)p.k * (p.terms == 1 ? 2 : 4);
+    if ((int64_t)p.hf * p.wf * row_bytes >= (1ll << 32)) return WOFT_EINVAL;
+    for (int l = 0; l < p.levels; ++l)
+        if (!p.f2[l] || p.h[l] <= 0 || p.w[l] <= 0 || p.h[l] > 16384 || p.w[l] > 16384 ||
+            (int64_t)p.h[l] * p.w[l] * row_bytes >= (1ll << 32) - 4096)
+            return WOFT_EINVAL;
+    p.out = bp->band;
+    p.coords = nullptr;
+    p.need = nullptr;
+    p.fh_part = nullptr;
+    p.roi_y0 = p.roi_x0 = p.roi_h = p.roi_w = 0;
+    p.smp_y0 = p.smp_x0 = p.smp_h = p.smp_w = 0;
+    hipStream_t s = (hipStream_t)stream;
+    const BlockRect br = block_rect(p);
+    dim3 grid((unsigned)(br.nx * br.ny));
+#define BANDK(T, RR, KK) woft_launch(0, corr_lookup_otf_kernel<T, RR, KK, 0, true>, grid, dim3(256), 0, s, p)
+    if (p.radius == 4) { if (p.terms == 3) BANDK(3, 4, 256); else BANDK(1, 4, 256); }
+    else               { if (p.terms == 3) BANDK(3, 3, 128); else BANDK(1, 3, 128); }
+#undef BANDK
+    return woft_launch_status();
+}
diff --git a/woft_amd/engine.py b/woft_amd/engine.py
--- a/woft_amd/engine.py
+++ b/woft_amd/engine.py
@@ -14,6 +14,8 @@
 PAIR_BRANCHES = os.environ.get("WOFT_PAIR", "1") != "0"
 PYRAMID_ONE_LAUNCH = os.environ.get("WOFT_PYRAMID", "1") != "0"
 FOLD_GATHER = os.environ.get("WOFT_FOLD_GATHER", "1") != "0"
+CORR_BAND = os.environ.get("WOFT_CORR_BAND", "1") != "0"
+BAND_MIN_LOOKUPS = 6
 
 
 def _ru(x, m):
@@ -107,7 +109,7 @@
 
 class RaftEngine:
     def __init__(self, state_dict, small=False, weighted=True, precision="fp32", corr="volume", volume_storage=None,
-                 mask_head=False):
+                 mask_head=False, corr_band="auto"):
         if precision not in ops.PRECISION:
             raise ValueError(f"precision must be one of {sorted(ops.PRECISION)}")
         if corr not in ("volume", "otf"):
@@ -115,6 +117,9 @@
         self.precision = precision
         self.prec_corr = self.prec_wh = "bf16x3" if precision in ("fp16", "f16mx8") else precision
         self.corr = corr
+        if corr_band not in ("auto", True, False):
+            raise ValueError("corr_band must be 'auto', True or False")
+        self.corr_band = corr_band
         self.volume_storage = volume_storage or ("bf16" if precision == "bf16" else "fp32")
         if self.volume_storage not in ("fp32", "bf16") or (self.volume_storage == "bf16" and precision == "fp32"):
             raise ValueError("volume_storage: 'fp32', or 'bf16' with the split-bf16 precisions (their GEMM packs it)")
@@ -255,6 +260,10 @@
         self.wh_events = None
         self.conv_events = None
         self._graphs = {}
+        self._band = None
+        self.band_valid = False
+        self._band_params = {}
+        self._graph_band = {}
         self.mk = self.mask = self.prog_iter_last = self.folded = self.fh_part = None
         self.x8 = self.x32 = self.wmean = self.wlow = self.cs_ws = self.cs_tot = self.wh6_b = self._wh6_pad = None
         self.a1 = self.a2 = self.wh0_t = self.wh_last = None
@@ -718,7 +727,54 @@
                 raise ValueError(kind)
 
     def _lookup(self, params):
+        if self.band_valid:
+            _timed(self.lookup_events, self._lookup_band, params)
+            return
         _timed(self.lookup_events, ops.run_lookup_otf if self.otf else ops.run_lookup, params)
+
+    def band_applies(self, lookups, flow_init=None):
+        e, sp = self.eng, self.eng.spec
+        if not CORR_BAND or e.corr_band is False or not self.otf or self.prec == "fp32" or flow_init is not None:
+            return False
+        if (sp.radius, sp.fdim) not in ops.BAND_INSTANCES or sp.levels > 4:
+            return False
+        return e.corr_band is True or lookups >= BAND_MIN_LOOKUPS
+
+    def _band_buffers(self):
+        if self._band is None:
+            sp = self.eng.spec
+            rows = ops.band_geometry(sp.radius, sp.levels)[3]
+            i32 = lambda n: torch.zeros(n, dtype=torch.int32, device="cuda")
+            self._band = (torch.zeros(self.P * rows * ops.BAND_LD, dtype=torch.float32, device="cuda"), i32(self.P), i32(1))
+        return self._band
+
+    def _band_build(self):
+        band, miss, count = self._band_buffers()
+        count.zero_()
+        ops.run_band_build(self._band_variant(self.lookup))
+        self.band_valid = True
+
+    def _band_variant(self, params):
+        key = id(params)
+        if key not in self._band_params:
+            band, miss, count = self._band_buffers()
+            fb = ops.copy_params(params)
+            fb.fh_part, fb.need = None, _lib.ptr(miss)
+            fb._keep = (getattr(params, "_keep", None), miss)
+            self._band_params[key] = (params, ops.make_lookup_band_params(params, band, miss, count), fb)
+        _, bp, fb = self._band_params[key]
+        bp.need = params.need
+        bp._fallback = fb
+        return bp
+
+    def _lookup_band(self, params):
+        bp = self._band_variant(params)
+        ops.run_lookup_band(bp)
+        ops.run_lookup_otf(bp._fallback)
+
+    @property
+    def band_miss_blocks(self):
+        return 0 if self._band is None else int(self._band[2].item())
 
     def _split(self, rows, out):
         if self.prec_corr == "bf16x3":
@@ -731,6 +787,7 @@
 
     def encode_source(self, reuse_target=False):
         reused = bool(reuse_target) and self.otf and self.target_valid
+        self.band_valid = False
         if reused:
             self.f1rows[:self.P].copy_(self.f2act[0].t.view(self.P, -1))
             if self.prec != "fp32":
@@ -754,6 +811,7 @@
 
     def encode_record(self, record):
         self.source_tag, self.target_valid = None, False
+        self.band_valid = False
         self.run(self.prog_f_src)
         self.run(self.prog_c_src)
         ops.features_pack(self.f1rows, self.net0.t, self.xbuf.t, self.P, self.record_dims, record)
@@ -761,6 +819,7 @@
     def restore_source(self, record):
         x3 = self.prec != "fp32" and self.prec_corr == "bf16x3"
         self.source_tag = None
+        self.band_valid = False
         ops.features_unpack(record, self.P, self.record_dims, self.f1rows, self.f1s if x3 else None, self.net0.t, self.xbuf.t,
                             self.inp_c.t)
         if self.prec != "fp32" and not x3:
@@ -769,6 +828,7 @@
 
     def restore_target(self, record):
         self.target_valid = False
+        self.band_valid = False
         ops.features_unpack(record, self.P, self.record_dims, self.f2act[0].t)
 
     def set_flow_init(self, flow_init):
@@ -785,10 +845,13 @@
         e, sp = self.eng, self.eng.spec
         if iters < 1:
             raise ValueError("iters must be >= 1")
+        self.band_valid = False
         if not target_restored:
             self.run(self.prog_f_dst)
         self.run(self.prog_volume)
         self.target_valid = True
+        if self.band_applies(iters + (1 if e.weighted and not skip_wh else 0), flow_init):
+            self._band_build()
         if flow_init is None:
             ops.coords_init(self.coords, self.hf, self.wf, self.flow4.t, self.flow_cat, self.xbuf.cs)
         else:
diff --git a/woft_amd/flow_provider.py b/woft_amd/flow_provider.py
--- a/woft_amd/flow_provider.py
+++ b/woft_amd/flow_provider.py
@@ -132,8 +132,11 @@
         logger.log(logging.WARNING if self.precision_source.startswith("built-in default") else logging.INFO, note)
         self.precision_note = note
         self.corr = os.environ.get("WOFT_CORR") or getattr(self.C, "corr", None) or "otf"
+        v = getattr(self.C, "corr_band", None)
+        self.corr_band = "auto" if (v is None or isinstance(v, type(self.C))) else (v if v == "auto" else bool(v))
         self.engine = RaftEngine(state_dict, small=small, weighted=weighted, precision=self.precision, corr=self.corr,
-                                 volume_storage=getattr(self.C, "volume_storage", None), mask_head=self.masked)
+                                 volume_storage=getattr(self.C, "volume_storage", None), mask_head=self.masked,
+                                 corr_band=self.corr_band)
         self._wh_loaded = {k: v for k, v in state_dict.items() if k.startswith("weight_head.net.")}
         self._wh_params, self._wh_flow = None, None
         v = getattr(self.C, "flow_region", None)
@@ -192,8 +195,10 @@
                 with torch.cuda.graph(g):
                     eager()
             plan._graphs[key] = g
+            plan._graph_band[key] = plan.band_valid
         else:
             g.replay()
+            plan.band_valid = plan._graph_band[key]
 
     def finish_weights(self, pts, count, n_max, out=None):
         plan, crop, oh, ow, o, do_sigmoid = self._deferred
diff --git a/woft_amd/ops.py b/woft_amd/ops.py
--- a/woft_amd/ops.py
+++ b/woft_amd/ops.py
@@ -7,7 +7,7 @@
 import torch
 
 from . import _lib, conv_select
-from ._lib import ConvParams, LookupOtfParams, LookupParams, check, ptr, stream_ptr
+from ._lib import ConvParams, LookupBandParams, LookupOtfParams, LookupParams, check, ptr, stream_ptr
 from .conv_select import KERNELS, PRECISION, Kernel, pair_ok
 
 DEV = "cuda"
@@ -411,6 +411,45 @@
     check(_lib.load().woft_corr_lookup_otf(C.byref(p), stream_ptr()), "woft_corr_lookup_otf")
 
 
+BAND_M0, BAND_LD = 3, 16
+BAND_INSTANCES = ((4, 256), (3, 128))
+
+
+def band_m(l):
+    return (BAND_M0 + (1 << l) - 1) >> l
+
+
+def band_geometry(radius, levels):
+    m = [band_m(l) for l in range(levels)]
+    w = [2 * (radius + 1 + ml) for ml in m]
+    off = [sum(w[:l]) for l in range(levels)]
+    return m, w, off, sum(w)
+
+
+def band_hit(cx, cy, x, y, levels):
+    for l in range(levels):
+        s = 1.0 / (1 << l)
+        if abs(math.floor(cx * s) - (x >> l)) > band_m(l) or abs(math.floor(cy * s) - (y >> l)) > band_m(l):
+            return False
+    return True
+
+
+def make_lookup_band_params(otf, band, miss, miss_count):
+    p = LookupBandParams()
+    C.memmove(C.byref(p), C.byref(otf), C.sizeof(LookupOtfParams))
+    p.band, p.miss, p.miss_count = ptr(band), ptr(miss), ptr(miss_count)
+    p._keep = (getattr(otf, "_keep", None), band, miss, miss_count)
+    return p
+
+
+def run_band_build(p):
+    check(_lib.load().woft_corr_band_build(C.byref(p), stream_ptr()), "woft_corr_band_build")
+
+
+def run_lookup_band(p):
+    check(_lib.load().woft_corr_lookup_band(C.byref(p), stream_ptr()), "woft_corr_lookup_band")
+
+
 def split_bf16_lines(x, out):
     check(_lib.load().woft_split_bf16_lines(ptr(x), x.numel(), ptr(out), stream_ptr()), "woft_split_bf16_lines")
 
```

Result: faster. 127.1, median of 6 (+2.3%).
